# lbroseus/TALC

Hardware: AMD Instinct MI355X
Metric: corrected long-read bases/sec (whole node); k-mer-probe HBM GB/s (higher is better)
Workload: dtype u8

## Files before the change

talc_amd/csrc/pure_capi.cpp:

```cpp
#include <algorithm>
#include <cstdint>
#include <vector>

#include "talc_pure.h"
#include "talc_wfa.h"

using namespace talc;

extern "C" {

int pure_is_expected_by_model(double alpha, uint32_t nextc, uint32_t cc, int classe_unexpected) {
  return is_expected_by_model(alpha, nextc, cc, classe_unexpected != 0) ? 1 : 0;
}
int pure_is_expected_by_last_node(double alpha, uint32_t nextc, uint32_t cc) {
  return is_expected_by_last_node(alpha, nextc, cc) ? 1 : 0;
}
int pure_tag_next_nodes(double alpha, double err, uint32_t minc, const uint32_t* cnt4, const uint32_t* jc4, uint32_t count,
                        int complex, int32_t* tags4, double* dist4) {
  int t[4];
  double d[4];
  int n = tag_next_nodes(alpha, err, minc, cnt4, jc4, count, complex != 0, t, d);
  for (int i = 0; i < 4; ++i) { tags4[i] = t[i]; dist4[i] = d[i]; }
  return n;
}

struct KP { int32_t key; int32_t payload; };
struct KPLess { bool operator()(const KP& a, const KP& b) const { return a.key < b.key; } };
void pure_gnu_sort_pairs(int32_t* keys, int32_t* payloads, int n) {
  std::vector<KP> v(n);
  for (int i = 0; i < n; ++i) v[i] = KP{keys[i], payloads[i]};
  gnu_sort(v.data(), n, KPLess());
  for (int i = 0; i < n; ++i) { keys[i] = v[i].key; payloads[i] = v[i].payload; }
}
void pure_std_sort_pairs(int32_t* keys, int32_t* payloads, int n) {
  std::vector<KP> v(n);
  for (int i = 0; i < n; ++i) v[i] = KP{keys[i], payloads[i]};
  std::sort(v.begin(), v.end(), KPLess());
  for (int i = 0; i < n; ++i) { keys[i] = v[i].key; payloads[i] = v[i].payload; }
}

void pure_gnu_heapsort_pairs(int32_t* keys, int32_t* payloads, int n) {
  std::vector<KP> v(n);
  for (int i = 0; i < n; ++i) v[i] = KP{keys[i], payloads[i]};
  gs_heapsort(v.data(), 0, n, KPLess());
  for (int i = 0; i < n; ++i) { keys[i] = v[i].key; payloads[i] = v[i].payload; }
}
void pure_std_heapsort_pairs(int32_t* keys, int32_t* payloads, int n) {
  std::vector<KP> v(n);
  for (int i = 0; i < n; ++i) v[i] = KP{keys[i], payloads[i]};
  std::partial_sort(v.begin(), v.end(), v.end(), KPLess());
  for (int i = 0; i < n; ++i) { keys[i] = v[i].key; payloads[i] = v[i].payload; }
}

int pure_gardening(uint32_t maxb, int n, const double* scores, const double* dists, uint32_t* kept, int32_t* isComplex) {
  std::vector<ValIdx> wv(n + 1);
  std::vector<Rank4> r1(n + 1), r2(n + 1);
  bool cx = false;
  int nk = gardening(maxb, n, scores, dists, wv.data(), r1.data(), r2.data(), kept, &cx);
  *isComplex = cx ? 1 : 0;
  return nk;
}

void pure_sort_anchors(double cc, uint32_t* pos, uint32_t* count, int n) {
  std::vector<AnchorRec> a(n);
  for (int i = 0; i < n; ++i) a[i] = AnchorRec{0, 0, pos[i], count[i]};
  gnu_sort(a.data(), n, LessAnchor{cc});
  for (int i = 0; i < n; ++i) { pos[i] = a[i].pos; count[i] = a[i].count; }
}

void pure_wfa_xdrop(const uint8_t* q, int qlen, const uint8_t* d, int dlen, int x, int32_t* out4) {
  const WfaResult r = wfa_xdrop_scalar(q, qlen, d, dlen, x);
  out4[0] = r.moved; out4[1] = r.extCols; out4[2] = r.extRows; out4[3] = r.score;
}
}
```

talc_amd/csrc/talc_capi_correct.inc:

```

static uint32_t next_launch_stamp() {
  static std::atomic<uint32_t> launches{0};
  return 0x01000000u + (launches.fetch_add(1) & 0xFFFFFFu);
}
static void ensure_edge_boxes(talc_ctx* c, Stage& st) {
  const uint64_t gap = (uint64_t)c->p.max_border_length + 256;
  const uint32_t seqCap = (uint32_t)align_up((uint64_t)(2.2 * (double)gap) + 4ull * c->p.k + 64, 16);
  const uint64_t need = (uint64_t)st.n_slots * edge_box_bytes(seqCap) + (uint64_t)st.n_slots * 4;
  if (c->sw.edgeTasks == 0 || c->p.max_start_anchors < 2 || c->p.max_start_anchors > EDGE_BOX_ANCHORS ||
      seqCap > (1u << 16) || need > (1ull << 30)) {
    st.boxes.reset(); st.boxes_bytes = 0;
    return;
  }
  if (need > st.boxes_bytes || seqCap != st.box_seq_cap) {
    st.boxes.reset(); st.boxes_bytes = 0;
    if (st.boxes.alloc(need) != hipSuccess) { (void)hipGetLastError(); return; }
    st.boxes_bytes = need; st.box_seq_cap = seqCap;
  }
}

static int ensure_stage(talc_ctx* c, Stage& st, uint32_t maxLen, uint32_t scale, uint32_t n_work) {
  const SearchCaps caps = make_caps(maxLen, c->p.k, scale, scale == 1 ? c->sw.seqArena : 0, scale == 1 && c->sw.tinyCaps);
  hipDeviceProp_t prop;
  HIPCHK(hipGetDeviceProperties(&prop, c->device));
  uint32_t want = (uint32_t)prop.multiProcessorCount * (scale == 1 ? 4u * TALC_SEARCH_WAVES_PER_SIMD : scale <= 8 ? 4u : 1u);
  if (c->sw.searchSlots) want = c->sw.searchSlots;
  const uint32_t wantSlots = std::max<uint32_t>(1, std::min<uint32_t>(want, n_work));
  if (scale > 1 && c->sw.failRetryAlloc)
    return fail(TALC_ERR_NOMEM, "TALC_TEST_FAIL_RETRY_ALLOC: the retry stage is refused");
  for (int attempt = 0; attempt < 2; ++attempt) {
    uint32_t slots = wantSlots;
    size_t freeB = 0, totalB = 0;
    HIPCHK(hipMemGetInfo(&freeB, &totalB));
    const uint64_t avail = (uint64_t)(0.6 * (double)freeB) + st.scratch_bytes;
    while (slots > 1 && (uint64_t)slots * caps.slotBytes > avail) slots /= 2;
    const uint64_t need = (uint64_t)slots * caps.slotBytes;
    const bool cramped = slots < wantSlots || (uint64_t)caps.slotBytes > avail;
    if (cramped && attempt == 0 && c->cache.pool_bytes) { c->cache.trim(0); continue; }
    if ((uint64_t)caps.slotBytes > avail && need > st.scratch_bytes)
      return fail(TALC_ERR_NOMEM, "per-wave scratch of %llu bytes does not fit the device", (unsigned long long)caps.slotBytes);
    if (need > st.scratch_bytes) {
      st.scratch.reset(); st.scratch_bytes = 0;
      if (st.scratch.alloc(need) != hipSuccess) {
        (void)hipGetLastError();
        if (attempt == 0) { c->cache.trim(0); continue; }
        return fail(TALC_ERR_NOMEM, "cannot allocate %llu bytes of search scratch", (unsigned long long)need);
      }
      st.scratch_bytes = need;
    }
    st.n_slots = slots;
    st.caps = caps;
    return TALC_OK;
  }
  return fail(TALC_ERR_NOMEM, "search scratch does not fit the device");
}

struct TraceHost {
  DevBuf<TraceRec> d_recs; DevBuf<uint32_t> d_nrec; DevBuf<uint8_t> d_pool; DevBuf<uint32_t> d_npool;
  uint32_t cap = 0, poolCap = 0;
};

#ifdef TALC_PROF
static int prof_report(talc_ctx* c, talc_batch* b, const uint64_t* counters) {
  if (!c->sw.profReads.empty()) {
    if (FILE* f = fopen(c->sw.profReads.c_str(), "w")) {
      fprintf(f, "read\tlen\tstatus\tregions\tcost_est\thead\ttail\tgap_sum\tfork\tsolid\tticks_100MHz\tgap_sq\tgap_max\tsq640\tsteps\tedge_ticks\tanchors\tanchor_max\tstart\tbridges\tbridge_max\n");
      for (uint32_t r = 0; r < b->n_reads; ++r) {
        const ReadState& st = b->h_state[r];
        fprintf(f, "%u\t%llu\t%d\t%u\t%u\t%u\t%u\t%u\t%u\t%u\t%u\t%u\t%u\t%u\t%u\t%u\t%u\t%u\t%u\t%u\t%u\n", r, (unsigned long long)(b->h_offsets[r + 1] - b->h_offsets[r]), st.status,
                st.nRegions, st.costEst, st.pfHead, st.pfTail, st.pfGapSum, st.pfFork, st.pfSolid, st.pfTicks, st.pfGapSq, st.pfGapMax, st.pfShortReg, st.pfSteps, st.pfEdgeTicks, st.pfAnchors, st.pfAnchorMax, st.pfStart, st.pfBridges, st.pfBridgeMax);
      }
      fclose(f);
    }
  }
  if (!c->sw.profPrint) return TALC_OK;
  static const char* nm[] = TALC_PF_NAMES;
  const uint64_t tot = counters[2 + PF_TOTAL];
  for (int i = 0; i < PF_N; ++i) fprintf(stderr, "[prof] %-10s %14llu cycles  %5.1f%%\n", nm[i], (unsigned long long)counters[2 + i], tot ? 100.0 * counters[2 + i] / tot : 0.0);
  if (counters[127] > counters[126] && c->stage.n_slots)
    fprintf(stderr, "[prof] wave utilisation: %.1f%% of %u waves x %.3f ms (first start to last end, 100 MHz counter)\n",
            100.0 * (double)counters[125] / ((double)(counters[127] - counters[126]) * c->stage.n_slots), c->stage.n_slots,
            (double)(counters[127] - counters[126]) / 1e5);
  if (counters[124] != ~0ull && counters[124] > counters[126])
    fprintf(stderr, "[prof] the work queue ran dry %.3f ms after the first wave's start\n", (double)(counters[124] - counters[126]) / 1e5);
  if (c->sw.profSlow && c->stage.n_slots) {
    const uint32_t nw = std::min<uint32_t>(c->stage.n_slots, 8192);
    std::vector<uint64_t> lg(2 * (size_t)nw);
    HIPCHK(hipMemcpy(lg.data(), c->d_counters.get() + 128, lg.size() * 8, hipMemcpyDeviceToHost));
    std::vector<uint32_t> idx(nw);
    for (uint32_t i = 0; i < nw; ++i) idx[i] = i;
    const uint32_t t0 = (uint32_t)counters[126];
    auto endOf = [&](uint32_t w) { return (uint32_t)((uint32_t)lg[2 * w + 1] - t0); };
    std::sort(idx.begin(), idx.end(), [&](uint32_t a, uint32_t b2) { return endOf(a) > endOf(b2); });
    fprintf(stderr, "[slow] wave end times (ms), deciles from the last:");
    for (int d = 0; d <= 10; ++d) fprintf(stderr, " %.1f", endOf(idx[std::min<uint32_t>(nw - 1, (uint32_t)((uint64_t)d * nw / 10))]) / 1e5);
    fprintf(stderr, "\n");
    for (uint32_t i = 0; i < std::min<uint32_t>(nw, 24); ++i) {
      const uint32_t w = idx[i];
      const uint32_t qi = (uint32_t)(lg[2 * w] >> 32), r = (uint32_t)lg[2 * w], st = (uint32_t)(lg[2 * w + 1] >> 32) - t0;
      const uint64_t L = (b->h_offsets.empty() || r >= b->n_reads) ? 0 : b->h_offsets[r + 1] - b->h_offsets[r];
      fprintf(stderr, "[slow] wave %5u ends %8.3f ms: last read %7u (queue %7u, len %6llu) started %8.3f ms\n", w, endOf(w) / 1e5, r, qi,
              (unsigned long long)L, st / 1e5);
    }
  }
  return TALC_OK;
}
#endif

static int run_pipeline(talc_ctx* c, talc_batch* b, TraceHost* th, uint32_t traceRead) {
  HIPCHK(hipSetDevice(c->device));
  hipStream_t s = c->stream;
  int rc;
  TraceBuf tb = {};
  if (th) { tb.recs = th->d_recs.get(); tb.nrec = th->d_nrec.get(); tb.cap = th->cap; tb.pool = th->d_pool.get(); tb.npool = th->d_npool.get(); tb.poolCap = th->poolCap; tb.steps = c->sw.traceSteps ? 1 : 0; }
  memset(&c->timing, 0, sizeof c->timing);
  c->timing.n_kmers = b->n_kmers; c->timing.n_bases = b->n_bases;
  HIPCHK(hipEventRecord(c->ev[0], s));
  if (!b->encoded && (rc = launch_encode(c, b))) return rc;
  HIPCHK(hipEventRecord(c->ev[1], s));
  if ((rc = launch_coverage(c, b))) return rc;
  HIPCHK(hipEventRecord(c->ev[2], s));
  HIPCHK(hipMemsetAsync(c->d_hist.get() + 1024, 0, 256 * sizeof(uint32_t), s));
  if (b->n_reads)
    hipLaunchKernelGGL(k_structure, dim3(b->n_reads), dim3(64), 0, s, c->dp, c->view, b->d_codes.get(), b->d_offsets.get(), b->d_koff.get(),
                       b->d_cov.get(), b->d_covw.get(), b->d_nin.get(), b->d_state.get(), b->d_regions.get(), b->d_regoff.get(), b->d_headcov.get(), b->n_reads, tb, traceRead, c->d_hist.get() + 1024);
  HIPCHK(hipGetLastError());
  HIPCHK(hipEventRecord(c->ev[3], s));
  if (b->n_reads) {
    HIPCHK(hipMemsetAsync(c->d_hist.get(), 0, 1024 * sizeof(uint32_t), s));
    const unsigned nb = (b->n_reads + 255) / 256;
    hipLaunchKernelGGL(k_order_scale, dim3(1), dim3(64), 0, s, c->d_hist.get() + 1024);
    hipLaunchKernelGGL(k_order_hist, dim3(nb), dim3(256), 0, s, b->d_state.get(), b->n_reads, c->d_hist.get(), c->d_hist.get() + 1024);
    hipLaunchKernelGGL(k_order_scan, dim3(1), dim3(1024), 0, s, c->d_hist.get());
    hipLaunchKernelGGL(k_order_scatter, dim3(nb), dim3(256), 0, s, b->d_state.get(), b->n_reads, c->d_hist.get(), b->d_order.get(), c->d_hist.get() + 1024);
    HIPCHK(hipGetLastError());
  }
  HIPCHK(hipMemsetAsync(c->d_queue.get(), 0, kQueueWords * sizeof(uint32_t), s));
  HIPCHK(hipMemsetAsync(c->d_counters.get(), 0, (128 + 2 * 8192) * sizeof(uint64_t), s));
  HIPCHK(hipMemsetAsync(c->d_counters.get() + 126, 0xFF, sizeof(uint64_t), s));
  HIPCHK(hipMemsetAsync(c->d_counters.get() + 124, 0xFF, sizeof(uint64_t), s));
  if (b->n_reads) {
    if ((rc = ensure_stage(c, c->stage, b->max_len, 1, b->n_reads))) return rc;
    ensure_edge_boxes(c, c->stage);
    EdgeTaskArgs ea = {};
    if (c->stage.boxes) {
      ea.boxes = c->stage.boxes.get();
      ea.avail = (uint32_t*)(c->stage.boxes.get() + (uint64_t)c->stage.n_slots * edge_box_bytes(c->stage.box_seq_cap));
      ea.seqCap = c->stage.box_seq_cap;
      ea.minWeak = c->sw.edgeTaskMin; ea.heavy = c->sw.edgeTaskHeavy; ea.heavyRounds = c->sw.edgeTaskRounds;
      ea.lingerMod = c->sw.edgeLingerMod; ea.test = c->sw.edgeRedo ? 1u : 0u;
      ea.autoSwitch = c->sw.edgeTasks > 0 ? nullptr : c->d_hist.get() + 1024 + 129;
      HIPCHK(hipMemsetAsync(ea.avail, 0, (uint64_t)c->stage.n_slots * 4, s));
    }
    hipLaunchKernelGGL(k_search, dim3(c->stage.n_slots), dim3(64), 0, s, c->dp, c->view, c->stage.caps, b->d_codes.get(), b->d_offsets.get(),
                       b->d_koff.get(), b->d_cov.get(), b->d_covw.get(), b->d_state.get(), b->d_regions.get(), b->d_regoff.get(), b->d_headcov.get(), b->d_out.get(), b->d_outoff.get(), b->d_order.get(),
                       b->n_reads, c->d_queue.get(), c->stage.scratch.get(), c->d_counters.get(), tb, traceRead, next_launch_stamp(), ea);
    HIPCHK(hipGetLastError());
  }
  HIPCHK(hipEventRecord(c->ev[4], s));
  b->h_state.resize(b->n_reads);
  if (b->n_reads) HIPCHK(hipMemcpyAsync(b->h_state.data(), b->d_state.get(), b->n_reads * sizeof(ReadState), hipMemcpyDeviceToHost, s));
  HIPCHK(hipStreamSynchronize(s));
  std::vector<uint32_t> retry;
  for (uint32_t r = 0; r < b->n_reads; ++r) if (b->h_state[r].overflow) retry.push_back(r);
  c->timing.n_retried = (uint32_t)retry.size();
  HIPCHK(hipEventRecord(c->ev[5], s));
  for (uint32_t scale = 8; scale <= 64 && !retry.empty(); scale *= 8) {
    Stage big;
    if ((rc = ensure_stage(c, big, b->max_len, scale, (uint32_t)retry.size()))) {
      if (rc == TALC_ERR_NOMEM) break;
      return rc;
    }
    DevBuf<uint32_t> d_retry;
    if (d_retry.alloc(retry.size()) != hipSuccess) { (void)hipGetLastError(); break; }
    HIPCHK(hipMemcpyAsync(d_retry.get(), retry.data(), retry.size() * 4, hipMemcpyHostToDevice, s));
    for (uint32_t r : retry) {
      b->h_state[r].overflow = 0;
      HIPCHK(hipMemcpyAsync(b->d_state.get() + r, &b->h_state[r], sizeof(ReadState), hipMemcpyHostToDevice, s));
    }
    HIPCHK(hipMemsetAsync(c->d_queue.get(), 0, kQueueWords * sizeof(uint32_t), s));
    hipLaunchKernelGGL(k_search, dim3(big.n_slots), dim3(64), 0, s, c->dp, c->view, big.caps, b->d_codes.get(), b->d_offsets.get(), b->d_koff.get(),
                       b->d_cov.get(), b->d_covw.get(), b->d_state.get(), b->d_regions.get(), b->d_regoff.get(), b->d_headcov.get(), b->d_out.get(), b->d_outoff.get(), d_retry.get(), (uint32_t)retry.size(),
                       c->d_queue.get(), big.scratch.get(), c->d_counters.get(), tb, traceRead, next_launch_stamp(), EdgeTaskArgs());
    HIPCHK(hipGetLastError());
    HIPCHK(hipMemcpyAsync(b->h_state.data(), b->d_state.get(), b->n_reads * sizeof(ReadState), hipMemcpyDeviceToHost, s));
    HIPCHK(hipStreamSynchronize(s));
    d_retry.reset(); big = Stage();
    std::vector<uint32_t> again;
    for (uint32_t r : retry) if (b->h_state[r].overflow) again.push_back(r);
    retry.swap(again);
  }
  HIPCHK(hipEventRecord(c->ev[6], s));
  uint32_t nfail = 0;
  std::vector<uint64_t> dense_off(b->n_reads + 1);
  uint64_t pos = 0;
  for (uint32_t r = 0; r < b->n_reads; ++r) {
    dense_off[r] = pos;
    pos += b->h_state[r].outLen;
    if (b->h_state[r].overflow) nfail++;
  }
  dense_off[b->n_reads] = pos;
  b->h_dense_off = dense_off;
  if (b->d_dense && b->dense_cap < pos) b->d_dense.reset();
  if (!b->d_dense) { b->dense_cap = std::max<uint64_t>(pos, 1); HIPCHK(b->d_dense.alloc(c->cache, b->dense_cap)); }
  if (!b->d_dense_off) HIPCHK(b->d_dense_off.alloc(c->cache, b->n_reads + 1));
  HIPCHK(hipMemcpyAsync(b->d_dense_off.get(), dense_off.data(), (b->n_reads + 1) * 8, hipMemcpyHostToDevice, s));
  if (b->n_reads)
    hipLaunchKernelGGL(k_pack, dim3(b->n_reads), dim3(256), 0, s, b->d_out.get(), b->d_outoff.get(), b->d_state.get(), b->d_dense_off.get(), b->d_dense.get(),
                       b->n_reads, c->p.reverse ? 1 : 0);
  HIPCHK(hipGetLastError());
  HIPCHK(hipEventRecord(c->ev[7], s));
  uint64_t counters[128] = {0};
  HIPCHK(hipMemcpyAsync(counters, c->d_counters.get(), 128 * 8, hipMemcpyDeviceToHost, s));
  HIPCHK(hipStreamSynchronize(s));
  HIPCHK(hipEventElapsedTime(&c->timing.encode_ms, c->ev[0], c->ev[1]));
  HIPCHK(hipEventElapsedTime(&c->timing.coverage_ms, c->ev[1], c->ev[2]));
  HIPCHK(hipEventElapsedTime(&c->timing.structure_ms, c->ev[2], c->ev[3]));
  HIPCHK(hipEventElapsedTime(&c->timing.search_ms, c->ev[3], c->ev[4]));
  HIPCHK(hipEventElapsedTime(&c->timing.retry_ms, c->ev[5], c->ev[6]));
  HIPCHK(hipEventElapsedTime(&c->timing.emit_ms, c->ev[6], c->ev[7]));
  c->timing.n_trail_steps = counters[0];
  c->timing.n_dp_cells = counters[1];
  c->timing.n_failed = nfail;
#ifdef TALC_PROF
  if ((rc = prof_report(c, b, counters))) return rc;
#endif
  b->corrected = true;
  if (nfail) {
    fail(TALC_WARN_READ_ERRORS, "%u read(s) exhausted the device scratch even in the retry pass (status TALC_READ_ERROR)", nfail);
    return TALC_WARN_READ_ERRORS;
  }
  return TALC_OK;
}

int talc_batch_correct(talc_ctx* c, talc_batch* b) {
  if (!c || !b || b->ctx != c) return fail(TALC_ERR_INVALID, "bad context/batch");
  return run_pipeline(c, b, nullptr, 0xFFFFFFFFu);
}

uint64_t talc_batch_corrected_bytes(const talc_batch* b) { return (b && b->corrected) ? b->h_dense_off[b->n_reads] : 0; }

int talc_batch_fetch_corrected(talc_ctx* c, talc_batch* b, char* out, uint64_t out_capacity, uint64_t* out_offsets,
                               int32_t* status) {
  if (!c || !b || b->ctx != c) return fail(TALC_ERR_INVALID, "bad context/batch");
  if (!b->corrected) return fail(TALC_ERR_STATE, "talc_batch_correct has not run on this batch");
  HIPCHK(hipSetDevice(c->device));
  const uint64_t total = b->h_dense_off[b->n_reads];
  if (out_offsets) memcpy(out_offsets, b->h_dense_off.data(), (b->n_reads + 1) * 8);
  if (status)
    for (uint32_t r = 0; r < b->n_reads; ++r) status[r] = b->h_state[r].overflow ? TALC_READ_ERROR : b->h_state[r].status;
  if (out) {
    if (out_capacity < total) return fail(TALC_ERR_CAPACITY, "output buffer too small: need %llu bytes", (unsigned long long)total);
    if (total) {
      HIPCHK(hipMemcpyAsync(out, b->d_dense.get(), total, hipMemcpyDeviceToHost, c->stream));
      HIPCHK(hipStreamSynchronize(c->stream));
    }
  }
  return TALC_OK;
}

int talc_batch_fetch_read_stats(talc_ctx* c, talc_batch* b, int64_t* stats5) {
  if (!c || !b || b->ctx != c || !stats5) return fail(TALC_ERR_INVALID, "bad context/batch/buffer");
  if (!b->corrected) return fail(TALC_ERR_STATE, "talc_batch_correct has not run on this batch");
  const uint32_t K = c->p.k;
  for (uint32_t r = 0; r < b->n_reads; ++r) {
    const ReadState& st = b->h_state[r];
    const uint64_t L = b->h_offsets[r + 1] - b->h_offsets[r];
    int64_t* o = stats5 + 5ull * r;
    const bool row = L > K;
    const bool corrected = st.status == TALC_READ_CORRECTED && !st.overflow;
    o[0] = row ? 1 : 0;
    o[1] = row ? (int64_t)L : 0;
    o[2] = (row && st.status != TALC_READ_NO_SOLID_KMER && st.status != TALC_READ_SKIPPED_SHORT) ? (int64_t)st.inSpan : 0;
    o[3] = (row && st.status != TALC_READ_NO_SOLID_KMER && st.status != TALC_READ_SKIPPED_SHORT) ? (int64_t)st.nRegions : 0;
    o[4] = (row && corrected) ? (int64_t)st.outLen : 0;
  }
  return TALC_OK;
}

int talc_batch_copy_corrected_device(talc_ctx* c, talc_batch* b, void* device_out, uint64_t out_capacity,
                                     uint64_t* out_offsets, int32_t* status) {
  if (!c || !b || b->ctx != c || !device_out) return fail(TALC_ERR_INVALID, "bad context/batch/buffer");
  if (!b->corrected) return fail(TALC_ERR_STATE, "talc_batch_correct has not run on this batch");
  HIPCHK(hipSetDevice(c->device));
  const uint64_t total = b->h_dense_off[b->n_reads];
  if (out_offsets) memcpy(out_offsets, b->h_dense_off.data(), (b->n_reads + 1) * 8);
  if (status)
    for (uint32_t r = 0; r < b->n_reads; ++r) status[r] = b->h_state[r].overflow ? TALC_READ_ERROR : b->h_state[r].status;
  if (out_capacity < total) return fail(TALC_ERR_CAPACITY, "device buffer too small: need %llu bytes", (unsigned long long)total);
  if (total) {
    HIPCHK(hipMemcpyAsync(device_out, b->d_dense.get(), total, hipMemcpyDeviceToDevice, c->stream));
    HIPCHK(hipStreamSynchronize(c->stream));
  }
  return TALC_OK;
}

int talc_correct_batch(talc_ctx* c, const char* bases, const uint64_t* offsets, uint32_t n_reads, char* out,
                       uint64_t out_capacity, uint64_t* out_offsets, int32_t* status) {
  talc_batch* b = nullptr;
  int rc = talc_batch_create(c, bases, offsets, n_reads, &b);
  if (rc) return rc;
  rc = talc_batch_correct(c, b);
  int rc2 = (rc >= 0) ? talc_batch_fetch_corrected(c, b, out, out_capacity, out_offsets, status) : rc;
  talc_batch_destroy(b);
  return rc2 ? rc2 : rc;
}

int64_t talc_batch_trace_read(talc_ctx* c, talc_batch* b, uint32_t read_index, char* buf, uint64_t cap) {
  if (!c || !b || b->ctx != c || read_index >= b->n_reads) return fail(TALC_ERR_INVALID, "bad context/batch/read index");
  HIPCHK(hipSetDevice(c->device));
  const uint64_t off = b->h_offsets[read_index], len = b->h_offsets[read_index + 1] - off;
  std::vector<char> raw(std::max<uint64_t>(len, 1));
  if (len) HIPCHK(hipMemcpy(raw.data(), b->d_raw.get() + off, len, hipMemcpyDeviceToHost));
  uint64_t offs[2] = {0, len};
  talc_batch* one = nullptr;
  int rc = talc_batch_create(c, raw.data(), offs, 1, &one);
  if (rc) return rc;
  const std::unique_ptr<talc_batch> tbch(one);
  TraceHost th;
  th.cap = 1u << 18; th.poolCap = 1u << 24;
  HIPCHK(th.d_recs.alloc(th.cap));
  HIPCHK(th.d_nrec.alloc(1)); HIPCHK(th.d_npool.alloc(1));
  HIPCHK(th.d_pool.alloc(th.poolCap));
  HIPCHK(hipMemsetAsync(th.d_nrec.get(), 0, 4, c->stream)); HIPCHK(hipMemsetAsync(th.d_npool.get(), 0, 4, c->stream));
  rc = run_pipeline(c, tbch.get(), &th, 0);
  std::ostringstream os;
  uint32_t nrec = 0, npool = 0;
  HIPCHK(hipMemcpy(&nrec, th.d_nrec.get(), 4, hipMemcpyDeviceToHost));
  HIPCHK(hipMemcpy(&npool, th.d_npool.get(), 4, hipMemcpyDeviceToHost));
  nrec = std::min(nrec, th.cap); npool = std::min(npool, th.poolCap);
  std::vector<TraceRec> recs(nrec);
  std::vector<uint8_t> pool(std::max<uint32_t>(npool, 1));
  if (nrec) HIPCHK(hipMemcpy(recs.data(), th.d_recs.get(), (size_t)nrec * sizeof(TraceRec), hipMemcpyDeviceToHost));
  if (npool) HIPCHK(hipMemcpy(pool.data(), th.d_pool.get(), npool, hipMemcpyDeviceToHost));
  const int stv = tbch->h_state.empty() ? -1 : (tbch->h_state[0].overflow ? TALC_READ_ERROR : tbch->h_state[0].status);
  os << "STATUS " << stv << "\n";
// ... 40 lines not shown
```

talc_amd/csrc/talc_kernels_search.h:

```cpp
#pragma once
#include "talc_common.h"
#include "talc_kernels_probe.h"
#include "talc_pure.h"
#include "talc_wave.h"

namespace talc {

#define TCAP 288
#define NBUF (2 * TCAP)
#ifndef LDS_DP_CAP
#define LDS_DP_CAP 320
#endif
#ifndef HOT
#define HOT 8
#endif
#ifndef AIMS_LDS
#define AIMS_LDS 16
#endif

enum : uint32_t {
  OVF_ANCHORS = 1, OVF_FULLPATHS = 2, OVF_FULLPOOL = 4, OVF_TRAILS = 8, OVF_SEQ = 16, OVF_OUT = 32, OVF_WEAKPOOL = 64,
  OVF_REGIONS = 128, OVF_DP = 256
};

// ... 384 lines not shown
          ++new_start_pos;
          if (degree_of(new_start_pos, 0) > 1) OK = true;
        }
      }
      uint32_t new_end_pos = regEnd;
      if (OK & !lastAndNone) {
        int degEnd;
        if (reg < Rdeg) degEnd = (int)s_degE[reg];
        else degEnd = degree_of(new_end_pos, 1);
        if ((degEnd == 0) & (new_end_pos != n - 1)) {
          OK = false;
          while ((new_end_pos > regS[reg]) & !OK) {
            --new_end_pos;
            if (degree_of(new_end_pos, 1) > 1) OK = true;
          }
        }
      }
      if (OK) {
        if (reg + 1 < R) span = ((int)regS[reg + 1] - (int)(new_end_pos + K));
        if (span < 0) {
          if ((int)regE[reg + 1] + span >= (int)regS[reg + 1]) { if (l == 0) regS[reg + 1] = regS[reg + 1] - (uint32_t)span; }
          else { if (l == 0) regS[reg + 1] = new_start_pos; OK = false; }
          startMoved = true;
          WSYNC();
        }
        if (OK) {
          uint32_t c = 0;
          for (uint32_t i = new_start_pos + l; i <= new_end_pos; i += 64) c = max(c, cov_at(cov, i).x);
          c = wave_max_u32(c);
          const bool expected = !is_expected_by_model(P.ALPHA, c, solidThr, true);
          if (expected) {
            WSYNC();
            if (l == 0) { regS[nNew] = new_start_pos; regE[nNew] = new_end_pos; }
            WSYNC();
            ++nNew;
          }
        }
      }
    }
  }
  uint32_t Rfinal = (nNew > 0) ? nNew : R;
  bool checok = (R > 0);

  if (Rfinal > 0) {
    unsigned long long len = 0;
    if (regS[0] > 0) len += regS[0];
    const uint32_t eLast = regE[Rfinal - 1];
    if (eLast + 1 < n) len += (unsigned long long)L - ((unsigned long long)eLast + K);
    unsigned long long part = 0;
    for (uint32_t i = l; i + 1 < Rfinal; i += 64) {
      part += (unsigned long long)regE[i] + K - regS[i];
      if (regS[i + 1] > regE[i] + K) part += (unsigned long long)regS[i + 1] - ((unsigned long long)regE[i] + K);
    }
    len += wave_sum_u64(part);
    len += (unsigned long long)eLast + K - regS[Rfinal - 1];
    checok &= (len == (unsigned long long)L);
  }
  st.nRegions = Rfinal;
  if (l < kHeadCov) headCov[(uint64_t)r * kHeadCov + (uint32_t)l] = ((uint32_t)l < n) ? cov_at(cov, (uint32_t)l).x : 0u;
  {
    WSYNC();
    uint32_t* regH = regS + 2 * regCap;
    for (uint32_t i = l; i < Rfinal; i += 64) {
      const uint32_t s0 = regS[i], e0 = regE[i];
      const uint32_t hs = cov_hit_index(cov, s0);
      const bool endHit = ((cov_word(cov, e0 >> 6).bits >> (e0 & 63u)) & 1ull) != 0ull;
      const bool clean = ((s0 ^ e0) < (uint32_t)TALC_COV_TILE) && (e0 >= s0) && endHit && (cov_hit_index(cov, e0) - hs == e0 - s0);
      regH[i] = (hs & ~kRegClean) | (clean ? kRegClean : 0u);
    }
  }
  {
    unsigned long long part = 0;
    for (uint32_t i = l; i < Rfinal; i += 64) part += (unsigned long long)regE[i] - regS[i] + 1;
    st.inSpan = (uint32_t)wave_sum_u64(part);
  }
  if (!checok) st.status = TALC_READ_NO_STRUCTURE;
  if (checok && Rfinal > 0) {
    unsigned long long part = 0, sq = 0;
    for (uint32_t i = l; i + 1 < Rfinal; i += 64) {
      const unsigned long long g = (regS[i + 1] > regE[i] + K) ? (unsigned long long)(regS[i + 1] - (regE[i] + K)) : 0ull;
      part += 870ull * g + 20000ull;
      sq += g * g;
    }
    const unsigned long long gq = (unsigned long long)P.costGapQuad + ((unsigned long long)P.costGapFork * nFork) / max(m, 1ull);
    unsigned long long cost = wave_sum_u64(part) + gq * min(wave_sum_u64(sq), (unsigned long long)P.costGapCap * P.costGapCap);
    st.costGap = (uint32_t)min(cost >> 6, 0xFFFFFFFFull);
    if (l == 0) { atomicAdd(&batchStats[2 * (r & 63u)], (uint32_t)min(nFork, 0xFFFFull)); atomicAdd(&batchStats[2 * (r & 63u) + 1], (uint32_t)min(m, 0xFFFFFull)); }
    const unsigned long long head = regS[0], eLast = regE[Rfinal - 1];
    const unsigned long long tail = (eLast + 1 < n) ? (unsigned long long)L - (eLast + K) : 0ull;
    if (head > 0 && head <= P.MAX_BORDER_LEN) cost += (unsigned long long)P.costEdgeLin * head + (unsigned long long)P.costEdgeQuad * head * head;
    if (tail > 0 && tail <= P.MAX_BORDER_LEN) cost += (unsigned long long)P.costEdgeLin * tail + (unsigned long long)P.costEdgeQuad * tail * tail;
    cost += 50ull * (unsigned long long)L;
#ifdef TALC_PROF
    {
      unsigned long long gs = 0;
      for (uint32_t i = l; i + 1 < Rfinal; i += 64) gs += (regS[i + 1] > regE[i] + K) ? (unsigned long long)(regS[i + 1] - (regE[i] + K)) : 0ull;
      st.pfGapSum = (uint32_t)wave_sum_u64(gs);
      unsigned long long g2 = 0, sr = 0; uint32_t gm = 0;
      for (uint32_t i = l; i < Rfinal; i += 64) {
        const unsigned long long g = (i + 1 < Rfinal && regS[i + 1] > regE[i] + K) ? (unsigned long long)(regS[i + 1] - (regE[i] + K)) : 0ull;
        g2 += g * g; gm = max(gm, (uint32_t)g); sr += min(g, 640ull) * min(g, 640ull);
      }
      st.pfGapSq = (uint32_t)min(wave_sum_u64(g2), 0xFFFFFFFFull); st.pfGapMax = wave_max_u32(gm); st.pfShortReg = (uint32_t)wave_sum_u64(sr); st.pfSteps = 0;
      st.pfHead = (uint32_t)head; st.pfTail = (uint32_t)tail; st.pfFork = (uint32_t)nFork; st.pfSolid = (uint32_t)m; st.pfTicks = 0;
    }
#endif
    cost >>= 6;
    st.costEst = (uint32_t)min(cost, 0xFFFFFFFFull);
  }
  if (l == 0) state[r] = st;
  if (trace.recs && r == traceRead && l == 0) {
    uint32_t k = atomicAdd(trace.nrec, 1u);
    if (k < trace.cap) trace.recs[k] = TraceRec{TR_THRESHOLD, 0, 0, 0, 0, thr, 0, 0};
    for (uint32_t i = 0; i < Rfinal; ++i) {
      k = atomicAdd(trace.nrec, 1u);
      if (k < trace.cap) trace.recs[k] = TraceRec{TR_REGION, (int)regS[i], (int)regE[i], 0, 0, 0.0, 0, 0};
    }
  }
}

struct TrailSet {
  uint64_t* kmer; uint64_t* nmask; double* dist; uint32_t* cnt; int32_t* score; uint32_t* fail; int32_t* lanc;
  int32_t* ranc; uint32_t* buf;
};
TALC_D TrailSet make_set(uint8_t* meta) {
  TrailSet s;
  s.kmer = (uint64_t*)(meta + TrailSetLayout::kmer); s.nmask = (uint64_t*)(meta + TrailSetLayout::nmask);
  s.dist = (double*)(meta + TrailSetLayout::dist); s.cnt = (uint32_t*)(meta + TrailSetLayout::cnt);
  s.score = (int32_t*)(meta + TrailSetLayout::score); s.fail = (uint32_t*)(meta + TrailSetLayout::fail);
  s.lanc = (int32_t*)(meta + TrailSetLayout::lanc); s.ranc = (int32_t*)(meta + TrailSetLayout::ranc);
  s.buf = (uint32_t*)(meta + TrailSetLayout::buf);
  return s;
}

struct TrailRec { uint64_t kmer, nmask; double dist; uint32_t cnt; int32_t score; uint32_t fail; int32_t lanc, ranc; uint32_t buf; };

#define LSYNC() do { __builtin_amdgcn_fence(__ATOMIC_ACQ_REL, "wavefront"); __builtin_amdgcn_wave_barrier(); } while (0)

__shared__ TrailRec g_hot[2 * HOT];
__shared__ uint64_t g_aimK[AIMS_LDS], g_aimN[AIMS_LDS];
__shared__ uint32_t g_aimPos[AIMS_LDS];
#define BLOOM_WORDS 128
__shared__ unsigned long long g_bloom[BLOOM_WORDS];
__shared__ __attribute__((aligned(16))) int g_dp[3 * LDS_DP_CAP];

struct EdgeCand {
  bool have; double score; double dist; double idscore; uint32_t len; uint32_t lanc, ranc;
};

enum { PF_PROBE = 0, PF_CHILD, PF_AIMS, PF_CYCLE, PF_FFWD, PF_SCOREBR, PF_GARDEN, PF_EVALFULL, PF_XDROP, PF_EXTNW,
       PF_EDGEMISC, PF_ANCHORS, PF_ASSEMBLE, PF_STEPB, PF_STEPE, PF_SRCHB, PF_SRCHE, PF_PROLOG, PF_INITTR, PF_TOTAL, PF_NCALLS, PF_NSTEPS,
       PF_FFLOAD, PF_FFREC, PF_FFFLUSH, PF_FFENTRY, PF_NRECS, PF_RD0, PF_RD1, PF_RD2, PF_RD3, PF_RD4, PF_RD5, PF_RDMAX,
       PF_XSTAGE, PF_XLEV, PF_XSEL, PF_REFB, PF_RESULT, PF_CYQ, PF_CYX, PF_CYHIT, PF_CYFILL,
       PF_SB11, PF_SB12, PF_SB21, PF_SB10, PF_SBOTHER, PF_SEGEN, PF_XCALLS, PF_XNLEV, PF_FSFORK, PF_FSDEAD, PF_FSFILT, PF_FSLIM, PF_FK1, PF_FK2, PF_FKBAIL, PF_FORK, PF_ANCCALLS, PF_ANCITER, PF_TPUB, PF_TOWN, PF_TSTOLEN, PF_TWAIT, PF_TRUN, PF_EA0, PF_EA1, PF_EA2, PF_EA3, PF_EA4, PF_EASUM3, PF_EASUM4, PF_RANCH, PF_RANCHMAX, PF_RBR, PF_RBRMAX, PF_N };
#define TALC_PF_NAMES {"probe", "child", "aims", "cycle", "ffwd", "scorebr", "garden", "evalfull", "xdrop", "extnw", "edgemisc", \
                       "anchors", "assemble", "stepb*", "stepe*", "srchb*", "srche*", "prolog", "inittr", "total", "#ffcalls", "#ffsteps", \
                       "ff.load", "ff.record", "ff.flush", "ff.entry", "#ffrecords", "#reads<0.25ms", "#reads<1ms", "#reads<4ms", \
                       "#reads<16ms", "#reads<64ms", "#reads>=64ms", "maxread(10ns)", "x.stage", "x.levels", "x.select", "b.ref", "b.result", \
                       "#cyc.query", "#cyc.exact", "#cyc.found", "cyc.fill%sum", \
                       "#stepb 1->1", "#stepb 1->2", "#stepb 2->1", "#stepb 1->0", "#stepb other", "#stepe generic", "#xdrop calls", "#xdrop levels", \
                       "#ffstop fork", "#ffstop deadend", "#ffstop filter", "#ffstop limit/other", "#forkstep 1 child", "#forkstep fork+deadend", "#forkstep bailed", "forkstep", "#anchor lists", "#anchor level tests", \
                       "#edges published", "#anchors by owner", "#anchors by others", "t.owner waits", "t.run by others", \
                       "#edge anchors<1ms", "#edge anchors<4ms", "#edge anchors<16ms", "#edge anchors<64ms", "#edge anchors>=64ms", "ticks anchors 16-64ms", "ticks anchors>=64ms", "(per read) anchors", "(per read) longest anchor", "(per read) bridge attempts", "(per read) longest bridge attempt"}

struct Wv {
  DevParams P; TableView T; SearchLimits C;
  const uint8_t* read; uint32_t L, n; const uint2* cov; double lambda;
  TrailSet G[2];
  int ia;
  uint8_t* seqPool;
  uint32_t nBuf;
  unsigned long long freeMask[NBUF / 64];
  uint8_t *ref, *fullPool, *edgeLong, *edgeShort, *edgeTmp, *weak;
  AnchorRec *ancL, *ancR; uint32_t* ancPos;
  FullMeta* fullMeta;
  int *dpG;
  double* gScores; double* gDists; ValIdx* gVal; Rank4* gRank; uint32_t* gKept;
  uint32_t *regS, *regE, *wOff, *wLen;
  int location, dirRight;
  uint32_t Ls, Le, Rs, Re;
  uint32_t weakLen;
  bool complexRegion;
  bool ffPopped;
  int nAncL, nAncR;
  uint32_t refLen;
  int nFull; uint32_t fullUsed;
  EdgeCand best2[2];
  int nEdges;
  unsigned long long cells, steps;
  uint32_t overflow;
  const TraceBuf* tracep;
  bool tracing, traceSteps;
  unsigned long long* wideBloom;
  int* rowPool;
  uint32_t searchNo;
  uint32_t rowStride, rowAvail;
  uint32_t wideMask;
  uint32_t launchStamp;
  const CovWord* covw;
  uint32_t* regH;
  uint32_t LH, RH;
  const uint32_t* headCov;
  uint8_t* refBuf;
  uint8_t* boxes; uint32_t* avail; uint32_t* qwords;
  uint32_t boxBytes, boxSeqCap, nSlots, mySlot, nWork, taskMinWeak;
  uint32_t taskHeavy;
  uint32_t qi, heavyUpTo;
  uint32_t holding;
  uint32_t stealSeq;
  unsigned long long moreCells, moreSteps;
  uint32_t nanSeen;
  uint32_t taskTest;
};

enum { LOC_HEAD = 0, LOC_INNER = 1, LOC_TAIL = 2 };

__shared__ Wv g_X;
#define X g_X
#ifdef TALC_PROF
__shared__ uint32_t g_prof[PF_N];
#endif

#ifdef TALC_PROF
#define PROF_DECL unsigned long long _pf_t
#define PF_EDGE_T0() (_pf_e0 = __builtin_amdgcn_s_memrealtime())
#define PF_EDGE_T1() (_pf_edge += (uint32_t)(__builtin_amdgcn_s_memrealtime() - _pf_e0))
#define PROF_BEGIN() (_pf_t = __builtin_amdgcn_s_memtime())
#define PROF_END(cat) (g_prof[cat] += (uint32_t)(__builtin_amdgcn_s_memtime() - _pf_t))
#define PROF_DECL2 unsigned long long _pf_t2
#define PROF_COUNT(cat, n) do { if (lane_id() == 0) g_prof[cat] += (uint32_t)(n); } while (0)
#define PROF_BEGIN2() (_pf_t2 = __builtin_amdgcn_s_memtime())
#define PROF_END2(cat) (g_prof[cat] += (uint32_t)(__builtin_amdgcn_s_memtime() - _pf_t2))
#else
#define PROF_DECL
#define PF_EDGE_T0() ((void)0)
#define PF_EDGE_T1() ((void)0)
#define PROF_BEGIN() ((void)0)
#define PROF_END(cat) ((void)0)
#define PROF_DECL2
#define PROF_COUNT(cat, n) ((void)0)
#define PROF_BEGIN2() ((void)0)
#define PROF_END2(cat) ((void)0)
#endif

TALC_D CovRead cur_cov() { CovRead c; c.hits = (const uint2 TALC_AS1*)X.cov; c.words = (const CovWord TALC_AS1*)X.covw; return c; }
TALC_DNC unsigned long long cov_lookup(uint32_t i) { const uint2 v = cov_at(cur_cov(), i); return ((unsigned long long)v.y << 32) | v.x; }
#define COVX(i) ((uint32_t)cov_lookup(i))
#define COVY(i) ((uint32_t)(cov_lookup(i) >> 32))

TALC_D int* dp_array(int which, int need) {
  if ((uint32_t)need > X.C.dpCap) { X.overflow |= OVF_DP; }
  return X.dpG + (uint64_t)which * X.C.dpCap;
}

#define NW_REG_NB 12
TALC_DNC int nw_score(const uint8_t* a, int la, const uint8_t* b, int lb, int match, int mismatch, int gap,
                    bool freeBegin) {
  la = uni(la); lb = uni(lb);
  if (la < lb) { const uint8_t* t = a; a = b; b = t; int tl = la; la = lb; lb = tl; }
  unsigned long long ncells = 0;
  if (la <= 64 * NW_REG_NB) {
    const int B = (la + 63) >> 6;
    int r;
    if (B <= 1) r = wave_nw_reg<1>(a, la, b, lb, match, mismatch, gap, freeBegin, ncells);
    else if (B <= 2) r = wave_nw_reg<2>(a, la, b, lb, match, mismatch, gap, freeBegin, ncells);
    else if (B <= 3) r = wave_nw_reg<3>(a, la, b, lb, match, mismatch, gap, freeBegin, ncells);
    else if (B <= 4) r = wave_nw_reg<4>(a, la, b, lb, match, mismatch, gap, freeBegin, ncells);
    else if (B <= 6) r = wave_nw_reg<6>(a, la, b, lb, match, mismatch, gap, freeBegin, ncells);
    else if (B <= 8) r = wave_nw_reg<8>(a, la, b, lb, match, mismatch, gap, freeBegin, ncells);
    else r = wave_nw_reg<NW_REG_NB>(a, la, b, lb, match, mismatch, gap, freeBegin, ncells);
    X.cells += ncells;
    return r;
  }
  if ((uint32_t)(la + 1) > X.C.dpCap) { X.overflow |= OVF_DP; return 0; }
  int* row = dp_array(0, la + 1);
  const int r = wave_nw(a, la, b, lb, match, mismatch, gap, freeBegin, row, ncells);
  X.cells += ncells;
  return r;
}

#define NW2_REG_NB 8
TALC_DNC unsigned long long edit_and_lcs_sweep(const uint8_t* a, int la_, const uint8_t* b, int lb_, bool haveEdit_, bool haveLcs_) {
  const int la = uni(la_), lb = uni(lb_);
  const bool haveEdit = uni((int)haveEdit_) != 0, haveLcs = uni((int)haveLcs_) != 0;
  int editScore = 0, lcsLen = 0;
  if (!haveEdit && !haveLcs && la <= 64 * NW2_REG_NB) {
    unsigned long long ncells = 0;
    wave_edit_lcs_reg<NW2_REG_NB>(a, la, b, lb, editScore, lcsLen, ncells);
    X.cells += ncells;
  } else {
    if (!haveEdit) editScore = nw_score(a, la, b, lb, 0, -1, -1, false);
    if (!haveLcs) lcsLen = nw_score(a, la, b, lb, 1, 0, 0, false);
  }
  return ((unsigned long long)(uint32_t)uni(lcsLen) << 32) | (uint32_t)uni(editScore);
}

TALC_DN void edit_and_lcs(const uint8_t* a_, int la, const uint8_t* b_, int lb, int& editScore, int& lcsLen, bool needEdit_,
                          int acceptLcs_) {
  la = uni(la); lb = uni(lb);
  const bool needEdit = uni((int)needEdit_) != 0;
  const int acceptLcs = uni(acceptLcs_);
  const int acceptA = (!needEdit && acceptLcs > 0) ? 2 * acceptLcs : INT_MAX;
  const uint8_t* a = uni_ptr(a_); const uint8_t* b = uni_ptr(b_);
  if (la < lb) { const uint8_t* t = a; a = b; b = t; int tl = la; la = lb; lb = tl; }
  bool haveEdit = !needEdit, haveLcs = false;
  if (!needEdit) editScore = 0;
  constexpr int STAGE = 3 * LDS_DP_CAP * 4;
  const int qpad = (la + 16) & ~7;
  if (lb > 0 && qpad + lb + 16 <= STAGE) {
    uint8_t TALC_AS3* stage = (uint8_t TALC_AS3*)g_dp;
    const int l = lane_id();
    gcu8 ga = (gcu8)a; gcu8 gb = (gcu8)b;
    stage_copy(stage, ga, la);
    stage_copy(stage + qpad, gb, lb);
    if (l == 0) { stage[la] = 0xF0; stage[qpad + lb] = 0xF1; }
    WSYNC();
// ... 457 lines not shown
#ifdef TALC_PROF
    if (lane_id() == 0) g_prof[PF_XCALLS] += 1;
#endif
    constexpr int STAGE = 3 * LDS_DP_CAP * 4;
    uint8_t TALC_AS3* stage = (uint8_t TALC_AS3*)g_dp;
    const int ndiagonals = min(max(xdrop, 0), qlen) + min(max(xdrop, 0), dlen) + 1;
    if (MODE == 2) {
      int* mem = X.dpG + 2ull * X.C.dpCap + 256;
      WfaPhase ph{-1, 31, mem, mem + 512};
      rc = wave_xdrop_wfa<1>(seq2 + S, qlen, seq1 + S, dlen, xdrop, stage, STAGE, extCols, extRows, extScore, ncells, &ph);
      if (rc == 2) {
        ph.fromLevel = 31; ph.toLevel = 63;
        rc = wave_xdrop_wfa<2>(seq2 + S, qlen, seq1 + S, dlen, xdrop, stage, STAGE, extCols, extRows, extScore, ncells, &ph);
        if (rc == 2) {
          ph.fromLevel = 63; ph.toLevel = 127;
          rc = wave_xdrop_wfa<4>(seq2 + S, qlen, seq1 + S, dlen, xdrop, stage, STAGE, extCols, extRows, extScore, ncells, &ph);
          if (rc == 2) {
            ph.fromLevel = 127; ph.toLevel = (ndiagonals <= 511) ? -1 : 255;
            rc = wave_xdrop_wfa<8>(seq2 + S, qlen, seq1 + S, dlen, xdrop, stage, STAGE, extCols, extRows, extScore, ncells, &ph);
            if (rc == 2) {
              ph.fromLevel = 255; ph.toLevel = -1;
              rc = wave_xdrop_wfa<16>(seq2 + S, qlen, seq1 + S, dlen, xdrop, stage, STAGE, extCols, extRows, extScore, ncells, &ph);
            }
          }
        }
      }
    }
    else if (MODE == 0 && ndiagonals <= 63) rc = wave_xdrop_wfa<1>(seq2 + S, qlen, seq1 + S, dlen, xdrop, stage, STAGE, extCols, extRows, extScore, ncells, nullptr, state ? keepKey : 0u);
    else if (MODE == 1 && ndiagonals <= 255) {
      int* mem = X.dpG + 2ull * X.C.dpCap + 256;
      WfaPhase ph{-1, 31, mem, mem + 512};
      rc = wave_xdrop_wfa<1>(seq2 + S, qlen, seq1 + S, dlen, xdrop, stage, STAGE, extCols, extRows, extScore, ncells, &ph, state ? keepKey : 0u);
      if (rc == 2) {
        ph.fromLevel = 31; ph.toLevel = (ndiagonals <= 127) ? -1 : 63;
        rc = wave_xdrop_wfa<2>(seq2 + S, qlen, seq1 + S, dlen, xdrop, stage, STAGE, extCols, extRows, extScore, ncells, &ph);
        if (rc == 2) {
          ph.fromLevel = 63; ph.toLevel = -1;
          rc = wave_xdrop_wfa<4>(seq2 + S, qlen, seq1 + S, dlen, xdrop, stage, STAGE, extCols, extRows, extScore, ncells, &ph);
        }
      }
    }
    else rc = -1;
    if (LEAF && rc < 0) { r.fallback = true; return r; }
    if (rc < 0) {
      rc = -1;
      const unsigned long long packed = xdrop_sweep(seq2 + S, qlen, seq1 + S, dlen, xdrop);
      extCols = (int)(uint32_t)packed; extRows = (int)(uint32_t)(packed >> 32);
    }
    PROF_END(PF_XDROP);
    X.cells += ncells;
  }
  const int ext1 = extRows, ext2 = extCols;
  r.extRef = state ? ext1 : ext2;
  r.extCand = state ? ext2 : ext1;
  r.lenRefExt = S + r.extRef;
  r.lenHistExt = S + r.extCand;
  r.posOnRef = X.dirRight ? (S + r.extRef) : (refLen - K - r.extRef);
  if (max(r.lenRefExt, r.lenHistExt) >= K) {
    if (withScore) {
      bool sameAnchor = LEAF && rc == 1;
      if (LEAF && !sameAnchor) { r.fallback = true; return r; }
      if (!LEAF && rc == 1) {
        const int l = lane_id();
        sameAnchor = ballot64(l < S && ((gcu8)ref)[l < S ? l : 0] != ((gcu8)cand)[l < S ? l : 0]) == 0ull;
      }
      if (sameAnchor) r.score = extScore;
      else { PROF_BEGIN(); r.score = nw_score(ref, r.lenRefExt, cand, r.lenHistExt, 0, -1, -1, false); PROF_END(PF_EXTNW); }
    }
  } else {
    r.score = (-1) * xdrop;
    r.stop = true;
  }
  return r;
}

TALC_DNC SeedExt seed_and_extension_wide(const uint8_t* ref, int refLen, const uint8_t* cand, int candLen, int xdrop, bool withScore) {
  return seed_and_extension_body<2>(ref, refLen, cand, candLen, xdrop, withScore);
}
TALC_DN SeedExt seed_and_extension_mid(const uint8_t* ref, int refLen, const uint8_t* cand, int candLen, int xdrop, bool withScore) {
  return seed_and_extension_body<1>(ref, refLen, cand, candLen, xdrop, withScore);
}
TALC_DN SeedExt seed_and_extension_mid_leaf(const uint8_t* ref, int refLen, const uint8_t* cand, int candLen, int xdrop, uint32_t keepKey) {
  return seed_and_extension_body<1, true>(ref, refLen, cand, candLen, xdrop, true, keepKey);
}
TALC_DN SeedExt seed_and_extension_leaf(const uint8_t* ref, int refLen, const uint8_t* cand, int candLen, int xdrop, uint32_t keepKey) {
  {
    const int rl = uni(refLen), cl = uni(candLen), x = max(uni(xdrop), 0);
    const int S = uni(X.dirRight) ? (int)X.P.K - 1 : (int)X.P.K;
    const int qlen = min(rl, cl) - S, dlen = max(rl, cl) - S;
    if (qlen > 0 && dlen > 0) {
      const int nd = min(x, qlen) + min(x, dlen) + 1;
      if (nd > 63 && nd <= 255) [[clang::musttail]] return seed_and_extension_mid_leaf(ref, refLen, cand, candLen, xdrop, keepKey);
    }
  }
  return seed_and_extension_body<0, true>(ref, refLen, cand, candLen, xdrop, true, keepKey);
}
TALC_DN SeedExt seed_and_extension(const uint8_t* ref, int refLen, const uint8_t* cand, int candLen, int xdrop, bool withScore) {
  {
    const int rl = uni(refLen), cl = uni(candLen), x = max(uni(xdrop), 0);
    const int S = uni(X.dirRight) ? (int)X.P.K - 1 : (int)X.P.K;
    const int qlen = min(rl, cl) - S, dlen = max(rl, cl) - S;
    if (qlen > 0 && dlen > 0) {
      const int nd = min(x, qlen) + min(x, dlen) + 1;
      if (nd > 255 && nd <= 1023) [[clang::musttail]] return seed_and_extension_wide(ref, refLen, cand, candLen, xdrop, withScore);
      if (nd > 63 && nd <= 255) [[clang::musttail]] return seed_and_extension_mid(ref, refLen, cand, candLen, xdrop, withScore);
    }
  }
  return seed_and_extension_body<0>(ref, refLen, cand, candLen, xdrop, withScore);
}

TALC_D SeedExt seedext_plain(int refLen, int candLen, int extCols, int extRows, int xdrop) {
  const int K = uni((int)X.P.K);
  const int S = uni(X.dirRight) ? K - 1 : K;
  const bool state = !(refLen < candLen);
  const int qlen = (state ? candLen : refLen) - S, dlen = (state ? refLen : candLen) - S;
  if (!(qlen > 0 && dlen > 0)) { extCols = 0; extRows = 0; }
  SeedExt r;
  r.stop = false; r.score = 0;
  r.extRef = state ? extRows : extCols;
  r.extCand = state ? extCols : extRows;
  r.lenRefExt = S + r.extRef;
  r.lenHistExt = S + r.extCand;
  r.posOnRef = X.dirRight ? (S + r.extRef) : (refLen - K - r.extRef);
  if (!(max(r.lenRefExt, r.lenHistExt) >= K)) { r.score = (-1) * xdrop; r.stop = true; }
  return r;
}

TALC_DN bool seed_and_extension_multi(const uint8_t* ref, int refLen, const uint8_t* cand, int candLen, int xHi, int* resCols,
                                      int* resRows, int* resScore) {
  PROF_DECL;
  refLen = uni(refLen); candLen = uni(candLen); xHi = uni(xHi); ref = uni_ptr(ref); cand = uni_ptr(cand);
  resCols = (int*)uni_ptr(resCols); resRows = (int*)uni_ptr(resRows); resScore = (int*)uni_ptr(resScore);
  const int K = (int)X.P.K;
  const int S = X.dirRight ? K - 1 : K;
  const bool state = !(refLen < candLen);
  const uint8_t* seq1 = state ? ref : cand; const int len1 = state ? refLen : candLen;
  const uint8_t* seq2 = state ? cand : ref; const int len2 = state ? candLen : refLen;
  const int qlen = len2 - S, dlen = len1 - S;
  if (!(qlen > 0 && dlen > 0) || xHi < 0) return false;
  PROF_BEGIN();
  constexpr int STAGE = 3 * LDS_DP_CAP * 4;
  uint8_t TALC_AS3* stage = (uint8_t TALC_AS3*)g_dp;
  unsigned long long ncells = 0;
  const int ndiagonals = min(xHi, qlen) + min(xHi, dlen) + 1;
  int rc = -1;
  if (ndiagonals <= 63) rc = wave_xdrop_wfa_multi<1>(seq2 + S, qlen, seq1 + S, dlen, xHi, stage, STAGE, resCols, resRows, resScore, ncells);
  else if (ndiagonals <= 127) rc = wave_xdrop_wfa_multi<2>(seq2 + S, qlen, seq1 + S, dlen, xHi, stage, STAGE, resCols, resRows, resScore, ncells);
  PROF_END(PF_XDROP);
  X.cells += ncells;
  WSYNC();
  return rc >= 0;
}

TALC_D bool trail_seed_and_extend(int set_, int t_, int len_, int xdrop_) {
  const int set = uni(set_), t = uni(t_), len = uni(len_), xdrop = uni(xdrop_);
  WSYNC();
  const uint32_t buf = (uint32_t)uni((int)tr_buf(set, t));
  SeedExt e = seed_and_extension_leaf(X.ref, (int)X.refLen, X.seqPool + (uint64_t)buf * X.C.seqCap, len, xdrop, buf + 1u);
  if (uni((int)e.fallback) != 0) e = seed_and_extension(X.ref, (int)X.refLen, X.seqPool + (uint64_t)buf * X.C.seqCap, len, xdrop, true);
  const int lenHistExt = uni(e.lenHistExt), score = uni(e.score), posOnRef = uni(e.posOnRef);
  const bool stop = uni((int)e.stop) != 0;
  TrailRec r = tr_get(set, t);
  const bool ok1 = (lenHistExt == len);
  r.fail = ok1 ? 0u : r.fail + 1u;
  r.score = score;
  if (X.dirRight) r.ranc = posOnRef; else r.lanc = posOnRef;
  const bool ok = (uni((int)r.fail) <= (uint32_t)X.P.MAX_BORDER_FAILURES) & !stop;
  if (lane_id() == 0) tr_put(set, t, r);
  tr_sync(t);
  return ok;
}

TALC_DN void record_edge(int set_, int t_, int len0_) {
  PROF_DECL;
  const int set = uni(set_), t = uni(t_), len0 = uni(len0_);
  const int K = (int)X.P.K;
  WSYNC();
  uint32_t trBuf, trFail, lanc, ranc; int lastScore; unsigned long long distBits;
  {
    const TrailRec tr = tr_get(set, t);
    trBuf = (uint32_t)uni((int)tr.buf); trFail = (uint32_t)uni((int)tr.fail); lastScore = uni(tr.score);
    lanc = (uint32_t)uni(tr.lanc); ranc = (uint32_t)uni(tr.ranc);
    distBits = uni64((unsigned long long)__double_as_longlong(tr.dist / ((double)len0 + 0.01)));
  }
  const uint8_t* path = X.seqPool + (uint64_t)trBuf * X.C.seqCap;
  int len = len0;
  const uint32_t nbBases = trFail * X.P.CHECK_INTERVAL;
  if ((uint32_t)len >= nbBases + (uint32_t)K) len = len - (int)nbBases;
  const int refLen = uni((int)X.refLen);
  const bool shorter = (len <= refLen);
  int xdrop1 = (int)lastScore * (-1);
  SeedExt cur, nxt;
  const uint8_t* A = uni_ptr(shorter ? X.ref : path); const int lenA = shorter ? refLen : len;
  const uint8_t* Bq = uni_ptr(shorter ? path : X.ref); const int lenB = shorter ? len : refLen;
  int* const resCols = uni_ptr(X.dpG);
  int* const resRows = resCols + X.C.dpCap;
  int* const resScore = resCols + 2ull * X.C.dpCap;
  bool multi = false;
  if (xdrop1 >= 1 && (uint32_t)(xdrop1 + 1) <= X.C.dpCap && xdrop1 < 128)
    multi = seed_and_extension_multi(A, lenA, Bq, lenB, xdrop1, resCols, resRows, resScore);
  auto scalar = [](SeedExt e) -> SeedExt {
    e.lenRefExt = uni(e.lenRefExt); e.lenHistExt = uni(e.lenHistExt); e.posOnRef = uni(e.posOnRef); e.score = uni(e.score);
    e.stop = uni((int)e.stop) != 0; e.extRef = uni(e.extRef); e.extCand = uni(e.extCand);
    return e;
  };
  auto ext_at = [&](int x) -> SeedExt {
    if (multi && x >= 0) return seedext_plain(lenA, lenB, uni(resCols[x]), uni(resRows[x]), x);
    return scalar(seed_and_extension(A, lenA, Bq, lenB, x, false));
  };
  nxt = ext_at(xdrop1);
  bool goFurther = true;
  do {
    --xdrop1;
    cur = nxt;
    nxt = ext_at(xdrop1);
    if (nxt.lenHistExt < cur.lenHistExt) goFurther = false;
  } while (goFurther & (xdrop1 > 0));
  bool haveScore = false;
  int multiScore = 0;
  if (multi && !cur.stop) {
    const int sc = uni(resScore[xdrop1 + 1]);
    const int S = X.dirRight ? K - 1 : K;
    const int l = lane_id();
    if (sc <= 0 && ballot64(l < S && ((gcu8)A)[l < S ? l : 0] != ((gcu8)Bq)[l < S ? l : 0]) == 0ull) { haveScore = true; multiScore = sc; }
  }
  PROF_BEGIN();
  int scoreI;
  int lcs;
  {
    int es;
    edit_and_lcs(A, cur.lenRefExt, Bq, cur.lenHistExt, es, lcs, !cur.stop && !haveScore, 0);
    es = uni(es); lcs = uni(lcs);
    scoreI = cur.stop ? cur.score : (haveScore ? multiScore : es);
  }
  const double score = (double)scoreI;
  const double idscore = (double)lcs / (double)max(cur.lenRefExt, cur.lenHistExt);
  const double dist = __longlong_as_double((long long)distBits);
  if (dist != dist) X.nanSeen = 1u;
  uint8_t* tmp = uni_ptr(X.edgeTmp);
  uint32_t newLen;
  if (!shorter) {
    newLen = (uint32_t)cur.lenRefExt;
    if (newLen > X.C.edgeCap) { X.overflow |= OVF_SEQ; return; }
    copy_bytes(tmp, path, newLen, false);
  } else {
    const uint32_t from = (uint32_t)cur.lenRefExt;
    const uint32_t rest = (uint32_t)refLen > from ? (uint32_t)refLen - from : 0;
    newLen = (uint32_t)len + rest;
    if (newLen > X.C.edgeCap) { X.overflow |= OVF_SEQ; return; }
    copy_bytes(tmp, path, (uint32_t)len, false);
    copy_bytes(tmp + len, X.ref + from, rest, false);
  }
  WSYNC();
  uint32_t cutLen = 0, cutFrom = 0;
  if (newLen > (uint32_t)K) { cutLen = newLen - (uint32_t)K; cutFrom = (uint32_t)K; }
  X.nEdges++;
  const int bi = shorter ? 1 : 0;
  EdgeCand best = X.best2[bi];
  uint8_t* bestSeq = shorter ? X.edgeShort : X.edgeLong;
  bool take = false;
  if (!best.have) take = true;
  else if (score > best.score) take = true;
  else if (score == best.score && dist > best.dist) take = true;
  if (uni((int)take)) {
    best.have = true; best.score = score; best.dist = dist; best.idscore = idscore; best.len = cutLen;
    best.lanc = lanc; best.ranc = ranc;
    X.best2[bi] = best;
    copy_bytes(bestSeq, tmp + cutFrom, cutLen, false);
    WSYNC();
  }
  PROF_END(PF_EDGEMISC);
}

struct StepTags { int tags; uint32_t nc[4]; };

TALC_D ModelThresholds model_thresholds(uint32_t count, bool& inTable) {
  ModelThresholds m;
  const uint32_t TALC_AS1* thr = (const uint32_t TALC_AS1*)X.P.thr;
  const uint32_t lnRaw = lambda_noise_of(count, X.P.ERR);
  inTable = (count < X.P.thrN) & (lnRaw < X.P.thrN);
  const uint32_t c = min(count, X.P.thrN - 1u), ln = min(lnRaw, X.P.thrN - 1u);
  m.minExpected = thr[2u * c];
  m.belowUnexpected = thr[2u * ln + 1u];
  return m;
}

TALC_D StepTags probe_and_tag(int t, bool valid, bool complex) {
  StepTags r;
  uint32_t cnt[4] = {0, 0, 0, 0}, jc[4] = {0, 0, 0, 0};
  int tg[4] = {TAG_NONE, TAG_NONE, TAG_NONE, TAG_NONE};
  double ds[4] = {0, 0, 0, 0};
  if (valid) {
    uint64_t km, nm; uint32_t lc;
    if (t < HOT) { const TrailRec& h = g_hot[X.ia * HOT + t]; km = h.kmer; nm = h.nmask; lc = h.cnt; }
    else { const TrailRec h = tr_get_slow(X.ia, t); km = h.kmer; nm = h.nmask; lc = h.cnt; }
    const uint32_t K = X.P.K;
    const uint64_t succN = X.dirRight ? (nm >> 1) : (nm & ((1ULL << (K - 1)) - 1));
    bool inTable;
    const ModelThresholds mt = model_thresholds(lc, inTable);
    if (!succN) dev_next_counts(X.T, km, X.dirRight, cnt, jc);
    if (inTable) tag_next_nodes_with(mt, X.P.ERR, X.P.MIN_COUNT, cnt, jc, lc, complex, tg, (double*)nullptr);
    else tag_next_nodes(X.P.ALPHA, X.P.ERR, X.P.MIN_COUNT, cnt, jc, lc, complex, tg, ds);
  }
  r.tags = (tg[0] & 0xff) | ((tg[1] & 0xff) << 8) | ((tg[2] & 0xff) << 16) | ((tg[3] & 0xff) << 24);
#pragma unroll
  for (int b = 0; b < 4; ++b) r.nc[b] = cnt[b];
  return r;
}
TALC_D double shfl_f64(double v, int src) {
  long long x = __double_as_longlong(v);
  int lo = lane_get((int)(x & 0xffffffffll), src), hi = lane_get((int)(x >> 32), src);
// ... 295 lines not shown
    }
  }
  const int slot = nNew + l;
  if (has) {
    ((gu8)X.seqPool)[(uint64_t)ch.buf * X.C.seqCap + (uint32_t)len] = (uint8_t)bI;
    tr_put(ib, slot, ch);
  }
  WSYNC();
  int hit = -1;
  {
    const AnchorRec* aims = X.dirRight ? X.ancR : X.ancL;
    const int nAims = X.dirRight ? X.nAncR : X.nAncL;
    const int nl = min(nAims, AIMS_LDS);
    for (int a = 0; a < nl; ++a) if (has && hit < 0 && g_aimK[a] == ch.kmer && g_aimN[a] == ch.nmask) hit = a;
    for (int a = AIMS_LDS; a < nAims; ++a) { const AnchorRec ar = aims[a]; if (has && hit < 0 && ar.kmer == ch.kmer && ar.nmask == ch.nmask) hit = a; }
  }
  uint32_t hv = 0;
  bool maybe = false;
  if (has && hit < 0) maybe = bloom_query(ch.kmer, ch.nmask, hv) && (len > (int)K);
#ifdef TALC_PROF
  { const int q = (int)__popcll(ballot64(has && hit < 0)), x = (int)__popcll(ballot64(maybe)); if (l == 0) { g_prof[PF_CYQ] += (uint32_t)q; g_prof[PF_CYX] += (uint32_t)x; } }
#endif
  unsigned long long sp = ballot64(has && (hit >= 0 || maybe)), popM = 0ull;
  while (sp != 0ull) {
    const int f = (int)__builtin_ctzll(sp); sp &= sp - 1ull;
    const int hitF = lane_get(hit, f);
    if (hitF >= 0) {
      const uint64_t kmF = ((uint64_t)(uint32_t)lane_get((int)(uint32_t)(ch.kmer >> 32), f) << 32) | (uint32_t)lane_get((int)(uint32_t)ch.kmer, f);
      const uint64_t nmF = ((uint64_t)(uint32_t)lane_get((int)(uint32_t)(ch.nmask >> 32), f) << 32) | (uint32_t)lane_get((int)(uint32_t)ch.nmask, f);
      if (!uni((int)record_bridge_at_aim(nNew + f, hitF, len, kmF, nmF))) popM |= 1ull << f;
    } else {
      const bool cyc = uni((int)is_cycle_exact(lane_get(t, f), nNew + f, len)) != 0;
#ifdef TALC_PROF
      if (l == 0 && cyc) g_prof[PF_CYHIT] += 1;
#endif
      if (cyc) { pool_free((uint32_t)lane_get((int)ch.buf, f)); popM |= 1ull << f; }
    }
  }
  const bool surv = has && (((popM >> l) & 1ull) == 0ull);
  if (surv && hit < 0) {
    atomicOr(&g_bloom[hv >> 25], (1ull << ((hv >> 19) & 63u)) | (1ull << ((hv >> 13) & 63u)));
    const uint32_t wm = X.wideMask;
    if (wm != 0u) wide_or(X.wideBloom + wide_word(hv, wm), wide_bits(hv));
  }
  const unsigned long long survM = ballot64(surv);
  if (popM != 0ull) {
    TrailRec r = TrailRec();
    if (surv) r = tr_get(ib, slot);
    WSYNC();
    const unsigned long long below = (l == 0) ? 0ull : (~0ull >> (64 - l));
    if (surv) tr_put(ib, nNew + (int)__popcll(survM & below), r);
  }
  nNew += (int)__popcll(survM);
  WSYNC();
  return nNew;
}

TALC_D int step_bridge(int nCur, int len, uint32_t& stepCounter) {
  PROF_DECL;
  const DevParams& P = X.P;
  const int l = lane_id();
  const AnchorRec* aims = X.dirRight ? X.ancR : X.ancL;
  const int nAims = X.dirRight ? X.nAncR : X.nAncL;
  const int ib = X.ia ^ 1;
  int nNew = 0;
  uint32_t pend = 0; int nPend = 0;
  const bool complexIn = ((uint32_t)nCur > P.MAXB);
  for (int base = 0; base < nCur; base += 64) {
    const int tl = base + l;
    PROF_BEGIN();
    const StepTags mine = probe_and_tag(tl, tl < nCur, complexIn);
    PROF_END(PF_PROBE);
    const int cnt = min(64, nCur - base);
    X.steps += (unsigned long long)cnt;
    if (nCur > 1) {
      PROF_BEGIN();
      const int nn = uni(bridge_children_by_lane(mine.tags, mine.nc[0], mine.nc[1], mine.nc[2], mine.nc[3], base, cnt, len, nNew));
      PROF_END(PF_CHILD);
      if (nn >= 0) { nNew = nn; continue; }
    }
    for (int tt = 0; tt < cnt; ++tt) {
      const int t = base + tt;
      const int tags = lane_get(mine.tags, tt);
      const uint32_t pnc0 = (uint32_t)lane_get((int)mine.nc[0], tt), pnc1 = (uint32_t)lane_get((int)mine.nc[1], tt),
                     pnc2 = (uint32_t)lane_get((int)mine.nc[2], tt), pnc3 = (uint32_t)lane_get((int)mine.nc[3], tt);
      const int lastI = last_successor(tags);
      if (lastI < 0) pool_free(tr_buf(X.ia, t));
#pragma nounroll
      for (int i = 0; i < 4; ++i) {
        const int tag = (int)(int8_t)((tags >> (8 * i)) & 0xff);
        if (tag == TAG_NONE || tag == TAG_UNEXPECTED) continue;
        const uint32_t nc = (i == 0) ? pnc0 : (i == 1) ? pnc1 : (i == 2) ? pnc2 : pnc3;
        if (nNew >= TCAP) { X.overflow |= OVF_TRAILS; continue; }
        if ((uint32_t)(len + 1) > X.C.seqCap) { X.overflow |= OVF_SEQ; continue; }
        PROF_BEGIN();
        uint64_t km2, nm2;
        make_child<true>(t, nNew, i, len, nc, i == lastI, km2, nm2);
        PROF_END(PF_CHILD);
        int hit = -1;
        PROF_BEGIN();
        {
          const int nl = min(nAims, AIMS_LDS);
          const bool eq0 = (l < nl) && (g_aimK[l] == km2) && (g_aimN[l] == nm2);
          const unsigned long long m0 = ballot64(eq0);
          if (m0) hit = (int)__ffsll((long long)m0) - 1;
          for (int ab = AIMS_LDS; ab < nAims && hit < 0; ab += 64) {
            const int a = ab + l;
            const bool eq = (a < nAims) && (aims[a].kmer == km2) && (aims[a].nmask == nm2);
            const unsigned long long m = ballot64(eq);
            if (m) hit = ab + (int)__ffsll((long long)m) - 1;
          }
        }
        PROF_END(PF_AIMS);
        if (hit >= 0) {
          if (!uni((int)record_bridge_at_aim(nNew, hit, len, km2, nm2))) continue;
          ++nNew;
        } else {
          PROF_BEGIN();
          uint32_t hv;
          const bool cyc = uni((int)is_cycle(t, nNew, len, km2, nm2, hv)) != 0;
          PROF_END(PF_CYCLE);
          if (cyc) { pool_free(tr_buf(ib, nNew)); continue; }
          if (l == nPend) pend = hv;
          if (++nPend == 64) { bloom_flush(pend, 64); nPend = 0; }
          ++nNew;
        }
      }
    }
  }
  bloom_flush(pend, nPend);
  const bool complex = ((uint32_t)nNew > P.MAXB);
  ++stepCounter;
#ifdef TALC_PROF
  if (l == 0) g_prof[(nCur == 1 && nNew == 1) ? PF_SB11 : (nCur == 1 && nNew == 2) ? PF_SB12 : (nCur == 2 && nNew == 1) ? PF_SB21 : (nCur == 1 && nNew == 0) ? PF_SB10 : PF_SBOTHER] += 1;
#endif
  int nOut;
  if (complex & (stepCounter % P.CHECK_INTERVAL == 0)) {
    PROF_BEGIN();
    score_bridges(ib, nNew, len, stepCounter);
    PROF_END(PF_SCOREBR);
    bool cx = false;
    PROF_BEGIN();
    nOut = uni(garden(nNew, len + 1, cx));
    PROF_END(PF_GARDEN);
    X.complexRegion |= cx;
  } else {
    swap_sets();
    nOut = nNew;
  }
  return nOut;
}

TALC_DNC int score_edges_multi(int ib_, int n_, int len_, int& xdrop_);
TALC_D int score_edges(int ib_, int n_, int len_, int& xdrop_) {
  const int n = uni(n_), len = uni(len_);
  if (n == 0) return 0;
  const int ib = uni(ib_);
  const int xdrop = uni(xdrop_) + 2;
  if (n == 1) {
    const bool ok = uni((int)trail_seed_and_extend(ib, 0, len, xdrop)) != 0;
    xdrop_ = ok ? (int)((double)uni(tr_get(ib, 0).score) * (-1)) : 0;
    if (!ok) { record_edge(ib, 0, len); pool_free((uint32_t)uni((int)tr_buf(ib, 0))); return 0; }
    return 1;
  }
  int xd = xdrop - 2;
  const int kept = uni(score_edges_multi(ib, n, len, xd));
  xdrop_ = uni(xd);
  return kept;
}
TALC_DNC int score_edges_multi(int ib_, int n_, int len_, int& xdrop_) {
  const int n = uni(n_), len = uni(len_), ib = uni(ib_);
  const int l = lane_id();
  const int xdrop = uni(xdrop_) + 2;
  int new_xdrop = 0;
  int nSel = 0;
  for (int t = 0; t < n; ++t) {
    const bool ok = uni((int)trail_seed_and_extend(ib, t, len, xdrop)) != 0;
    if (l == 0) X.gKept[t] = ok ? 1u : 0u;
    if (ok) {
      const int current_xdrop = (int)((double)uni(tr_get(ib, t).score) * (-1));
      if ((new_xdrop > current_xdrop) || (new_xdrop == 0)) new_xdrop = current_xdrop;
      ++nSel;
    }
  }
  WSYNC();
  xdrop_ = new_xdrop;
  if (nSel == 0) {
    for (int t = 0; t < n; ++t) { record_edge(ib, t, len); pool_free((uint32_t)uni((int)tr_buf(ib, t))); }
    return 0;
  }
  int w = 0;
  for (int t = 0; t < n; ++t) {
    if (uni((int)X.gKept[t])) {
      if (w != t) {
        const TrailRec r = tr_get(ib, t);
        WSYNC();
        if (l == 0) tr_put(ib, w, r);
        WSYNC();
      }
      ++w;
    } else {
      pool_free((uint32_t)uni((int)tr_buf(ib, t)));
    }
  }
  WSYNC();
  return w;
}

TALC_DN int step_edge(int nCur, int len, uint32_t& stepCounter, uint32_t PATH_MAXLENGTH, int& xdrop) {
  PROF_DECL;
  const DevParams& P = X.P;
  const int l = lane_id();
  const int ib = X.ia ^ 1;
  int nNew = 0;
  uint32_t pend = 0; int nPend = 0;
  const bool complexIn = (nCur > 7);
  for (int base = 0; base < nCur; base += 64) {
    const int tl = base + l;
    PROF_BEGIN();
    const StepTags mine = probe_and_tag(tl, tl < nCur, complexIn);
    PROF_END(PF_PROBE);
    const int cnt = min(64, nCur - base);
    X.steps += (unsigned long long)cnt;
    for (int tt = 0; tt < cnt; ++tt) {
      const int t = base + tt;
      const int tags = lane_get(mine.tags, tt);
      const uint32_t pnc0 = (uint32_t)lane_get((int)mine.nc[0], tt), pnc1 = (uint32_t)lane_get((int)mine.nc[1], tt),
                     pnc2 = (uint32_t)lane_get((int)mine.nc[2], tt), pnc3 = (uint32_t)lane_get((int)mine.nc[3], tt);
      int counter = 0;
      const int lastI = last_successor(tags);
#pragma nounroll
      for (int i = 0; i < 4; ++i) {
        const int tag = (int)(int8_t)((tags >> (8 * i)) & 0xff);
        if (tag == TAG_NONE || tag == TAG_UNEXPECTED) continue;
        ++counter;
        const uint32_t nc = (i == 0) ? pnc0 : (i == 1) ? pnc1 : (i == 2) ? pnc2 : pnc3;
        if (nNew >= TCAP) { X.overflow |= OVF_TRAILS; continue; }
        if ((uint32_t)(len + 1) > X.C.seqCap) { X.overflow |= OVF_SEQ; continue; }
        PROF_BEGIN();
        uint64_t km2, nm2;
        make_child<false>(t, nNew, i, len, nc, i == lastI, km2, nm2);
        PROF_END(PF_CHILD);
        PROF_BEGIN();
        uint32_t hv;
        const bool cycle = uni((int)is_cycle(t, nNew, len, km2, nm2, hv)) != 0;
        PROF_END(PF_CYCLE);
        if (cycle || (stepCounter + 1 > PATH_MAXLENGTH)) {
          trail_seed_and_extend(ib, nNew, len + 1, xdrop);
          record_edge(ib, nNew, len + 1);
          pool_free(tr_buf(ib, nNew));
          continue;
        }
        if (l == nPend) pend = hv;
        if (++nPend == 64) { bloom_flush(pend, 64); nPend = 0; }
        ++nNew;
      }
      if (counter == 0) {
        trail_seed_and_extend(X.ia, t, len, xdrop);
        record_edge(X.ia, t, len);
        pool_free(tr_buf(X.ia, t));
      }
    }
  }
  bloom_flush(pend, nPend);
  ++stepCounter;
#ifdef TALC_PROF
  if (l == 0) g_prof[PF_SEGEN] += 1;
#endif
  int nOut;
  if ((stepCounter % P.CHECK_INTERVAL == 0) || ((uint32_t)nNew >= P.MAX_BORDER_PATHS)) {
    nNew = uni(score_edges(X.ia ^ 1, nNew, len + 1, xdrop));
    if (nNew > 5) {
      bool cx = false;
      PROF_BEGIN();
      nOut = uni(garden(nNew, len + 1, cx));
      PROF_END(PF_GARDEN);
      X.complexRegion |= cx;
    } else { swap_sets(); nOut = nNew; }
  } else { swap_sets(); nOut = nNew; }
  return nOut;
}

template <bool dirRight>
TALC_D int fast_forward_dir(int len_, uint32_t& stepCounter_, uint32_t PATH_MAXLENGTH_, bool edge_) {
  const DevParams& P = X.P;
  const int l = lane_id();
  const bool edge = uni((int)edge_) != 0;
  if (uni((int)(X.traceSteps)) != 0) return 0;
  const TrailRec r0 = tr_get(X.ia, 0);
  if (uni64(r0.nmask) != 0ull) return 0;
  const uint32_t K = (uint32_t)uni((int)P.K), MINC = (uint32_t)uni((int)P.MIN_COUNT), CHECK = (uint32_t)uni((int)P.CHECK_INTERVAL);
  const uint32_t seqCap = (uint32_t)uni((int)X.C.seqCap), PMAX = (uint32_t)uni((int)PATH_MAXLENGTH_);
  const uint64_t cap = uni64(X.T.capacity);
  const Bucket TALC_AS4* tab = (const Bucket TALC_AS4*)uni_ptr(dirRight ? X.T.right : X.T.left);
  const uint64_t kmask = (1ULL << (2 * K)) - 1, m1 = (1ULL << (2 * (K - 1))) - 1;
  uint64_t kmer = uni64(r0.kmer);
  uint32_t cnt = (uint32_t)uni((int)r0.cnt);
  const int len0 = uni(len_);
  const uint32_t sc0 = (uint32_t)uni((int)stepCounter_);
  int maxSteps = 0;
  if (sc0 < PMAX && (uint32_t)len0 < seqCap) {
    maxSteps = (int)min(PMAX - sc0, seqCap - (uint32_t)len0);
    if (edge) maxSteps = min(maxSteps, (int)(CHECK - (sc0 % CHECK)));
  }
  gu8 seq = (gu8)uni_ptr(X.seqPool + (uint64_t)r0.buf * X.C.seqCap);
  const unsigned long long bw0 = g_bloom[l], bw1 = g_bloom[l + 64];
  int bwLo = (int)(uint32_t)bw0, bwHi = (int)(uint32_t)(bw0 >> 32), bxLo = (int)(uint32_t)bw1, bxHi = (int)(uint32_t)(bw1 >> 32);
  int recN = 0, recB = 0;
  uint32_t cFlush = cnt;
  double dist = r0.dist;
  int done = 0, flushed = 0;
  uint64_t key = dirRight ? (kmer & m1) : (kmer >> 2);

  auto flush = [&]() {
    const int n = done - flushed;
    if (n <= 0) return;
    if (l < n) seq[len0 + flushed + l] = (uint8_t)recB;
    int cprev = lane_shr1(recN);
    if (l == 0) cprev = (int)cFlush;
    const double term = fabs((double)(uint32_t)cprev - (double)(uint32_t)recN) / sqrt((double)(uint32_t)cprev);
    const unsigned long long tb = (unsigned long long)__double_as_longlong(term);
    const int tLo = (int)(uint32_t)tb, tHi = (int)(uint32_t)(tb >> 32);
    for (int j = 0; j < n; ++j) {
      const unsigned long long v = ((unsigned long long)(uint32_t)lane_get(tHi, j) << 32) | (uint32_t)lane_get(tLo, j);
      dist = dist + __longlong_as_double((long long)v);
    }
    cFlush = (uint32_t)lane_get(recN, n - 1);
    flushed = done;
  };

  uint64_t slot = table_slot(table_hash(key), cap);
  v8u32 b = *(const v8u32 TALC_AS4*)(tab + slot);
  while (done < maxSteps) {
    bool found = false;
    while (true) {
      const uint64_t bk = ((uint64_t)b[1] << 32) | b[0];
      if ((bk & kKeyMask) == key) { found = true; break; }
      if (bk == kEmptyKey) break;
      if (++slot == cap) slot = 0;
      b = *(const v8u32 TALC_AS4*)(tab + slot);
    }
    if (!found) break;
    asm volatile("" :: "s"(b[6]), "s"(b[7]));
    const uint32_t c0 = b[2], c1 = b[3], c2 = b[4], c3 = b[5];
    int m;
    asm("s_cmp_ge_u32 %4, %5\n\ts_cselect_b32 %0, 1, 0\n\ts_cmp_ge_u32 %3, %5\n\ts_addc_u32 %0, %0, %0\n\t"
        "s_cmp_ge_u32 %2, %5\n\ts_addc_u32 %0, %0, %0\n\ts_cmp_ge_u32 %1, %5\n\ts_addc_u32 %0, %0, %0"
        : "=&s"(m) : "s"(c0), "s"(c1), "s"(c2), "s"(c3), "s"(MINC) : "scc");
    if (m == 0 || (m & (m - 1)) != 0) break;
    const int which = __builtin_ctz((unsigned)m);
    uint32_t nc;
    asm("s_max_u32 %0, %1, %2\n\ts_max_u32 %0, %0, %3\n\ts_max_u32 %0, %0, %4" : "=&s"(nc) : "s"(c0), "s"(c1), "s"(c2), "s"(c3) : "scc");
    uint64_t km2;
    if (dirRight) km2 = ((kmer << 2) | (uint64_t)which) & kmask;
    else km2 = ((uint64_t)which << (2 * (K - 1))) | (kmer >> 2);
    key = dirRight ? (km2 & m1) : (km2 >> 2);
    const uint64_t h2 = table_hash(key);
    slot = table_slot(h2, cap);
    b = *(const v8u32 TALC_AS4*)(tab + slot);
    const int bwi = bloom_word(h2);
    const int bwl = bwi & 63;
    const bool upper = (bwi & 64) != 0;
    const unsigned long long bm = bloom_mask(h2);
    const unsigned long long bv = upper ? (((unsigned long long)(uint32_t)lane_get(bxHi, bwl) << 32) | (uint32_t)lane_get(bxLo, bwl))
                                        : (((unsigned long long)(uint32_t)lane_get(bwHi, bwl) << 32) | (uint32_t)lane_get(bwLo, bwl));
    if ((bv & bm) == bm) break;
    if (upper) { bxLo = lane_set(bxLo, (int)(uint32_t)(bv | bm), bwl); bxHi = lane_set(bxHi, (int)(uint32_t)((bv | bm) >> 32), bwl); }
    else { bwLo = lane_set(bwLo, (int)(uint32_t)(bv | bm), bwl); bwHi = lane_set(bwHi, (int)(uint32_t)((bv | bm) >> 32), bwl); }
    const int rs = done - flushed;
    recN = lane_set(recN, (int)nc, rs);
    recB = lane_set(recB, which, rs);
    kmer = km2;
    cnt = nc;
    ++done;
    if (done - flushed == 64) flush();
  }

  flush();
  g_bloom[l] = ((unsigned long long)(uint32_t)bwHi << 32) | (uint32_t)bwLo;
  g_bloom[l + 64] = ((unsigned long long)(uint32_t)bxHi << 32) | (uint32_t)bxLo;
  stepCounter_ = sc0 + (uint32_t)done;
#ifdef TALC_PROF
  if (l == 0) { g_prof[PF_NCALLS] += 1; g_prof[PF_NSTEPS] += (uint32_t)done; }
#endif
  if (done) {
    X.steps += (unsigned long long)done;
    if (l == 0) {
      TrailRec r = r0;
      r.kmer = kmer; r.cnt = cnt; r.dist = dist;
      tr_put(X.ia, 0, r);
    }
  }
  LSYNC();
  return done;
}

template <int P>
TALC_D uint32_t dpp_row_shr(uint32_t v, uint32_t old) {
  return (uint32_t)__builtin_amdgcn_update_dpp((int)old, (int)v, 0x110 + P, 0xF, 0xF, false);
}

template <bool dirRight, bool WIDEF>
TALC_D int fast_forward_walk(int len_, uint32_t& stepCounter_, uint32_t PATH_MAXLENGTH_, bool edge_) {
  PROF_DECL; PROF_DECL2;
  PROF_BEGIN2();
  const DevParams& P = X.P;
  const int l = lane_id();
  const bool edge = uni((int)edge_) != 0;
  if (uni((int)(X.traceSteps)) != 0) return 0;
  const TrailRec r0 = tr_get(X.ia, 0);
  if (uni64(r0.nmask) != 0ull) return 0;
  const uint32_t K = (uint32_t)uni((int)P.K), CHECK = (uint32_t)uni((int)P.CHECK_INTERVAL);
  const uint32_t seqCap = (uint32_t)uni((int)X.C.seqCap), PMAX = (uint32_t)uni((int)PATH_MAXLENGTH_);
  const uint64_t cap = uni64(X.T.capacity);
  const uint32_t TALC_AS1* wtab = (const uint32_t TALC_AS1*)uni_ptr(dirRight ? X.T.walkRight : X.T.walkLeft);
  const uint32_t wideMask = WIDEF ? (uint32_t)uni((int)X.wideMask) : 0u;
  unsigned long long* const wideBloom = WIDEF ? (unsigned long long*)uni_ptr(X.wideBloom) : nullptr;
  const uint64_t kmask = (1ULL << (2 * K)) - 1, m1 = (1ULL << (2 * (K - 1))) - 1;
  uint64_t kmer = uni64(r0.kmer);
  uint32_t cnt = (uint32_t)uni((int)r0.cnt);
  const int len0 = uni(len_);
  const uint32_t sc0 = (uint32_t)uni((int)stepCounter_);
  int maxSteps = 0;
  if (sc0 < PMAX && (uint32_t)len0 < seqCap) {
    maxSteps = (int)min(PMAX - sc0, seqCap - (uint32_t)len0);
    if (edge) maxSteps = min(maxSteps, (int)(CHECK - (sc0 % CHECK)));
  }
  gu8 seq = (gu8)uni_ptr(X.seqPool + (uint64_t)r0.buf * X.C.seqCap);
  const int nAims = edge ? 0 : uni(dirRight ? X.nAncR : X.nAncL);
  int lanc = uni((int)r0.lanc), ranc = uni((int)r0.ranc);
  bool popped = false;
  uint32_t* recN = (uint32_t*)g_dp;
  uint32_t cFlush = cnt;
  double dist = r0.dist;
  int done = 0, flushed = 0;

  auto flush = [&]() {
    const int n = done - flushed;
    if (n <= 0) return;
    PROF_DECL; PROF_BEGIN();
    const uint32_t cn = (l < n) ? recN[l] : 1u;
    const uint32_t cprev = (l == 0) ? cFlush : ((l < n) ? recN[l - 1] : 1u);
    const double term = fabs((double)cprev - (double)cn) / sqrt((double)cprev);
    double* recT = (double*)(g_dp + 64);
    recT[l] = term;
    LSYNC();
#pragma unroll 8
    for (int j = 0; j < n; ++j) dist = dist + recT[j];
    cFlush = (uint32_t)lane_get((int)cn, n - 1);
    flushed = done;
    LSYNC();
    PROF_END(PF_FFFLUSH);
  };

  const uint32_t laneOff = (l < TALC_WALK_LEVELS) ? (uint32_t)(2 + (l >> 1)) : (l == TALC_WALK_LEVELS + 1 ? 1u : 0u);
  const uint32_t laneShift = (l < TALC_WALK_LEVELS && (l & 1)) ? 16u : 0u;
  const int lj = min(l, TALC_WALK_LEVELS - 1);
  const uint32_t laneSingle = (l < TALC_WALK_LEVELS) ? kWalkSingle : 0u;
  uint64_t key = dirRight ? (kmer & m1) : (kmer >> 2);
  uint32_t hh = (uint32_t)(table_hash(key) >> 32);
  PROF_END2(PF_FFENTRY);
  uint32_t ePre = 0;
  bool havePre = false;
  while (done < maxSteps) {
    if (done - flushed > 64 - TALC_WALK_LEVELS) flush();
    PROF_BEGIN();
    uint64_t slot = ((uint64_t)hh * (uint64_t)(uint32_t)cap) >> 32;
    uint32_t e = havePre ? ePre : wtab[slot * 8 + laneOff];
    havePre = false;
    bool found = true;
    while (true) {
      const uint64_t bk = ((uint64_t)(uint32_t)lane_get((int)e, TALC_WALK_LEVELS + 1) << 32) | (uint32_t)lane_get((int)e, TALC_WALK_LEVELS);
      if (bk == key) break;
      if (bk == kEmptyKey) { found = false; break; }
      if (++slot == cap) slot = 0;
      e = wtab[slot * 8 + laneOff];
    }
    PROF_END(PF_FFLOAD);
#ifdef TALC_PROF
    if (l == 0) g_prof[PF_NRECS] += 1;
#endif
    if (!found) break;
    PROF_BEGIN();
    const uint32_t lev = (e >> laneShift) & 0xFFFFu, top = lev & kWalkTopNone;
#ifdef TALC_PROF
    {
      const unsigned long long pm = ballot64((l < TALC_WALK_LEVELS) && (lev & kWalkSingle) != 0u);
      const int j0 = __builtin_ctzll(~pm);
      if (j0 < TALC_WALK_LEVELS && j0 < maxSteps - done) {
        const uint32_t t0 = (uint32_t)lane_get((int)top, j0);
        if (l == 0) g_prof[(t0 >= X.P.MIN_COUNT) ? PF_FSFORK : PF_FSDEAD] += 1;
      }
    }
#endif
    const unsigned long long passMask = ballot64((lev & laneSingle) != 0u);
    int nOK = min(__builtin_ctzll(~passMask), maxSteps - done);
    if (nOK == 0) break;
    const uint32_t which = (l < TALC_WALK_LEVELS) ? (lev >> kWalkBaseShift) : 0u;
    uint32_t pre = which << (dirRight ? 2 * (TALC_WALK_LEVELS - 1 - lj) : 2 * lj);
    pre |= dpp_row_shr<1>(pre, 0u);
    pre |= dpp_row_shr<2>(pre, 0u);
    pre |= dpp_row_shr<4>(pre, 0u);
    pre |= dpp_row_shr<8>(pre, 0u);
    uint64_t km;
    if (dirRight) km = ((kmer << (2 * (lj + 1))) | (uint64_t)(pre >> (2 * (TALC_WALK_LEVELS - 1 - lj)))) & kmask;
    else km = ((uint64_t)pre << (2 * (K - 1 - (uint32_t)lj))) | (kmer >> (2 * (lj + 1)));
    const uint64_t key2 = dirRight ? (km & m1) : (km >> 2);
    const uint32_t hv = (uint32_t)(table_hash(key2) >> 32);
    {
      const uint64_t slotN = ((uint64_t)(uint32_t)lane_get((int)hv, TALC_WALK_LEVELS - 1) * (uint64_t)(uint32_t)cap) >> 32;
      ePre = wtab[slotN * 8 + laneOff];
    }
    bool dup = dpp_row_shr<1>(hv, ~hv) == hv;
    dup |= dpp_row_shr<2>(hv, ~hv) == hv;
    dup |= dpp_row_shr<3>(hv, ~hv) == hv;
    dup |= dpp_row_shr<4>(hv, ~hv) == hv;
    dup |= dpp_row_shr<5>(hv, ~hv) == hv;
    dup |= dpp_row_shr<6>(hv, ~hv) == hv;
    dup |= dpp_row_shr<7>(hv, ~hv) == hv;
    dup |= dpp_row_shr<8>(hv, ~hv) == hv;
    dup |= dpp_row_shr<9>(hv, ~hv) == hv;
    dup |= dpp_row_shr<10>(hv, ~hv) == hv;
    dup |= dpp_row_shr<11>(hv, ~hv) == hv;
    static_assert(TALC_WALK_LEVELS == 12, "the lane roles above are written for 12 levels (+ 2 key lanes) in a 16-lane row");
    const int bwi = (int)(hv >> 25);
    const unsigned long long bm = (1ull << ((hv >> 19) & 63u)) | (1ull << ((hv >> 13) & 63u));
    bool seen = (g_bloom[bwi] & bm) == bm;
    unsigned long long* const wideW = WIDEF ? wideBloom + wide_word(hv, wideMask) : nullptr;
    const unsigned long long bmW = WIDEF ? wide_bits(hv) : 0ull;
    if (WIDEF) {
      const bool ask = seen && (l < TALC_WALK_LEVELS);
      if (ballot64(ask) != 0ull) { const unsigned long long bvW = ask ? wide_load(wideW) : 0ull; seen = ask && ((bvW & bmW) == bmW); }
    }
    const unsigned long long hitMask = ballot64(seen || dup) | (1ull << TALC_WALK_LEVELS);
    const int hitLevel = __builtin_ctzll(hitMask);
    int aimIdx = -1;
    if (nAims > 0 && nAims <= AIMS_LDS && hitLevel < nOK) {
      const uint64_t kmH = ((uint64_t)(uint32_t)lane_get((int)(uint32_t)(km >> 32), hitLevel) << 32) | (uint32_t)lane_get((int)(uint32_t)km, hitLevel);
      const unsigned long long am = ballot64((l < nAims) && (g_aimK[l < AIMS_LDS ? l : 0] == kmH) && (g_aimN[l < AIMS_LDS ? l : 0] == 0ull));
      if (am != 0ull) aimIdx = (int)__builtin_ctzll(am);
    }
#ifdef TALC_PROF
    if (hitLevel < nOK && aimIdx < 0 && l == 0) g_prof[PF_FSFILT] += 1;
#endif
    nOK = min(nOK, hitLevel);
    const int nTake = nOK + (aimIdx >= 0 ? 1 : 0);
    if (nTake == 0) break;
    if (l < nTake) {
      atomicOr(&g_bloom[bwi], bm);
      if (WIDEF) wide_or(wideW, bmW);
      recN[done - flushed + l] = top;
      seq[len0 + done + l] = (uint8_t)which;
    }
    const int last = nTake - 1;
    kmer = ((uint64_t)(uint32_t)lane_get((int)(uint32_t)(km >> 32), last) << 32) | (uint32_t)lane_get((int)(uint32_t)km, last);
    key = dirRight ? (kmer & m1) : (kmer >> 2);
    hh = (uint32_t)lane_get((int)hv, last);
    havePre = (last == TALC_WALK_LEVELS - 1);
    cnt = (uint32_t)lane_get((int)top, last);
    done += nTake;
    LSYNC();
    PROF_END(PF_FFREC);
    if (aimIdx >= 0) {
      flush();
      WSYNC();
      const int apos = (int)g_aimPos[aimIdx];
      if (dirRight) ranc = apos; else lanc = apos;
      const uint32_t clen = (uint32_t)(len0 + done);
      if (X.nFull >= (int)X.C.fullCap) X.overflow |= OVF_FULLPATHS;
      else if (X.fullUsed + clen > X.C.fullPool) X.overflow |= OVF_FULLPOOL;
      else {
        wave_copy_bytes(X.fullPool + X.fullUsed, (const uint8_t*)seq, clen, false);
        if (l == 0) X.fullMeta[X.nFull] = FullMeta{X.fullUsed, clen, lanc, ranc, dist / ((double)clen + 0.01)};
        X.fullUsed += (clen + 15u) & ~15u;
        X.nFull++;
        WSYNC();
      }
      if (X.overflow) break;
      if (clen > X.refLen) { popped = true; break; }
      continue;
    }
    if (nOK < TALC_WALK_LEVELS) break;
  }
  flush();
  stepCounter_ = sc0 + (uint32_t)done;
#ifdef TALC_PROF
  if (l == 0) { g_prof[PF_NCALLS] += 1; g_prof[PF_NSTEPS] += (uint32_t)done; }
#endif
  if (done) {
    X.steps += (unsigned long long)done;
    if (l == 0) {
      TrailRec r = r0;
      r.kmer = kmer; r.cnt = cnt; r.dist = dist; r.lanc = lanc; r.ranc = ranc;
      tr_put(X.ia, 0, r);
    }
  }
  if (popped) { pool_free((int)r0.buf); X.ffPopped = true; }
  LSYNC();
  return done;
}

TALC_DN int fast_forward_steps(int len, uint32_t& stepCounter, uint32_t PATH_MAXLENGTH, bool edge) {
  return uni((int)X.dirRight) ? fast_forward_dir<true>(len, stepCounter, PATH_MAXLENGTH, edge)
                              : fast_forward_dir<false>(len, stepCounter, PATH_MAXLENGTH, edge);
}
TALC_DNC int fast_forward_wide(int len, uint32_t& stepCounter, uint32_t PATH_MAXLENGTH, bool edge) {
  return uni((int)X.dirRight) ? fast_forward_walk<true, true>(len, stepCounter, PATH_MAXLENGTH, edge)
                              : fast_forward_walk<false, true>(len, stepCounter, PATH_MAXLENGTH, edge);
}
TALC_DN int fast_forward(int len, uint32_t& stepCounter, uint32_t PATH_MAXLENGTH, bool edge) {
  if (uni((int)(X.T.walkRight != nullptr && X.P.MIN_COUNT < kWalkTopNone)) != 0)
  {
    if (uni((int)X.wideMask) != 0) [[clang::musttail]] return fast_forward_wide(len, stepCounter, PATH_MAXLENGTH, edge);
    return uni((int)X.dirRight) ? fast_forward_walk<true, false>(len, stepCounter, PATH_MAXLENGTH, edge)
                                : fast_forward_walk<false, false>(len, stepCounter, PATH_MAXLENGTH, edge);
  }
  [[clang::musttail]] return fast_forward_steps(len, stepCounter, PATH_MAXLENGTH, edge);
}

TALC_DN int fork_step(int len_, uint32_t sc_, uint32_t PMAX_) {
  PROF_DECL;
  PROF_BEGIN();
  const DevParams& P = X.P;
  const int l = lane_id();
  const int len = uni(len_);
  const uint32_t sc = (uint32_t)uni((int)sc_), PMAX = (uint32_t)uni((int)PMAX_);
  if (uni((int)X.traceSteps) != 0) return 0;
  if ((uint32_t)uni((int)P.MAXB) < 2u || (uint32_t)uni((int)P.MAX_INNER_PATHS) < 2u) return 0;
  const TrailRec r0 = tr_get(X.ia, 0);
  if (uni64(r0.nmask) != 0ull) return 0;
  const uint32_t K = (uint32_t)uni((int)P.K), MINC = (uint32_t)uni((int)P.MIN_COUNT), seqCap = (uint32_t)uni((int)X.C.seqCap);
  if (!(sc < PMAX) || (uint32_t)len + 1u > seqCap) return 0;
  const bool dirRight = uni(X.dirRight) != 0;
  const uint64_t kmask = (1ULL << (2 * K)) - 1, m1 = (1ULL << (2 * (K - 1))) - 1;
  const uint64_t kmer = uni64(r0.kmer);
  const uint32_t cnt = (uint32_t)uni((int)r0.cnt);
  auto child_of = [&](uint64_t km, uint32_t b) -> uint64_t {
    return dirRight ? (((km << 2) | (uint64_t)b) & kmask) : (((uint64_t)b << (2 * (K - 1))) | (km >> 2));
  };
  auto get64 = [&](uint64_t v, int src) -> uint64_t {
    return ((uint64_t)(uint32_t)lane_get((int)(uint32_t)(v >> 32), src) << 32) | (uint32_t)lane_get((int)(uint32_t)v, src);
  };
  bool tipInTable;
  const ModelThresholds mtTip = model_thresholds(cnt, tipInTable);
  if (uni((int)tipInTable) == 0) return 0;
  const uint64_t kmMine = (l == 4) ? kmer : child_of(kmer, (uint32_t)(l & 3));
  const uint64_t keyMine = dirRight ? (kmMine & m1) : (kmMine >> 2);
  const Bucket* tab = dirRight ? X.T.right : X.T.left;
  const uint64_t cap = X.T.capacity;
  const uint64_t hMine = table_hash(keyMine);
  uint64_t slotMine = table_slot(hMine, cap);
  BucketRegs br;
  br.key = kEmptyKey; br.cnt[0] = br.cnt[1] = br.cnt[2] = br.cnt[3] = 0u; br.jc01 = br.jc23 = 0u;
  if (l <= 4) br = load_bucket(tab + slotMine);
  bool okTip = false;
  if (l == 4) okTip = probe_bucket_from(tab, cap, keyMine, slotMine, br);
  uint32_t tc[4], tj[4];
  {
    const uint32_t found4 = (uint32_t)lane_get((int)okTip, 4);
#pragma unroll
    for (int i = 0; i < 4; ++i) {
      tc[i] = found4 ? (uint32_t)lane_get((int)br.cnt[i], 4) : 0u;
      tj[i] = found4 ? (uint32_t)lane_get((int)br.jc(i), 4) : 0u;
    }
  }
  int tg[4];
  tag_next_nodes_with(mtTip, P.ERR, MINC, tc, tj, cnt, false, tg, (double*)nullptr);
  int fm = 0;
#pragma unroll
  for (int i = 0; i < 4; ++i) if (tg[i] != TAG_NONE && tg[i] != TAG_UNEXPECTED) fm |= 1 << i;
  fm = uni(fm);
  const int nF = __builtin_popcount((unsigned)fm);
  int taken = 0;
  if (nF == 1 || nF == 2) {
    const bool mine = (l < 4) && (((fm >> l) & 1) != 0);
    const uint32_t hvMine = (uint32_t)(hMine >> 32);
    bool maybe = false;
    if (mine) { uint32_t hq; maybe = bloom_query(kmMine, 0ull, hq); }
    const int iA = __builtin_ctz((unsigned)fm);
    int iS = iA, bC = 0;
    uint32_t cS = 0, cC = 0, hvS = 0, hvC = 0;
    uint64_t kmS = 0, kmC = 0;
    bool ok = ballot64(mine && maybe) == 0ull;
    if (ok && nF == 2) {
      ok = (sc + 1u < PMAX) && ((uint32_t)len + 2u <= seqCap);
      if (ok) {
        bool found = false;
        if (mine) found = probe_bucket_from(tab, cap, keyMine, slotMine, br);
        uint32_t nSucc = 0, which = 0, cSucc = 0;
#pragma unroll
        for (int i = 0; i < 4; ++i) if (found && br.cnt[i] >= MINC) { ++nSucc; which = (uint32_t)i; cSucc = br.cnt[i]; }
        const int iB = __builtin_ctz((unsigned)(fm & (fm - 1)));
        const int nA = lane_get((int)nSucc, iA), nB = lane_get((int)nSucc, iB);
        ok = ((nA == 1) & (nB == 0)) | ((nA == 0) & (nB == 1));
        if (ok) {
          iS = nA ? iA : iB;
          bC = lane_get((int)which, iS);
          cC = (uint32_t)lane_get((int)cSucc, iS);
        }
      }
    }
    if (ok) {
      cS = (iS == 0) ? tc[0] : (iS == 1) ? tc[1] : (iS == 2) ? tc[2] : tc[3];
      kmS = get64(kmMine, iS);
      hvS = (uint32_t)lane_get((int)hvMine, iS);
      if (nF == 2) {
        kmC = child_of(kmS, (uint32_t)bC);
        ok = !bloom_query(kmC, 0ull, hvC);
        hvC = (uint32_t)uni((int)hvC);
      }
    }
    if (ok) {
      const uint32_t wm = (uint32_t)uni((int)X.wideMask);
      gu8 seq = (gu8)uni_ptr(X.seqPool + (uint64_t)r0.buf * X.C.seqCap);
      if (l == 0) {
        TrailRec r = r0;
        seq[len] = (uint8_t)iS;
        r.dist = r0.dist + fabs((double)cnt - (double)cS) / sqrt((double)cnt);
        r.kmer = kmS; r.cnt = cS;
        atomicOr(&g_bloom[hvS >> 25], (1ull << ((hvS >> 19) & 63u)) | (1ull << ((hvS >> 13) & 63u)));
        if (wm != 0u) wide_or(X.wideBloom + wide_word(hvS, wm), wide_bits(hvS));
        if (nF == 2) {
          seq[len + 1] = (uint8_t)bC;
          r.dist = r.dist + fabs((double)cS - (double)cC) / sqrt((double)cS);
          r.kmer = kmC; r.cnt = cC;
          atomicOr(&g_bloom[hvC >> 25], (1ull << ((hvC >> 19) & 63u)) | (1ull << ((hvC >> 13) & 63u)));
          if (wm != 0u) wide_or(X.wideBloom + wide_word(hvC, wm), wide_bits(hvC));
        }
        tr_put(X.ia, 0, r);
      }
      taken = nF;
      X.steps += (nF == 2) ? 3ull : 1ull;
      LSYNC();
    }
  }
#ifdef TALC_PROF
  if (l == 0) g_prof[taken == 1 ? PF_FK1 : taken == 2 ? PF_FK2 : PF_FKBAIL] += 1;
#endif
  PROF_END(PF_FORK);
  return taken;
}

TALC_D void init_first_trail(const AnchorRec& a, const AnchorRec* inList, bool withAims, uint32_t pathMax) {
  const int K = (int)X.P.K;
  uint32_t firstCount;
  {
    const uint32_t h = (uint32_t)uni((int)(X.dirRight ? X.LH : X.RH)), rs0 = (uint32_t)uni((int)(X.dirRight ? X.Ls : X.Rs));
    if ((h & kRegClean) != 0u && a.pos >= rs0) firstCount = (*(const v2u32 TALC_AS1*)((const uint2 TALC_AS1*)X.cov + (h & ~kRegClean) + (a.pos - rs0))).x;
    else firstCount = COVX(a.pos);
  }
  (void)inList;
  pool_reset();
  const uint32_t b0 = (uint32_t)pool_alloc();
  {
    const int l0 = lane_id();
    if (l0 < K) ((gu8)(X.seqPool + (uint64_t)b0 * X.C.seqCap))[l0] = ((gcu8)X.read)[a.pos + (uint32_t)(X.dirRight ? l0 : K - 1 - l0)];
  }
  if (withAims && (uint32_t)uni((int)X.rowAvail) != 0u) row_set_covered(b0, 0u);
  uint32_t wm = 0;
  if (pathMax > (uint32_t)WIDE_BLOOM_MIN_PATH && X.wideBloom != nullptr && X.T.walkRight != nullptr && X.P.MIN_COUNT < kWalkTopNone) {
    uint32_t words = 1024;
    while (words < (uint32_t)WIDE_BLOOM_WORDS && words < pathMax / 2) words <<= 1;
    wm = words - 1;
    for (uint32_t i = (uint32_t)lane_id(); i < words; i += 64) X.wideBloom[i] = 0ull;
    WSYNC();
  }
  X.wideMask = (uint32_t)uni((int)wm);
  if (lane_id() == 0) g_keep.owner = 0u;
  g_bloom[lane_id()] = 0ull; g_bloom[lane_id() + 64] = 0ull;
  LSYNC();
// ... 95 lines not shown
    if (!pool_shape(PATH_MAXLENGTH)) return false;
    rows_shape();
    PROF_BEGIN2(); init_first_trail(a, anchors + s, true, PATH_MAXLENGTH); PROF_END2(PF_INITTR);
    int nCur = 1;
    int len = (int)K;
    const uint32_t maxInner = (uint32_t)uni((int)P.MAX_INNER_PATHS);
    while ((int)(nCur > 0) & (int)((uint32_t)nCur <= maxInner) & (int)((uint32_t)uni((int)stepCounter) < PATH_MAXLENGTH) & (int)(uni((int)X.overflow) == 0)) {
      if (nCur == 1) {
        PROF_BEGIN2(); len += uni(fast_forward(len, stepCounter, PATH_MAXLENGTH, false)); PROF_END2(PF_FFWD);
        if (X.ffPopped) { X.ffPopped = false; nCur = 0; break; }
        if (!(stepCounter < PATH_MAXLENGTH)) break;
        const int fs = uni(fork_step(len, stepCounter, PATH_MAXLENGTH));
        if (fs > 0) { len += fs; stepCounter += (uint32_t)fs; continue; }
      }
      PROF_BEGIN2();
      nCur = uni(step_bridge(nCur, len, stepCounter));
      PROF_END2(PF_STEPB);
      ++len;
      if (uni((int)(X.traceSteps))) trace_rec(TR_STEP, (int)stepCounter, nCur, X.nFull, 0, 0.0, nullptr, 0, false);
    }
#ifdef TALC_PROF
    if (l == 0) {
      const uint32_t dt = (uint32_t)(__builtin_amdgcn_s_memrealtime() - _pf_b0);
      g_prof[PF_RBR] += 1; if (dt > g_prof[PF_RBRMAX]) g_prof[PF_RBRMAX] = dt;
    }
#endif
    if (X.overflow) return false;
    if (X.nFull > 0) {
      int nOK = 0;
      const uint32_t limit2 = X.Re;
      PROF_BEGIN();
      FullMeta lone = FullMeta();
      uint32_t loneFlags = 0;
      unsigned long long loneIdBits = 0;
      for (int t = 0; t < X.nFull; ++t) {
        const FullMeta fm = X.fullMeta[t];
        const uint8_t* ps = X.fullPool + fm.off;
        double score, idv;
        int es, lcs;
        int accept = 0;
        bool needed = true;
        if (X.nFull == 1 && P.MIN_INNER > 0.0) {
          const double mxl = (double)max(X.refLen, fm.len);
          int T = (int)ceil(P.MIN_INNER * mxl);
          while (T > 1 && (double)(T - 1) / mxl >= P.MIN_INNER) --T;
          while ((double)T / mxl < P.MIN_INNER) ++T;
          accept = T;
          uint32_t cutLen1 = 0; bool ok1 = true;
          if (fm.len >= 2 * K) cutLen1 = fm.len - 2 * K;
          else if (fm.len > K) ok1 = ((uint32_t)fm.ranc + 2 * K - fm.len <= limit2);
          else ok1 = false;
          const uint32_t bestLen1 = ok1 ? cutLen1 : 0u;
          const double diff1 = (double)X.weakLen - (double)bestLen1;
          needed = ok1 && ((diff1 < X.weakLen * 0.05) || ((X.weakLen < 6) & (bestLen1 < 6)));
        }
        es = 0; lcs = 0;
        if (uni((int)needed)) {
          int quick = -1;
          if (X.nFull == 1 && accept > 0) quick = uni(lcs_reaches(X.ref, (int)X.refLen, ps, (int)fm.len, accept));
          if (quick >= 0) lcs = quick;
          else edit_and_lcs(X.ref, (int)X.refLen, ps, (int)fm.len, es, lcs, X.nFull > 1, accept);
        }
        score = (double)es;
        idv = (double)lcs / (double)max(X.refLen, fm.len);
        bool ok = true;
        uint32_t cutLen = 0;
        uint32_t ranc = (uint32_t)fm.ranc;
        if (fm.len >= 2 * K) cutLen = fm.len - 2 * K;
        else if ((fm.len < 2 * K) & (fm.len > K)) {
          if (ranc + 2 * K - fm.len <= limit2) ranc = ranc + 2 * K - fm.len;
          else ok = false;
        } else ok = false;
        if (X.nFull == 1) {
          lone = fm; lone.ranc = (int32_t)ranc;
          loneFlags = (ok ? 1u : 0u) | (cutLen << 1);
          loneIdBits = uni64((unsigned long long)__double_as_longlong(idv));
        } else if (l == 0) {
          X.gScores[t] = score; X.gDists[t] = idv; X.gKept[t] = (ok ? 1u : 0u) | (cutLen << 1);
          X.fullMeta[t].ranc = (int32_t)ranc;
        }
        nOK += ok ? 1 : 0;
      }
      if (X.nFull > 1) WSYNC();
      PROF_END(PF_EVALFULL);
      const int nCand = (nOK == X.nFull) ? X.nFull : nOK;
      PROF_BEGIN();
      if (nCand > 0) {
        FullMeta bm;
        uint32_t flags;
        double bestId;
        if (X.nFull == 1) {
          bm.off = (uint32_t)uni((int)lone.off); bm.len = (uint32_t)uni((int)lone.len); bm.lanc = uni(lone.lanc); bm.ranc = uni(lone.ranc); bm.dist = 0.0;
          flags = (uint32_t)uni((int)loneFlags);
          bestId = __longlong_as_double((long long)loneIdBits);
        } else {
          const int index = uni(find_best_bridge(nCand));
          bm = X.fullMeta[index];
          flags = X.gKept[index];
          bestId = X.gDists[index];
        }
        const uint32_t bestLen = (flags & 1u) ? (flags >> 1) : 0u;
        const double diff = (double)X.weakLen - (double)bestLen;
        if (((diff < X.weakLen * 0.05) || ((X.weakLen < 6) & (bestLen < 6))) & (bestId >= P.MIN_INNER)) {
          X.Le = (uint32_t)bm.lanc;
          X.Rs = (uint32_t)bm.ranc;
          if (weakUsed + bestLen > X.C.weakPool) { X.overflow |= OVF_WEAKPOOL; return false; }
          if (bestLen) copy_bytes(X.weak + weakUsed, X.fullPool + bm.off + K, bestLen, !X.dirRight);
          weakOutOff = weakUsed; weakOutLen = bestLen;
          weakUsed += bestLen;
          WSYNC();
          found = true;
        }
      }
      PROF_END(PF_RESULT);
    }
  }
  return found;
}

TALC_D void edge_anchor_search(const AnchorRec* anchors_, int s_) {
  PROF_DECL2;
#ifdef TALC_PROF
  const unsigned long long _pf_a0 = __builtin_amdgcn_s_memrealtime();
#endif
  const DevParams& P = X.P;
  const AnchorRec* anchors = uni_ptr(anchors_);
  const int s = uni(s_);
  const uint32_t K = (uint32_t)uni((int)P.K);
  const uint32_t readLen = (uint32_t)uni((int)X.L), maxInner = (uint32_t)uni((int)P.MAX_INNER_PATHS), CHECK = (uint32_t)uni((int)P.CHECK_INTERVAL);
  const AnchorRec a = uni_anchor(anchors + s);
  const uint32_t whichStart = a.pos;
  uint32_t stepCounter = 0;
  int xdrop = (int)((double)(int)P.CHECK_INTERVAL * P.FAILURE_RATE + 1.0);
  uint32_t gapLen;
  X.refLen = 0;
  X.ref = X.refBuf;
  if (X.dirRight) {
    gapLen = readLen - (whichStart + K);
    X.ref = const_cast<uint8_t*>(X.read) + whichStart;
    X.refLen = readLen - whichStart;
  } else {
    gapLen = whichStart;
    ref_append(whichStart, whichStart + K);
    ref_append(0, whichStart);
  }
  WSYNC();
  const uint32_t PATH_MAXLENGTH = (uint32_t)(int)(1.2 * (double)gapLen + (double)(2 * K));
  if (!pool_shape(PATH_MAXLENGTH)) return;
  PROF_BEGIN2(); init_first_trail(a, anchors + s, false, PATH_MAXLENGTH); PROF_END2(PF_INITTR);
  int nCur = 1;
  int len = (int)K;
  while ((int)(nCur > 0) & (int)((uint32_t)nCur <= maxInner) & (int)((uint32_t)uni((int)stepCounter) < PATH_MAXLENGTH) & (int)(uni((int)X.overflow) == 0)) {
    if (nCur == 1) {
      PROF_BEGIN2();
      const int ff = uni(fast_forward(len, stepCounter, PATH_MAXLENGTH, true));
      len += ff;
      PROF_END2(PF_FFWD);
      if (ff > 0 && ((uint32_t)uni((int)stepCounter) % CHECK == 0)) {
        PROF_BEGIN2();
        nCur = uni(score_edges(X.ia, 1, len, xdrop));
        PROF_END2(PF_STEPE);
        continue;
      }
      if (!((uint32_t)uni((int)stepCounter) < PATH_MAXLENGTH)) break;
    }
    PROF_BEGIN2();
    nCur = uni(step_edge(nCur, len, stepCounter, PATH_MAXLENGTH, xdrop));
    PROF_END2(PF_STEPE);
    ++len;
    if (uni((int)(X.traceSteps)))
      trace_rec(TR_STEP, (int)stepCounter, nCur, X.nEdges, xdrop, 0.0, nullptr, 0, false);
  }
#ifdef TALC_PROF
  if (lane_id() == 0) {
    const unsigned long long dt = __builtin_amdgcn_s_memrealtime() - _pf_a0;
    const int bk = dt < 100000ull ? 0 : dt < 400000ull ? 1 : dt < 1600000ull ? 2 : dt < 6400000ull ? 3 : 4;
    g_prof[PF_EA0 + bk] += 1;
    if (bk == 3) g_prof[PF_EASUM3] += (uint32_t)dt;
    if (bk == 4) g_prof[PF_EASUM4] += (uint32_t)dt;
    g_prof[PF_RANCH] += 1; if ((uint32_t)dt > g_prof[PF_RANCHMAX]) g_prof[PF_RANCHMAX] = (uint32_t)dt;
  }
#endif
}

TALC_DN void edge_anchor_search_task(const AnchorRec* anchors, int s) { edge_anchor_search(anchors, s); }

#define EDGE_BOX_ANCHORS 8
struct EdgeBoxHdr {
  const uint8_t* read; const uint2* cov; const CovWord* covw; double lambda;
  uint32_t L, n, location, dirRight, Ls, Le, Rs, Re, LH, RH, weakLen, limit;
  uint32_t done, first, pad[2];
  AnchorRec anc[EDGE_BOX_ANCHORS];
};
struct EdgeBoxRes { EdgeCand best[2]; uint32_t complex, overflow, redo, pad; };
static_assert(sizeof(EdgeCand) == 48 && sizeof(EdgeBoxRes) == 112 && sizeof(AnchorRec) == 24, "edge box records are moved as dwords");
static_assert(offsetof(EdgeBoxHdr, anc) == 96 && sizeof(EdgeBoxHdr) == 96 + 24 * EDGE_BOX_ANCHORS, "edge box header layout");
static const uint32_t kBoxResOff = 320, kBoxResStride = 128, kBoxSeqOff = kBoxResOff + EDGE_BOX_ANCHORS * kBoxResStride;
__host__ __device__ inline uint64_t edge_box_bytes(uint32_t seqCap) { return (kBoxSeqOff + 2ull * EDGE_BOX_ANCHORS * seqCap + 255ull) / 256ull * 256ull; }

struct EdgeTaskArgs {
  uint8_t* boxes; uint32_t* avail;
  uint32_t seqCap;
  uint32_t minWeak;
  uint32_t heavy, heavyRounds;
  uint32_t lingerMod;
  uint32_t test;
  const uint32_t* autoSwitch;
};
TALC_D uint32_t aload32(const uint32_t* p) { return __hip_atomic_load(p, __ATOMIC_RELAXED, __HIP_MEMORY_SCOPE_AGENT); }
TALC_D void astore32(uint32_t* p, uint32_t v) { __hip_atomic_store(p, v, __ATOMIC_RELAXED, __HIP_MEMORY_SCOPE_AGENT); }
TALC_D uint32_t aadd32(uint32_t* p, uint32_t v) { return __hip_atomic_fetch_add(p, v, __ATOMIC_RELAXED, __HIP_MEMORY_SCOPE_AGENT); }
TALC_D uint32_t axchg32(uint32_t* p, uint32_t v) { return __hip_atomic_exchange(p, v, __ATOMIC_RELAXED, __HIP_MEMORY_SCOPE_AGENT); }
TALC_D void agent_fence() { __builtin_amdgcn_fence(__ATOMIC_SEQ_CST, "agent"); }
TALC_D uint8_t* edge_box(uint32_t slot) { return X.boxes + (uint64_t)slot * X.boxBytes; }
TALC_D uint32_t* edge_box_seq(uint8_t* box, int s, int bi) { return (uint32_t*)(box + kBoxSeqOff + (uint64_t)(2 * s + bi) * X.boxSeqCap); }

TALC_DNC void edge_box_store(uint8_t* box_, int s_, uint32_t complexFlag_) {
  uint8_t* box = uni_ptr(box_); const int s = uni(s_);
  const int l = lane_id();
  LSYNC();
  EdgeBoxRes* st = (EdgeBoxRes*)g_dp;
  const uint32_t cap = (uint32_t)uni((int)X.boxSeqCap);
  const bool tooLong = (X.best2[0].have && X.best2[0].len > cap) || (X.best2[1].have && X.best2[1].len > cap);
  if (l == 0) {
    st->best[0] = X.best2[0]; st->best[1] = X.best2[1];
    st->complex = uni((int)complexFlag_); st->overflow = X.overflow; st->redo = (X.nanSeen != 0u || tooLong) ? 1u : 0u; st->pad = 0;
  }
  LSYNC();
  uint32_t* dst = (uint32_t*)(box + kBoxResOff + (uint32_t)s * kBoxResStride);
  if (l < (int)(sizeof(EdgeBoxRes) / 4)) astore32(dst + l, (uint32_t)g_dp[l]);
  if (!tooLong) {
    for (int bi = 0; bi < 2; ++bi) {
      if (!X.best2[bi].have) continue;
      const uint32_t nw = (X.best2[bi].len + 3u) >> 2;
      const uint32_t* src = (const uint32_t*)uni_ptr(bi == 0 ? X.edgeLong : X.edgeShort);
      uint32_t* q = uni_ptr(edge_box_seq(box, s, bi));
      for (uint32_t i = (uint32_t)l; i < nw; i += 64) astore32(q + i, src[i]);
    }
  }
  LSYNC();
}
TALC_D void edge_box_load(uint8_t* box, int s) {
  const int l = lane_id();
  LSYNC();
  const uint32_t* src = (const uint32_t*)(box + kBoxResOff + (uint32_t)s * kBoxResStride);
  if (l < (int)(sizeof(EdgeBoxRes) / 4)) g_dp[l] = (int)aload32(src + l);
  LSYNC();
}
TALC_D void edge_box_take(uint8_t* box, int s, int bi, uint32_t len) {
  uint32_t* dst = (uint32_t*)uni_ptr(bi == 0 ? X.edgeLong : X.edgeShort);
  const uint32_t* q = uni_ptr(edge_box_seq(box, s, bi));
  const uint32_t nw = (len + 3u) >> 2;
  for (uint32_t i = (uint32_t)lane_id(); i < nw; i += 64) dst[i] = aload32(q + i);
}
TALC_D void edge_box_fold(uint8_t* box, int first, int limit) {
  EdgeCand best0, best1; best0.have = false; best1.have = false;
  int win0 = -1, win1 = -1;
  for (int s = first; s < limit; ++s) {
    edge_box_load(box, s);
    const EdgeBoxRes* r = (const EdgeBoxRes*)g_dp;
    const EdgeCand c0 = r->best[0], c1 = r->best[1];
    if (c0.have && (!best0.have || c0.score > best0.score || (c0.score == best0.score && c0.dist > best0.dist))) { best0 = c0; win0 = s; }
    if (c1.have && (!best1.have || c1.score > best1.score || (c1.score == best1.score && c1.dist > best1.dist))) { best1 = c1; win1 = s; }
  }
  LSYNC();
  X.best2[0] = best0; X.best2[1] = best1;
  if (uni(win0) >= 0) edge_box_take(box, uni(win0), 0, best0.len);
  if (uni(win1) >= 0) edge_box_take(box, uni(win1), 1, best1.len);
  WSYNC();
}

TALC_D bool queue_is_dry() {
  uint32_t v = 0;
  if (lane_id() == 0) v = aload32(X.qwords);
  return (uint32_t)uni((int)v) >= X.nWork;
}

TALC_D int edge_ctx_load(uint8_t* box) {
  const int l = lane_id();
  const uint32_t* box32 = (const uint32_t*)box;
  LSYNC();
  if (l < 24) g_dp[l] = (int)aload32(box32 + l);
  LSYNC();
  const EdgeBoxHdr* h = (const EdgeBoxHdr*)g_dp;
  const int limit = uni((int)h->limit);
  X.read = h->read; X.cov = h->cov; X.covw = h->covw; X.lambda = h->lambda; X.L = h->L; X.n = h->n;
  X.location = (int)h->location; X.dirRight = (int)h->dirRight;
  X.Ls = h->Ls; X.Le = h->Le; X.Rs = h->Rs; X.Re = h->Re; X.LH = h->LH; X.RH = h->RH; X.weakLen = h->weakLen;
  X.ffPopped = false; X.tracing = false; X.traceSteps = false;
  X.nAncL = X.dirRight ? limit : 0; X.nAncR = X.dirRight ? 0 : limit;
  LSYNC();
  return limit;
}

TALC_DNC bool edge_task_steal(int tries);

TALC_DNC int edge_anchors_as_tasks(const AnchorRec* anchors_, int s0_, int limit_) {
  const AnchorRec* anchors = uni_ptr(anchors_);
  const int s0 = uni(s0_), limit = uni(limit_);
  const int l = lane_id();
  const uint32_t me = (uint32_t)uni((int)X.mySlot);
  uint8_t* box = uni_ptr(edge_box(me));
  uint32_t* box32 = (uint32_t*)box;
  uint32_t* done = box32 + offsetof(EdgeBoxHdr, done) / 4;
  const int first = s0 > 0 ? s0 - 1 : s0;
  if (s0 > 0) {
    const uint32_t cap = (uint32_t)uni((int)X.boxSeqCap);
    if ((X.best2[0].have && X.best2[0].len > cap) || (X.best2[1].have && X.best2[1].len > cap)) return 0;
    edge_box_store(box, s0 - 1, 0u);
  }
  LSYNC();
  {
    EdgeBoxHdr* h = (EdgeBoxHdr*)g_dp;
    if (l == 0) {
      h->read = X.read; h->cov = X.cov; h->covw = X.covw; h->lambda = X.lambda;
      h->L = X.L; h->n = X.n; h->location = (uint32_t)X.location; h->dirRight = (uint32_t)X.dirRight;
      h->Ls = X.Ls; h->Le = X.Le; h->Rs = X.Rs; h->Re = X.Re; h->LH = X.LH; h->RH = X.RH; h->weakLen = X.weakLen; h->limit = (uint32_t)limit;
      h->done = 0; h->first = (uint32_t)s0; h->pad[0] = 0; h->pad[1] = 0;
    }
    LSYNC();
    if (l < 24) astore32(box32 + l, (uint32_t)g_dp[l]);
    for (int i = l; i < 6 * limit; i += 64) astore32(box32 + 24 + i, ((const uint32_t*)anchors)[i]);
    LSYNC();
  }
  agent_fence();
  const uint32_t nTasks = (uint32_t)(limit - s0);
  if (l == 0) { aadd32(X.qwords + kQueueOpen, nTasks); (void)axchg32(X.avail + me, nTasks); }
  PROF_COUNT(PF_TPUB, 1);
  uint32_t nMine = 0;
  while (true) {
    int old = 0;
    if (l == 0) old = (int)aadd32(X.avail + me, 0xFFFFFFFFu);
    old = uni(old);
    if (old <= 0) break;
    if (l == 0) (void)aadd32(X.qwords + kQueueOpen, 0xFFFFFFFFu);
    ++nMine;
    PROF_COUNT(PF_TOWN, 1);
    const int s = limit - old;
    X.best2[0].have = false; X.best2[1].have = false; X.nanSeen = 0u;
    edge_anchor_search_task(anchors, s);
    edge_box_store(box, s, 0u);
    if (uni((int)X.overflow)) break;
  }
  int rest = 0;
  if (l == 0) { rest = (int)axchg32(X.avail + me, 0u); if (rest < 0) rest = 0; if (rest > 0) (void)aadd32(X.qwords + kQueueOpen, (uint32_t)(-rest)); }
  rest = uni(rest);
  const uint32_t expected = nTasks - (uint32_t)rest - nMine;
  PROF_COUNT(PF_TSTOLEN, expected);
  {
    PROF_DECL; PROF_BEGIN();
    if (l == 0) { while (aload32(done) < expected) __builtin_amdgcn_s_sleep(32); }
    WSYNC();
    PROF_END(PF_TWAIT);
  }
  agent_fence();
  if (uni((int)X.overflow)) return 0;
  uint32_t ovf = 0, redo = 0, cx = 0;
  for (int s = s0; s < limit; ++s) {
    edge_box_load(box, s);
    const EdgeBoxRes* r = (const EdgeBoxRes*)g_dp;
    ovf |= r->overflow; redo |= r->redo; cx |= r->complex;
  }
  LSYNC();
  if (uni((int)ovf)) { X.overflow |= (uint32_t)uni((int)ovf); return 0; }
  if (uni((int)redo)) {
    edge_box_fold(box, first, s0);
    return 0;
  }
  if (uni((int)cx)) X.complexRegion = true;
  edge_box_fold(box, first, limit);
  return 1;
}

TALC_DNC void edge_task_run(uint32_t victim_, int old_) {
  PROF_DECL2;
  PROF_BEGIN2();
  const int l = lane_id();
  const int old = uni(old_);
  agent_fence();
  uint8_t* box = uni_ptr(edge_box((uint32_t)uni((int)victim_)));
  uint32_t* box32 = (uint32_t*)box;
  const int limit = edge_ctx_load(box), s = limit - old;
  X.headCov = nullptr;
  X.cells = 0; X.steps = 0; X.overflow = 0; X.complexRegion = false;
  X.nanSeen = 0u; X.nEdges = 0;
  AnchorRec* mine = uni_ptr(X.dirRight ? X.ancL : X.ancR);
  if (s >= 0 && s < limit && limit <= EDGE_BOX_ANCHORS) {
    if (l < 6) ((uint32_t*)(mine + s))[l] = aload32(box32 + 24 + 6 * s + l);
    WSYNC();
    X.best2[0].have = false; X.best2[1].have = false;
    edge_anchor_search_task(mine, s);
    if (X.taskTest) X.nanSeen = 1u;
    edge_box_store(box, s, X.complexRegion ? 1u : 0u);
  }
  agent_fence();
  if (l == 0) (void)aadd32(box32 + offsetof(EdgeBoxHdr, done) / 4, 1u);
  PROF_END2(PF_TRUN);
}

TALC_DNC bool edge_task_steal(int tries_) {
  const int l = lane_id();
  const int tries = uni(tries_);
  const uint32_t nS = (uint32_t)uni((int)X.nSlots), me = (uint32_t)uni((int)X.mySlot);
  {
    int open = 0;
    if (l == 0) open = (int)aload32(X.qwords + kQueueOpen);
    if (uni(open) <= 0) return false;
  }
  const uint32_t nWin = (nS + 63u) >> 6;
  for (int k = 0; k < tries; ++k) {
    X.stealSeq += 1u;
    const uint32_t win = (me * 2654435761u + X.stealSeq * 40503u) % nWin;
    const uint32_t i = win * 64u + (uint32_t)l;
    const int v = (i < nS && i != me) ? (int)aload32(X.avail + i) : 0;
    unsigned long long m = ballot64(v > 0);
    while (m != 0ull) {
      const int src = (int)__builtin_ctzll(m);
      m &= m - 1ull;
      const uint32_t victim = (uint32_t)__shfl((int)i, src);
      int old = 0;
      if (l == 0) old = (int)aadd32(X.avail + victim, 0xFFFFFFFFu);
      old = uni(old);
      if (old > 0) {
        if (l == 0) (void)aadd32(X.qwords + kQueueOpen, 0xFFFFFFFFu);
        edge_task_run(victim, old);
        return true;
      }
    }
  }
  return false;
}

TALC_DNC void edge_between_reads() {
  if (!X.holding) { X.holding = 1u; return; }
  if (lane_id() == 0) (void)aadd32(X.qwords + kQueueFinished, 1u);
  while (edge_task_steal(1)) { X.moreCells += X.cells; X.moreSteps += X.steps; }
}
TALC_DNC unsigned long long edge_linger(uint32_t n_work_) {
  const uint32_t n_work = (uint32_t)uni((int)n_work_);
  const int l = lane_id();
  unsigned long long idle = 0;
  while (true) {
    WSYNC();
    if (edge_task_steal(8)) { X.moreCells += X.cells; X.moreSteps += X.steps; continue; }
    uint32_t fin = 0;
    if (l == 0) fin = aload32(X.qwords + kQueueFinished);
    if ((uint32_t)uni((int)fin) >= n_work) break;
    const unsigned long long t0 = __builtin_amdgcn_s_memrealtime();
    for (int i = 0; i < 4; ++i) __builtin_amdgcn_s_sleep(127);
    idle += __builtin_amdgcn_s_memrealtime() - t0;
  }
  return idle;
}

TALC_DN bool search_edge(uint32_t& weakOutOff, uint32_t& weakOutLen, uint32_t& weakUsed) {
  const DevParams& P = X.P;
  const AnchorRec* anchors = uni_ptr(X.dirRight ? X.ancL : X.ancR);
  const int nAnch = uni(X.dirRight ? X.nAncL : X.nAncR);
  const int limit = min(nAnch, uni((int)P.MAX_START_ANCHORS));
  X.best2[0].have = false; X.best2[1].have = false; X.nEdges = 0; X.nanSeen = 0u;
  bool mayPublish = (X.boxes != nullptr) && limit <= EDGE_BOX_ANCHORS && !X.tracing && X.weakLen >= X.taskMinWeak;
  for (int s = 0; s < limit; ++s) {
    if (uni((int)mayPublish) && limit - s >= 2 && ((X.weakLen >= X.taskHeavy && X.qi < X.heavyUpTo) || queue_is_dry())) {
      const int folded = uni(edge_anchors_as_tasks(anchors, s, limit));
      if (X.overflow) return false;
      if (folded) break;
      mayPublish = false;
    }
    edge_anchor_search(anchors, s);
    if (X.overflow) return false;
  }
  bool found = false;
  if (X.best2[1].have || X.best2[0].have) {
    const int wi = X.best2[0].have ? 0 : 1;
    const EdgeCand w = X.best2[wi];
    const uint8_t* wseq = (wi == 0) ? X.edgeLong : X.edgeShort;
    const double diff = (double)X.weakLen - (double)w.len;
    double minScore;
    if ((X.weakLen >= 300) || X.complexRegion) minScore = fmax(0.75, P.MIN_BORDER);
    else minScore = P.MIN_BORDER;
    if (((diff < X.weakLen * 0.05) || ((X.weakLen < 6) & (w.len < 6))) & (w.idscore >= minScore)) {
      found = true;
      if (weakUsed + w.len > X.C.weakPool) { X.overflow |= OVF_WEAKPOOL; return false; }
      if (w.len) copy_bytes(X.weak + weakUsed, wseq, w.len, !X.dirRight);
      weakOutOff = weakUsed; weakOutLen = w.len;
      weakUsed += w.len;
      if (X.location == LOC_TAIL) X.Le = w.lanc; else X.Rs = w.ranc;
      WSYNC();
    }
  }
  return found;
}

TALC_DNC void trace_search_cold() {
  if (!X.tracing) return;
  const int locRef = X.location == LOC_HEAD ? 0 : X.location == LOC_INNER ? 1 : 2;
  const int nL = (X.location == LOC_HEAD) ? 0 : X.nAncL, nR = (X.location == LOC_TAIL) ? 0 : X.nAncR;
  trace_rec(TR_SEARCH, locRef, X.dirRight, nL, nR, 0.0, nullptr, 0, false);
  const int K = (int)X.P.K;
  for (int i = 0; i < nL; ++i) trace_rec(TR_ANCHOR, 0, (int)X.ancL[i].pos, (int)X.ancL[i].count, 0, 0.0, X.read + X.ancL[i].pos, K, false);
  for (int i = 0; i < nR; ++i) trace_rec(TR_ANCHOR, 1, (int)X.ancR[i].pos, (int)X.ancR[i].count, 0, 0.0, X.read + X.ancR[i].pos, K, false);
}

#ifndef TALC_SEARCH_WAVES_PER_SIMD
#define TALC_SEARCH_WAVES_PER_SIMD 5
#endif
__global__ void __launch_bounds__(64, TALC_SEARCH_WAVES_PER_SIMD)
k_search(DevParams P, TableView T, SearchCaps C, const uint8_t* __restrict__ codes, const uint64_t* __restrict__ offsets,
         const uint64_t* __restrict__ koff, const uint2* __restrict__ covAll, const CovWord* __restrict__ covWords,
         ReadState* __restrict__ state,
         const uint32_t* __restrict__ regions, const uint64_t* __restrict__ regoff, const uint32_t* __restrict__ headCovAll,
         uint8_t* __restrict__ outAll,
         const uint64_t* __restrict__ outoff, const uint32_t* __restrict__ order, uint32_t n_work,
         uint32_t* __restrict__ queue, uint8_t* __restrict__ scratchAll, uint64_t* __restrict__ counters, TraceBuf trace,
         uint32_t traceRead, uint32_t launchStamp, EdgeTaskArgs E) {
  __shared__ uint32_t s_next;
  const int l = lane_id();
  uint8_t* slot = scratchAll + (uint64_t)blockIdx.x * C.slotBytes;
  X.P = P; X.T = T; X.C = (const SearchLimits&)C;
  X.G[0] = make_set(slot + C.o_setA);
  X.G[1] = make_set(slot + C.o_setB);
  X.ia = 0;
  X.seqPool = slot + C.o_seqPool;
  X.refBuf = slot + C.o_ref; X.ref = X.refBuf; X.ancL = (AnchorRec*)(slot + C.o_ancL); X.ancR = (AnchorRec*)(slot + C.o_ancR);
  X.ancPos = (uint32_t*)(slot + C.o_ancPos);
  X.fullMeta = (FullMeta*)(slot + C.o_fullMeta); X.fullPool = slot + C.o_fullPoolB;
  X.edgeLong = slot + C.o_edgeLong; X.edgeShort = slot + C.o_edgeShort; X.edgeTmp = slot + C.o_edgeTmp;
  X.dpG = (int*)(slot + C.o_dp);
  X.wideBloom = (unsigned long long*)(slot + C.o_wideBloom); X.wideMask = 0;
  X.rowPool = (int*)(slot + C.o_rowPool); X.rowStride = 0; X.rowAvail = 0;
  X.launchStamp = launchStamp;
  if (E.boxes != nullptr && E.autoSwitch != nullptr && *E.autoSwitch == 0u) E.boxes = nullptr;
  X.boxes = E.boxes; X.avail = E.avail; X.qwords = queue; X.boxSeqCap = E.seqCap; X.boxBytes = (uint32_t)edge_box_bytes(E.seqCap);
  X.nSlots = gridDim.x; X.mySlot = blockIdx.x; X.nWork = n_work; X.taskMinWeak = E.minWeak; X.nanSeen = 0u; X.taskTest = E.test;
  X.taskHeavy = E.heavy; X.heavyUpTo = (E.heavyRounds >= 0xFFFFu) ? 0xFFFFFFFFu : E.heavyRounds * gridDim.x;
  X.qi = 0; X.holding = 0u; X.stealSeq = 0u; X.moreCells = 0; X.moreSteps = 0;
  const uint32_t lingerMod = max(E.lingerMod, 1u);
  X.searchNo = 16u;
  {
    uint8_t* g = slot + C.o_gard;
    X.gScores = (double*)g; g += 8ull * (TCAP + 64);
    X.gDists = (double*)g; g += 8ull * (TCAP + 64);
    X.gVal = (ValIdx*)g; g += 16ull * (TCAP + 64);
    X.gRank = (Rank4*)g; g += 32ull * (TCAP + 64);
    X.gKept = (uint32_t*)g;
// ... 403 lines not shown
```

talc_amd/csrc/talc_switches.h:

```cpp
#pragma once
#include <algorithm>
#include <cstdint>
#include <cstdlib>
#include <string>

namespace talc {

struct Switches {
  int timing = 0;
  bool hostParse = false;
  int walk = -1;
  uint32_t filterBits = 20;
  uint32_t tableSlotsX10 = 0;
  uint32_t searchSlots = 0;
  uint32_t seqArena = 0;
  bool tinyCaps = false;
  bool failRetryAlloc = false;
  int edgeTasks = -1;
  uint32_t edgeTaskMin = 150, edgeTaskHeavy = 200, edgeTaskRounds = 0xFFFF, edgeLingerMod = 16;
  bool edgeRedo = false;
  bool traceSteps = false;
  uint32_t fakeGpus = 0;
  std::string profReads;
  bool profPrint = false, profSlow = false;
};

inline Switches read_switches() {
  auto given = [](const char* name) { return std::getenv(name) != nullptr; };
  auto num = [](const char* name, long unset) { const char* e = std::getenv(name); return e ? std::atol(e) : unset; };
  auto clamped = [&](const char* name, long unset, long lo, long hi) { return (uint32_t)std::min(std::max(num(name, unset), lo), hi); };
  Switches s;
  if (const char* e = std::getenv("TALC_TIMING")) s.timing = e[0] == '2' ? 2 : 1;
  s.hostParse = given("TALC_HOST_PARSE");
  if (given("TALC_WALK")) s.walk = num("TALC_WALK", 0) != 0 ? 1 : 0;
  if (const char* e = std::getenv("TALC_FILTER_BITS")) s.filterBits = (uint32_t)std::min<uint64_t>(64, std::max<uint64_t>(4, std::strtoull(e, nullptr, 10)));
  if (const char* e = std::getenv("TALC_TABLE_SLOTS_X10")) { const uint64_t v = std::strtoull(e, nullptr, 10); if (v >= 20 && v <= 80) s.tableSlotsX10 = (uint32_t)v; }
  s.searchSlots = clamped("TALC_SEARCH_SLOTS", 0, 0, 1L << 30);
  s.seqArena = clamped("TALC_SEQ_ARENA", 0, 0, 1L << 30);
  s.tinyCaps = num("TALC_TEST_TINY_CAPS", 0) > 0;
  s.failRetryAlloc = given("TALC_TEST_FAIL_RETRY_ALLOC");
  if (given("TALC_EDGE_TASKS")) { const long v = num("TALC_EDGE_TASKS", 0); s.edgeTasks = v == 0 ? 0 : v > 0 ? 1 : -1; }
  s.edgeTaskMin = clamped("TALC_EDGE_TASK_MIN", 150, 0, 1L << 30);
  s.edgeTaskHeavy = clamped("TALC_EDGE_TASK_HEAVY", 200, 0, 1L << 30);
  s.edgeTaskRounds = clamped("TALC_EDGE_TASK_ROUNDS", 0xFFFF, 0, 0xFFFF);
  s.edgeLingerMod = clamped("TALC_EDGE_LINGER_MOD", 16, 1, 1L << 20);
  s.edgeRedo = given("TALC_TEST_EDGE_REDO");
  s.traceSteps = num("TALC_TRACE_STEPS", 0) != 0;
  s.fakeGpus = clamped("TALC_FAKE_GPUS", 0, 0, 1L << 20);
  if (const char* e = std::getenv("TALC_PROF_READS")) s.profReads = e;
  s.profPrint = given("TALC_PROF_PRINT");
  s.profSlow = given("TALC_PROF_SLOW");
  return s;
}

}
```

talc_amd/csrc/talc_wave.h:

```cpp
#pragma once
#include <limits.h>

#include "talc_common.h"

namespace talc {

#define WSYNC() __syncthreads()

TALC_D int lane_id() { return (int)__builtin_amdgcn_mbcnt_hi(~0u, __builtin_amdgcn_mbcnt_lo(~0u, 0u)); }
TALC_D int lane_id_here() { int l = lane_id(); asm volatile("" : "+v"(l)); return l; }
#define TALC_WAVE_REDUCE(v, OP, IDENT)                                                                   \
  do {                                                                                                   \
    v = OP(v, __builtin_amdgcn_update_dpp(IDENT, v, 0x111, 0xF, 0xF, false));                            \
    v = OP(v, __builtin_amdgcn_update_dpp(IDENT, v, 0x112, 0xF, 0xF, false));                            \
    v = OP(v, __builtin_amdgcn_update_dpp(IDENT, v, 0x114, 0xF, 0xF, false));                            \
    v = OP(v, __builtin_amdgcn_update_dpp(IDENT, v, 0x118, 0xF, 0xF, false));                            \
    v = OP(v, __builtin_amdgcn_update_dpp(IDENT, v, 0x142, 0xA, 0xF, false));                            \
    v = OP(v, __builtin_amdgcn_update_dpp(IDENT, v, 0x143, 0xC, 0xF, false));                            \
  } while (0)
TALC_D int wave_max_i32(int v) {
  TALC_WAVE_REDUCE(v, max, INT_MIN);
  return __builtin_amdgcn_readlane(v, 63);
}
TALC_D int talc_or_i32(int a, int b) { return a | b; }
// ... 410 lines not shown
  return min(wfa_first_diff_raw(x, y) >> 3, 8u);
}
template <int NR>
TALC_D void wfa_extend(const uint8_t TALC_AS3* stage, int qpad, int kmin, int (&a)[NR], bool (&act)[NR]) {
  const int l = lane_id();
  if constexpr (NR == 1) {
    const int k = kmin + l;
    unsigned qa = (unsigned)((a[0] + k) >> 1), da = qa + (unsigned)(qpad - k), t = 0u;
    if (act[0]) {
      t = wfa_first_diff_raw(lds_load_u64(stage + qa), lds_load_u64(stage + da));
      a[0] += 2 * (int)min(t >> 3, 8u); qa += 8; da += 8;
    }
    while (ballot64(t > 63u) != 0ull) {
      const bool go = t > 63u;
      t = 0u;
      if (go) {
        const unsigned long long q0 = lds_load_u64(stage + qa), d0 = lds_load_u64(stage + da);
        const unsigned long long q1 = lds_load_u64(stage + qa + 8), d1 = lds_load_u64(stage + da + 8);
        const unsigned t0 = wfa_first_diff_raw(q0, d0), t1 = wfa_first_diff_raw(q1, d1);
        const unsigned n = (t0 > 63u) ? 8u + min(t1 >> 3, 8u) : (t0 >> 3);
        a[0] += 2 * (int)n; qa += 16; da += 16;
        t = min(t0, t1);
      }
    }
    act[0] = false;
  } else {
    unsigned qa[NR], da[NR];
    bool any = false;
#pragma unroll
    for (int s = 0; s < NR; ++s) {
      const int k = kmin + 64 * s + l;
      qa[s] = (unsigned)((a[s] + k) >> 1); da[s] = (unsigned)(qpad + ((a[s] - k) >> 1));
      if (act[s]) {
        const unsigned n = wfa_equal_prefix8(lds_load_u64(stage + qa[s]), lds_load_u64(stage + da[s]));
        a[s] += 2 * (int)n; qa[s] += 8; da[s] += 8;
        act[s] = (n == 8u);
      }
      any |= act[s];
    }
    while (ballot64(any) != 0ull) {
      any = false;
#pragma unroll
      for (int s = 0; s < NR; ++s) {
        if (act[s]) {
          const unsigned long long q0 = lds_load_u64(stage + qa[s]), d0 = lds_load_u64(stage + da[s]);
          const unsigned long long q1 = lds_load_u64(stage + qa[s] + 8), d1 = lds_load_u64(stage + da[s] + 8);
          const unsigned n0 = wfa_equal_prefix8(q0, d0), n1 = wfa_equal_prefix8(q1, d1);
          const unsigned n = (n0 == 8u) ? 8u + n1 : n0;
          a[s] += 2 * (int)n; qa[s] += 16; da[s] += 16;
          act[s] = (n == 16u);
          any |= act[s];
        }
      }
    }
  }
}

template <int NR>
TALC_D int wfa_select(const int (&F)[NR], const int (&E)[NR], int kmin, int kmax, int qlen, int dlen,
                      int& extCols, int& extRows, int& extScore) {
  const int l = lane_id();
  const int NEG = -(1 << 29);
  int mF = NEG;
#pragma unroll
  for (int s = 0; s < NR; ++s) mF = max(mF, F[s]);
  const int A = wave_max_i32(mF);
  const int cols = qlen + 1, rows = dlen + 1;
  auto minmaxS = [&](int a, bool dropTopBorder, int& mn, int& mx) {
    int lmn = INT_MAX, lmx = INT_MIN;
#pragma unroll
    for (int s = 0; s < NR; ++s) {
      const int k = kmin + 64 * s + l;
      const int c = (a + k) >> 1;
      const bool on = (((k - a) & 1) == 0) & (F[s] >= a) & !(dropTopBorder & (c == a));
      if (on) { lmn = min(lmn, c); lmx = max(lmx, c); }
    }
    mn = wave_min_i32(lmn); mx = wave_max_i32(lmx);
  };
  auto at = [&](const int (&r)[NR], int k) -> int {
    const int j = k - kmin, slot = j >> 6;
    int v = r[0];
#pragma unroll
    for (int s = 0; s < NR; ++s) if (s == slot) v = r[s];
    return lane_get(v, j & 63);
  };
  auto kept = [&](int a, int c) -> bool {
    const int k = 2 * c - a;
    if (c < 0 || a - c < 0 || k < kmin || k > kmax) return false;
    return at(F, k) >= a;
  };
  auto take = [&](int a, int c) { extCols = c; extRows = a - c; extScore = -at(E, 2 * c - a); };
  auto firstMax = [&](int a) -> int {
    int key = INT_MAX;
#pragma unroll
    for (int s = 0; s < NR; ++s) {
      const int j = 64 * s + l, k = kmin + j;
      if ((((k - a) & 1) == 0) & (F[s] == a)) key = min(key, (E[s] << 10) | j);
    }
    const int kk = wave_min_i32(key);
    if (kk == INT_MAX) return 0;
    const int k = kmin + (kk & 1023);
    extCols = (a + k) >> 1; extRows = (a - k) >> 1; extScore = -(kk >> 10);
    return 1;
  };
  bool early = false;
  if (A + 1 >= 2) {
    int mn, mx;
    minmaxS(A, false, mn, mx);
    const int lo = max(1 + mn, A + 3 - rows), hi = min(2 + mx, cols);
    early = lo >= hi;
  }
  if (!early) return firstMax(A);
  int maxColA = 1;
  if (A >= 2) {
    int mn1, mx1, mn2, mx2;
    minmaxS(A - 1, true, mn1, mx1);
    minmaxS(A - 2, false, mn2, mx2);
    const int cm = max(mx1, mx2);
    maxColA = (cm == INT_MIN) ? cols : min(2 + cm, cols);
  }
  const int c2 = maxColA - 1;
  if (kept(A, c2)) { take(A, c2); return 1; }
  if (A >= 2 && kept(A, c2 - 1)) { take(A, c2 - 1); return 1; }
  return firstMax(A - 1);
}

TALC_D void stage_copy(uint8_t TALC_AS3* dst, gcu8 src, int n) {
  const int l = lane_id_here();
  typedef uint64_t __attribute__((aligned(1))) u64u;
  const int nw = n >> 3;
  for (int w = l; w < nw; w += 64) ((uint64_t TALC_AS3*)dst)[w] = *(const u64u TALC_AS1*)(src + 8 * w);
  const int t = (nw << 3) + l;
  if (t < n) dst[t] = src[t];
}

struct WfaPhase {
  int fromLevel;
  int toLevel;
  int* memF; int* memE;
};

#ifdef TALC_PROF
__shared__ uint32_t g_wprof[4];
#define WPROF_T() __builtin_amdgcn_s_memtime()
#define WPROF_ADD(i, t0) (g_wprof[i] += (uint32_t)(__builtin_amdgcn_s_memtime() - (t0)))
#else
#define WPROF_T() 0ull
#define WPROF_ADD(i, t0) ((void)(t0))
#endif

struct WfaKeep { uint32_t owner; int level; int qlenAt; int pad_; uint16_t F[64]; uint8_t E[64]; };
__shared__ WfaKeep g_keep;

template <int NR>
TALC_D int wave_xdrop_wfa(const uint8_t* __restrict__ querySeg_, int qlen, const uint8_t* __restrict__ dbSeg_, int dlen, int x,
                          uint8_t TALC_AS3* stage, int stageCap, int& extCols, int& extRows, int& extScore,
                          unsigned long long& cells, const WfaPhase* ph = nullptr, uint32_t keepKey_ = 0) {
  gcu8 querySeg = (gcu8)uni_ptr(querySeg_); gcu8 dbSeg = (gcu8)uni_ptr(dbSeg_);
  const int l = lane_id();
  qlen = uni(qlen); dlen = uni(dlen); x = uni(x);
  extCols = extRows = extScore = 0;
  if (qlen <= 0 || dlen <= 0) return 0;
  const int NEG = -(1 << 29);
  const int X = min(max(x, 0), 1 << 20);
  const int fromLevel = ph ? ph->fromLevel : -1, toLevel = ph ? ph->toLevel : -1;
  const int Xm = (toLevel >= 0) ? min(X, toLevel) : X;
  const int kmin = -min(Xm, dlen), kmax = min(Xm, qlen);
  const int nd = kmax - kmin + 1;
  if (nd > 64 * NR - 1) return -1;
  const int qS = min(qlen, dlen + X), dS = min(dlen, qlen + X);
  const int qpad = (qS + 16) & ~7;
  if (qpad + dS + 16 > stageCap) return -1;
  const unsigned long long _t0 = WPROF_T();
  if (fromLevel < 0) {
    stage_copy(stage, querySeg, qS);
    stage_copy(stage + qpad, dbSeg, dS);
    if (l == 0) { stage[qS] = 0xF0; stage[qpad + dS] = 0xF1; }
  }
  WSYNC();
  WPROF_ADD(0, _t0);
  const unsigned long long _t1 = WPROF_T();
  const int bmax = x >= 2 ? x - 1 : (x == 1 ? 1 : 0);
  const int corner = qlen + dlen;
  int F[NR], E[NR], amax[NR], forb[NR];
#pragma unroll
  for (int s = 0; s < NR; ++s) {
    const int j = 64 * s + l, k = kmin + j, ak = k < 0 ? -k : k;
    amax[s] = (j < nd) ? min(2 * qlen - k, 2 * dlen + k) : NEG;
    forb[s] = (ak == bmax + 1) ? ak : -1;
    F[s] = NEG; E[s] = 0;
  }
  auto extend = [&](int (&a)[NR], bool (&act)[NR]) { wfa_extend<NR>(stage, qpad, kmin, a, act); };
  bool cornerHit = false;
  int cornerE = 0;
  int eStart = 1;
  const uint32_t keepKey = (NR == 1 && fromLevel < 0) ? (uint32_t)uni((int)keepKey_) : 0u;
  bool tracking = keepKey != 0u;
  const int kOfLane = kmin + l;
  const int aq = 2 * qlen - kOfLane;
  bool resumed = false;
  if (NR == 1 && keepKey != 0u) {
    const int lv = uni(g_keep.level), qat = uni(g_keep.qlenAt);
    if ((uint32_t)uni((int)g_keep.owner) == keepKey && lv >= 1 && lv < x && lv <= 31 && lv < qat && qat <= qlen && lv < dlen) {
      const int ak = kOfLane < 0 ? -kOfLane : kOfLane;
      const bool in = (l < nd) & (ak <= lv);
      const uint32_t f16 = g_keep.F[(kOfLane + 32) & 63];
      F[0] = (in && f16 != 0xFFFFu) ? (int)f16 : NEG;
      E[0] = in ? (int)g_keep.E[(kOfLane + 32) & 63] : 0;
      eStart = lv + 1;
      resumed = true;
    }
  }
  auto keep_level = [&](int level) {
    if (level >= 1 && level <= 31) {
      if (l < nd) { g_keep.F[(kOfLane + 32) & 63] = (uint16_t)(F[0] >= 0 ? F[0] : 0xFFFF); g_keep.E[(kOfLane + 32) & 63] = (uint8_t)E[0]; }
      if (l == 0) { g_keep.owner = keepKey; g_keep.level = level; g_keep.qlenAt = qlen; }
    }
  };
  if (resumed) {
  } else
  if (fromLevel >= 0) {
#pragma unroll
    for (int s = 0; s < NR; ++s) {
      const int j = 64 * s + l, k = kmin + j, ak = k < 0 ? -k : k;
      const bool in = (j < nd) & (ak <= fromLevel);
      F[s] = in ? ph->memF[in ? k + 256 : 256] : NEG;
      E[s] = in ? ph->memE[in ? k + 256 : 256] : 0;
    }
    eStart = fromLevel + 1;
  } else {
    int a0[NR]; bool act0[NR];
    const int j0 = -kmin;
#pragma unroll
    for (int s = 0; s < NR; ++s) { a0[s] = 0; act0[s] = (64 * s + l == j0) && x >= 0; }
    extend(a0, act0);
#pragma unroll
    for (int s = 0; s < NR; ++s) if (64 * s + l == j0) F[s] = a0[s];
    unsigned long long hit = 0;
#pragma unroll
    for (int s = 0; s < NR; ++s) hit |= ballot64(F[s] == corner);
    cornerHit = hit != 0ull;
    if (tracking && ballot64(F[0] == aq) != 0ull) tracking = false;
  }
  const int eEnd = (toLevel >= 0) ? min(x, toLevel) : x;
  unsigned long long work = 0;
  const int kc = qlen - dlen;
  const bool cornerInBand = (kc >= kmin) & (kc <= kmax);
  int eLast = eStart - 1;
  for (int e = eStart; e <= eEnd && !cornerHit; ++e) {
    if (NR == 1 && tracking && e == x) { keep_level(e - 1); tracking = false; }
    const bool forbLevel = (e == bmax + 1);
    int rotR[NR], rotL[NR];
#pragma unroll
    for (int s = 0; s < NR; ++s) { rotR[s] = lane_ror1(F[s]); rotL[s] = lane_rol1(F[s]); }
    const int sLo = max(0, -e - kmin) >> 6, sHi = min(nd - 1, e - kmin) >> 6;
    int b[NR]; bool act[NR];
#pragma unroll
    for (int s = 0; s < NR; ++s) {
      b[s] = NEG; act[s] = false;
      if (NR == 1 || (s >= sLo && s <= sHi)) {
        const int fl = (NR > 1 && l == 0) ? rotR[(s + NR - 1) % NR] : rotR[s];
        const int fr = (NR > 1 && l == 63) ? rotL[(s + 1) % NR] : rotL[s];
        int v2 = fl + 1; v2 = (v2 <= amax[s]) ? v2 : NEG;
        int v3 = fr + 1; v3 = (v3 <= amax[s]) ? v3 : NEG;
        int v = max(max(v2, v3), min(F[s] + 2, amax[s]));
        if (forbLevel) v = (v == forb[s]) ? NEG : v;
        b[s] = v;
        act[s] = (v > F[s]) & (v >= 0);
      }
    }
    bool moved[NR];
#pragma unroll
    for (int s = 0; s < NR; ++s) moved[s] = act[s];
    extend(b, act);
    if (NR == 1 && tracking && ballot64(b[0] == aq) != 0ull) {
      keep_level(e - 1);
      tracking = false;
    }
    unsigned long long hit = 0;
#pragma unroll
    for (int s = 0; s < NR; ++s) {
      if (moved[s]) { F[s] = b[s]; E[s] = e; }
      if (cornerInBand) hit |= ballot64(F[s] == corner);
    }
    if (hit != 0ull) { cornerHit = true; cornerE = e; }
    eLast = e;
  }
  if (NR == 1 && tracking && !cornerHit && eLast < x) keep_level(eLast);
  if (eLast >= eStart) {
    const int eh = min(eLast, (nd - 1) / 2);
    const int lo = max(eh, eStart - 1);
    if (eh >= eStart) work += (unsigned long long)((eh - eStart + 1) * (eh + eStart + 1));
    if (eLast > lo) work += (unsigned long long)((eLast - lo) * nd);
  }
  cells += work;
  WPROF_ADD(1, _t1);
#ifdef TALC_PROF
  if (eLast >= eStart) g_wprof[3] += (uint32_t)(eLast - eStart + 1);
#endif
  const unsigned long long _t2 = WPROF_T();
  if (cornerHit) { extCols = qlen; extRows = dlen; extScore = -cornerE; return 1; }
  if (toLevel >= 0 && toLevel < x) {
#pragma unroll
    for (int s = 0; s < NR; ++s) {
      const int j = 64 * s + l, k = kmin + j, ak = k < 0 ? -k : k;
      if ((j < nd) & (ak <= toLevel)) { ph->memF[k + 256] = F[s]; ph->memE[k + 256] = E[s]; }
    }
    WSYNC();
    return 2;
  }
  const int rsel = wfa_select<NR>(F, E, kmin, kmax, qlen, dlen, extCols, extRows, extScore);
  WPROF_ADD(2, _t2);
  return rsel;
}

template <int NR>
TALC_D int wave_xdrop_wfa_multi(const uint8_t* __restrict__ querySeg_, int qlen, const uint8_t* __restrict__ dbSeg_, int dlen, int xHi,
                                uint8_t TALC_AS3* stage, int stageCap, int* resCols, int* resRows, int* resScore,
                                unsigned long long& cells) {
  gcu8 querySeg = (gcu8)uni_ptr(querySeg_); gcu8 dbSeg = (gcu8)uni_ptr(dbSeg_);
  const int l = lane_id();
  qlen = uni(qlen); dlen = uni(dlen); xHi = uni(xHi);
  if (qlen <= 0 || dlen <= 0 || xHi < 0) return -1;
  const int NEG = -(1 << 29);
  const int X = min(xHi, 1 << 20);
  const int kmin = -min(X, dlen), kmax = min(X, qlen);
  const int nd = kmax - kmin + 1;
  if (nd > 64 * NR - 1) return -1;
  const int qS = min(qlen, dlen + X), dS = min(dlen, qlen + X);
  const int qpad = (qS + 16) & ~7;
  if (qpad + dS + 16 > stageCap) return -1;
  stage_copy(stage, querySeg, qS);
// ... 327 lines not shown
```

talc_amd/csrc/talc_wfa.h:

```cpp
#pragma once
#include <climits>
#include <cstdint>
#include <vector>

namespace talc {

struct WfaResult { int moved; int extCols; int extRows; int score; };

inline WfaResult wfa_xdrop_scalar(const uint8_t* q, int qlen, const uint8_t* d, int dlen, int x) {
  WfaResult res = {0, 0, 0, 0};
  if (qlen == 0 || dlen == 0) return res;
  const int NEG = -(1 << 29);
  const int bmax = x >= 2 ? x - 1 : (x == 1 ? 1 : 0);
  const int X = x < 0 ? 0 : x;
  const int kmin = -(X < dlen ? X : dlen), kmax = (X < qlen ? X : qlen);
  const int nd = kmax - kmin + 1;
  std::vector<int> F(nd + 2, NEG), G(nd + 2, NEG), E(nd + 2, 0), amin(nd + 2), amax(nd + 2);
  auto idx = [&](int k) { return k - kmin + 1; };
  for (int k = kmin; k <= kmax; ++k) {
    const int ak = k < 0 ? -k : k;
    amin[idx(k)] = ak + (ak > bmax ? 2 : 0);
    const int a1 = 2 * qlen - k, a2 = 2 * dlen + k;
    amax[idx(k)] = a1 < a2 ? a1 : a2;
  }
  auto extend = [&](int a, int k) {
    int c = (a + k) / 2, r = (a - k) / 2;
    while (c < qlen && r < dlen && q[c] == d[r]) { ++c; ++r; }
    return c + r;
  };
  const int corner = qlen + dlen, kc = qlen - dlen;
  F[idx(0)] = x >= 0 ? extend(0, 0) : 0;
  bool cornerHit = (kc >= kmin && kc <= kmax && F[idx(kc)] == corner);
  int cornerE = 0;
  for (int e = 1; e <= x && !cornerHit; ++e) {
    for (int k = kmin; k <= kmax; ++k) {
      const int i = idx(k);
      const int fm = F[i], fl = F[i - 1], fr = F[i + 1];
      int best = NEG;
      const int v[3] = {fm + 2, fl + 1, fr + 1};
      for (int t = 0; t < 3; ++t)
        if (v[t] >= amin[i] && v[t] <= amax[i] && v[t] > best) best = v[t];
      int nv = fm;
      if (best > fm) { nv = extend(best, k); E[i] = e; }
      G[i] = nv;
    }
    F.swap(G);
    if (kc >= kmin && kc <= kmax && F[idx(kc)] == corner) { cornerHit = true; cornerE = e; }
  }
  if (cornerHit) { res.moved = 1; res.extCols = qlen; res.extRows = dlen; res.score = -cornerE; return res; }
  int A = 0;
  for (int k = kmin; k <= kmax; ++k) if (F[idx(k)] > A) A = F[idx(k)];
  const int cols = qlen + 1, rows = dlen + 1;
  auto minmaxS = [&](int a, bool dropTopBorder, int& mn, int& mx) {
    mn = INT_MAX; mx = INT_MIN;
    if (a < 0) return;
    for (int k = kmin; k <= kmax; ++k) {
      if (((k - a) & 1) || F[idx(k)] < a) continue;
      const int c = (a + k) / 2;
      if (dropTopBorder && c == a) continue;
      if (c < mn) mn = c;
      if (c > mx) mx = c;
    }
  };
  auto kept = [&](int a, int c) {
    const int k = 2 * c - a;
    return c >= 0 && a - c >= 0 && k >= kmin && k <= kmax && F[idx(k)] >= a;
  };
  auto firstMax = [&](int a) {
    int bestE = INT_MAX, bestK = 0;
    for (int k = kmin; k <= kmax; ++k) {
      if (((k - a) & 1) || F[idx(k)] != a) continue;
      if (E[idx(k)] < bestE) { bestE = E[idx(k)]; bestK = k; }
    }
    if (bestE == INT_MAX) return;
    res.moved = 1; res.extCols = (a + bestK) / 2; res.extRows = (a - bestK) / 2; res.score = -bestE;
  };
  bool early = false;
  if (A + 1 >= 2) {
    int mn, mx; minmaxS(A, false, mn, mx);
    const int a = A + 1;
    const int lo = (1 + mn > a + 2 - rows) ? 1 + mn : a + 2 - rows;
    const int hi = (2 + mx < cols) ? 2 + mx : cols;
    early = lo >= hi;
  }
  if (!early) { firstMax(A); return res; }
  int maxColA;
  if (A >= 2) {
    int mn1, mx1, mn2, mx2;
    minmaxS(A - 1, true, mn1, mx1); minmaxS(A - 2, false, mn2, mx2);
    const int cm = mx1 > mx2 ? mx1 : mx2;
    maxColA = (2 + cm < cols) ? 2 + cm : cols;
  } else {
    maxColA = 1;
  }
  const int c2 = maxColA - 1;
  auto take = [&](int a, int c) {
    const int k = 2 * c - a;
    res.moved = 1; res.extCols = c; res.extRows = a - c; res.score = -E[idx(k)];
  };
  if (kept(A, c2)) { take(A, c2); return res; }
  if (A >= 2 && kept(A, c2 - 1)) { take(A, c2 - 1); return res; }
  firstMax(A - 1);
  return res;
}

}
```

Baseline: 4.648 billion.

## Add fused edge lane that walks and scores single-path edges with resumable WFA

Introduces an edge_lane path for single-trail edge extension that combines the fast-forward k-mer walk with x-drop seed extension. The walk body is refactored into reusable walk_record/walk_flush helpers, and the WFA gains a prestaged mode plus resumable kept-level state so repeated x-drop checks can continue instead of restarting. The aim is to cut repeated re-staging and re-alignment work at each check interval. It brings a sizeable new control path, enabled by default, with correctness risk in resume conditions and extra state to maintain.

```diff
diff --git a/talc_amd/csrc/pure_capi.cpp b/talc_amd/csrc/pure_capi.cpp
--- a/talc_amd/csrc/pure_capi.cpp
+++ b/talc_amd/csrc/pure_capi.cpp
@@ -72,4 +72,12 @@
   const WfaResult r = wfa_xdrop_scalar(q, qlen, d, dlen, x);
   out4[0] = r.moved; out4[1] = r.extCols; out4[2] = r.extRows; out4[3] = r.score;
 }
+
+int pure_wfa_xdrop_resume(const uint8_t* q, int qlen, const uint8_t* d, int dlen, int x, int32_t* keep130, int32_t* out4) {
+  static_assert(sizeof(WfaKept) == 130 * sizeof(int32_t), "WfaKept is 130 ints");
+  bool resumed = false;
+  const WfaResult r = wfa_xdrop_scalar_run(q, qlen, d, dlen, x, reinterpret_cast<WfaKept*>(keep130), &resumed);
+  out4[0] = r.moved; out4[1] = r.extCols; out4[2] = r.extRows; out4[3] = r.score;
+  return resumed ? 1 : 0;
 }
+}
diff --git a/talc_amd/csrc/talc_capi_correct.inc b/talc_amd/csrc/talc_capi_correct.inc
--- a/talc_amd/csrc/talc_capi_correct.inc
+++ b/talc_amd/csrc/talc_capi_correct.inc
@@ -143,12 +143,13 @@
     if ((rc = ensure_stage(c, c->stage, b->max_len, 1, b->n_reads))) return rc;
     ensure_edge_boxes(c, c->stage);
     EdgeTaskArgs ea = {};
+    ea.test = c->sw.edgeLane ? 0u : kTestNoEdgeLane;
     if (c->stage.boxes) {
       ea.boxes = c->stage.boxes.get();
       ea.avail = (uint32_t*)(c->stage.boxes.get() + (uint64_t)c->stage.n_slots * edge_box_bytes(c->stage.box_seq_cap));
       ea.seqCap = c->stage.box_seq_cap;
       ea.minWeak = c->sw.edgeTaskMin; ea.heavy = c->sw.edgeTaskHeavy; ea.heavyRounds = c->sw.edgeTaskRounds;
-      ea.lingerMod = c->sw.edgeLingerMod; ea.test = c->sw.edgeRedo ? 1u : 0u;
+      ea.lingerMod = c->sw.edgeLingerMod; ea.test |= c->sw.edgeRedo ? kTestEdgeRedo : 0u;
       ea.autoSwitch = c->sw.edgeTasks > 0 ? nullptr : c->d_hist.get() + 1024 + 129;
       HIPCHK(hipMemsetAsync(ea.avail, 0, (uint64_t)c->stage.n_slots * 4, s));
     }
@@ -179,9 +180,11 @@
       HIPCHK(hipMemcpyAsync(b->d_state.get() + r, &b->h_state[r], sizeof(ReadState), hipMemcpyHostToDevice, s));
     }
     HIPCHK(hipMemsetAsync(c->d_queue.get(), 0, kQueueWords * sizeof(uint32_t), s));
+    EdgeTaskArgs rea = {};
+    rea.test = c->sw.edgeLane ? 0u : kTestNoEdgeLane;
     hipLaunchKernelGGL(k_search, dim3(big.n_slots), dim3(64), 0, s, c->dp, c->view, big.caps, b->d_codes.get(), b->d_offsets.get(), b->d_koff.get(),
                        b->d_cov.get(), b->d_covw.get(), b->d_state.get(), b->d_regions.get(), b->d_regoff.get(), b->d_headcov.get(), b->d_out.get(), b->d_outoff.get(), d_retry.get(), (uint32_t)retry.size(),
-                       c->d_queue.get(), big.scratch.get(), c->d_counters.get(), tb, traceRead, next_launch_stamp(), EdgeTaskArgs());
+                       c->d_queue.get(), big.scratch.get(), c->d_counters.get(), tb, traceRead, next_launch_stamp(), rea);
     HIPCHK(hipGetLastError());
     HIPCHK(hipMemcpyAsync(b->h_state.data(), b->d_state.get(), b->n_reads * sizeof(ReadState), hipMemcpyDeviceToHost, s));
     HIPCHK(hipStreamSynchronize(s));
diff --git a/talc_amd/csrc/talc_kernels_search.h b/talc_amd/csrc/talc_kernels_search.h
--- a/talc_amd/csrc/talc_kernels_search.h
+++ b/talc_amd/csrc/talc_kernels_search.h
@@ -560,7 +560,7 @@
        PF_EDGEMISC, PF_ANCHORS, PF_ASSEMBLE, PF_STEPB, PF_STEPE, PF_SRCHB, PF_SRCHE, PF_PROLOG, PF_INITTR, PF_TOTAL, PF_NCALLS, PF_NSTEPS,
        PF_FFLOAD, PF_FFREC, PF_FFFLUSH, PF_FFENTRY, PF_NRECS, PF_RD0, PF_RD1, PF_RD2, PF_RD3, PF_RD4, PF_RD5, PF_RDMAX,
        PF_XSTAGE, PF_XLEV, PF_XSEL, PF_REFB, PF_RESULT, PF_CYQ, PF_CYX, PF_CYHIT, PF_CYFILL,
-       PF_SB11, PF_SB12, PF_SB21, PF_SB10, PF_SBOTHER, PF_SEGEN, PF_XCALLS, PF_XNLEV, PF_FSFORK, PF_FSDEAD, PF_FSFILT, PF_FSLIM, PF_FK1, PF_FK2, PF_FKBAIL, PF_FORK, PF_ANCCALLS, PF_ANCITER, PF_TPUB, PF_TOWN, PF_TSTOLEN, PF_TWAIT, PF_TRUN, PF_EA0, PF_EA1, PF_EA2, PF_EA3, PF_EA4, PF_EASUM3, PF_EASUM4, PF_RANCH, PF_RANCHMAX, PF_RBR, PF_RBRMAX, PF_N };
+       PF_SB11, PF_SB12, PF_SB21, PF_SB10, PF_SBOTHER, PF_SEGEN, PF_XCALLS, PF_XNLEV, PF_FSFORK, PF_FSDEAD, PF_FSFILT, PF_FSLIM, PF_FK1, PF_FK2, PF_FKBAIL, PF_FORK, PF_ANCCALLS, PF_ANCITER, PF_TPUB, PF_TOWN, PF_TSTOLEN, PF_TWAIT, PF_TRUN, PF_EA0, PF_EA1, PF_EA2, PF_EA3, PF_EA4, PF_EASUM3, PF_EASUM4, PF_RANCH, PF_RANCHMAX, PF_RBR, PF_RBRMAX, PF_EDGELANE, PF_N };
 #define TALC_PF_NAMES {"probe", "child", "aims", "cycle", "ffwd", "scorebr", "garden", "evalfull", "xdrop", "extnw", "edgemisc", \
                        "anchors", "assemble", "stepb*", "stepe*", "srchb*", "srche*", "prolog", "inittr", "total", "#ffcalls", "#ffsteps", \
                        "ff.load", "ff.record", "ff.flush", "ff.entry", "#ffrecords", "#reads<0.25ms", "#reads<1ms", "#reads<4ms", \
@@ -569,7 +569,9 @@
                        "#stepb 1->1", "#stepb 1->2", "#stepb 2->1", "#stepb 1->0", "#stepb other", "#stepe generic", "#xdrop calls", "#xdrop levels", \
                        "#ffstop fork", "#ffstop deadend", "#ffstop filter", "#ffstop limit/other", "#forkstep 1 child", "#forkstep fork+deadend", "#forkstep bailed", "forkstep", "#anchor lists", "#anchor level tests", \
                        "#edges published", "#anchors by owner", "#anchors by others", "t.owner waits", "t.run by others", \
-                       "#edge anchors<1ms", "#edge anchors<4ms", "#edge anchors<16ms", "#edge anchors<64ms", "#edge anchors>=64ms", "ticks anchors 16-64ms", "ticks anchors>=64ms", "(per read) anchors", "(per read) longest anchor", "(per read) bridge attempts", "(per read) longest bridge attempt"}
+                       "#edge anchors<1ms", "#edge anchors<4ms", "#edge anchors<16ms", "#edge anchors<64ms", "#edge anchors>=64ms", "ticks anchors 16-64ms", "ticks anchors>=64ms", "(per read) anchors", "(per read) longest anchor", "(per read) bridge attempts", "(per read) longest bridge attempt", "edgelane*"}
+
+enum : uint32_t { kTestEdgeRedo = 1u, kTestNoEdgeLane = 2u };
 
 struct Wv {
   DevParams P; TableView T; SearchLimits C;
@@ -1333,11 +1335,13 @@
   return rc >= 0;
 }
 
-TALC_D bool trail_seed_and_extend(int set_, int t_, int len_, int xdrop_) {
+TALC_D bool trail_seed_and_extend(int set_, int t_, int len_, int xdrop_, bool leafFell = false) {
   const int set = uni(set_), t = uni(t_), len = uni(len_), xdrop = uni(xdrop_);
   WSYNC();
   const uint32_t buf = (uint32_t)uni((int)tr_buf(set, t));
-  SeedExt e = seed_and_extension_leaf(X.ref, (int)X.refLen, X.seqPool + (uint64_t)buf * X.C.seqCap, len, xdrop, buf + 1u);
+  SeedExt e;
+  e.fallback = true;
+  if (!leafFell) e = seed_and_extension_leaf(X.ref, (int)X.refLen, X.seqPool + (uint64_t)buf * X.C.seqCap, len, xdrop, buf + 1u);
   if (uni((int)e.fallback) != 0) e = seed_and_extension(X.ref, (int)X.refLen, X.seqPool + (uint64_t)buf * X.C.seqCap, len, xdrop, true);
   const int lenHistExt = uni(e.lenHistExt), score = uni(e.score), posOnRef = uni(e.posOnRef);
   const bool stop = uni((int)e.stop) != 0;
@@ -1939,13 +1943,13 @@
 }
 
 TALC_DNC int score_edges_multi(int ib_, int n_, int len_, int& xdrop_);
-TALC_D int score_edges(int ib_, int n_, int len_, int& xdrop_) {
+TALC_D int score_edges(int ib_, int n_, int len_, int& xdrop_, bool leafFell = false) {
   const int n = uni(n_), len = uni(len_);
   if (n == 0) return 0;
   const int ib = uni(ib_);
   const int xdrop = uni(xdrop_) + 2;
   if (n == 1) {
-    const bool ok = uni((int)trail_seed_and_extend(ib, 0, len, xdrop)) != 0;
+    const bool ok = uni((int)trail_seed_and_extend(ib, 0, len, xdrop, leafFell)) != 0;
     xdrop_ = ok ? (int)((double)uni(tr_get(ib, 0).score) * (-1)) : 0;
     if (!ok) { record_edge(ib, 0, len); pool_free((uint32_t)uni((int)tr_buf(ib, 0))); return 0; }
     return 1;
@@ -2187,70 +2191,19 @@
   return (uint32_t)__builtin_amdgcn_update_dpp((int)old, (int)v, 0x110 + P, 0xF, 0xF, false);
 }
 
-template <bool dirRight, bool WIDEF>
-TALC_D int fast_forward_walk(int len_, uint32_t& stepCounter_, uint32_t PATH_MAXLENGTH_, bool edge_) {
-  PROF_DECL; PROF_DECL2;
-  PROF_BEGIN2();
-  const DevParams& P = X.P;
+struct WalkLanes { uint32_t laneOff, laneShift, laneSingle; int lj; };
+struct WalkTip { uint64_t kmer, key; uint32_t hh, cnt; uint32_t ePre; bool havePre; int done, flushed; };
+template <bool dirRight, bool WIDEF, class Also>
+TALC_D int walk_record(const WalkLanes& WL, WalkTip& W, int room, const uint32_t TALC_AS1* wtab, uint64_t cap, uint32_t K, gu8 seq, int len0,
+                       uint32_t* recN, int nAims, uint32_t wideMask, unsigned long long* wideBloom, int& nOK, int& aimIdx, Also also) {
+  PROF_DECL;
   const int l = lane_id();
-  const bool edge = uni((int)edge_) != 0;
-  if (uni((int)(X.traceSteps)) != 0) return 0;
-  const TrailRec r0 = tr_get(X.ia, 0);
-  if (uni64(r0.nmask) != 0ull) return 0;
-  const uint32_t K = (uint32_t)uni((int)P.K), CHECK = (uint32_t)uni((int)P.CHECK_INTERVAL);
-  const uint32_t seqCap = (uint32_t)uni((int)X.C.seqCap), PMAX = (uint32_t)uni((int)PATH_MAXLENGTH_);
-  const uint64_t cap = uni64(X.T.capacity);
-  const uint32_t TALC_AS1* wtab = (const uint32_t TALC_AS1*)uni_ptr(dirRight ? X.T.walkRight : X.T.walkLeft);
-  const uint32_t wideMask = WIDEF ? (uint32_t)uni((int)X.wideMask) : 0u;
-  unsigned long long* const wideBloom = WIDEF ? (unsigned long long*)uni_ptr(X.wideBloom) : nullptr;
   const uint64_t kmask = (1ULL << (2 * K)) - 1, m1 = (1ULL << (2 * (K - 1))) - 1;
-  uint64_t kmer = uni64(r0.kmer);
-  uint32_t cnt = (uint32_t)uni((int)r0.cnt);
-  const int len0 = uni(len_);
-  const uint32_t sc0 = (uint32_t)uni((int)stepCounter_);
-  int maxSteps = 0;
-  if (sc0 < PMAX && (uint32_t)len0 < seqCap) {
-    maxSteps = (int)min(PMAX - sc0, seqCap - (uint32_t)len0);
-    if (edge) maxSteps = min(maxSteps, (int)(CHECK - (sc0 % CHECK)));
-  }
-  gu8 seq = (gu8)uni_ptr(X.seqPool + (uint64_t)r0.buf * X.C.seqCap);
-  const int nAims = edge ? 0 : uni(dirRight ? X.nAncR : X.nAncL);
-  int lanc = uni((int)r0.lanc), ranc = uni((int)r0.ranc);
-  bool popped = false;
-  uint32_t* recN = (uint32_t*)g_dp;
-  uint32_t cFlush = cnt;
-  double dist = r0.dist;
-  int done = 0, flushed = 0;
-
-  auto flush = [&]() {
-    const int n = done - flushed;
-    if (n <= 0) return;
-    PROF_DECL; PROF_BEGIN();
-    const uint32_t cn = (l < n) ? recN[l] : 1u;
-    const uint32_t cprev = (l == 0) ? cFlush : ((l < n) ? recN[l - 1] : 1u);
-    const double term = fabs((double)cprev - (double)cn) / sqrt((double)cprev);
-    double* recT = (double*)(g_dp + 64);
-    recT[l] = term;
-    LSYNC();
-#pragma unroll 8
-    for (int j = 0; j < n; ++j) dist = dist + recT[j];
-    cFlush = (uint32_t)lane_get((int)cn, n - 1);
-    flushed = done;
-    LSYNC();
-    PROF_END(PF_FFFLUSH);
-  };
-
-  const uint32_t laneOff = (l < TALC_WALK_LEVELS) ? (uint32_t)(2 + (l >> 1)) : (l == TALC_WALK_LEVELS + 1 ? 1u : 0u);
-  const uint32_t laneShift = (l < TALC_WALK_LEVELS && (l & 1)) ? 16u : 0u;
-  const int lj = min(l, TALC_WALK_LEVELS - 1);
-  const uint32_t laneSingle = (l < TALC_WALK_LEVELS) ? kWalkSingle : 0u;
-  uint64_t key = dirRight ? (kmer & m1) : (kmer >> 2);
-  uint32_t hh = (uint32_t)(table_hash(key) >> 32);
-  PROF_END2(PF_FFENTRY);
-  uint32_t ePre = 0;
-  bool havePre = false;
-  while (done < maxSteps) {
-    if (done - flushed > 64 - TALC_WALK_LEVELS) flush();
+  const uint32_t laneOff = WL.laneOff, laneShift = WL.laneShift, laneSingle = WL.laneSingle;
+  const int lj = WL.lj;
+  uint64_t& kmer = W.kmer; uint64_t& key = W.key; uint32_t& hh = W.hh; uint32_t& cnt = W.cnt; uint32_t& ePre = W.ePre; bool& havePre = W.havePre;
+  int& done = W.done; const int flushed = W.flushed;
+  nOK = 0; aimIdx = -1;
     PROF_BEGIN();
     uint64_t slot = ((uint64_t)hh * (uint64_t)(uint32_t)cap) >> 32;
     uint32_t e = havePre ? ePre : wtab[slot * 8 + laneOff];
@@ -2267,22 +2220,22 @@
 #ifdef TALC_PROF
     if (l == 0) g_prof[PF_NRECS] += 1;
 #endif
-    if (!found) break;
+    if (!found) return 0;
     PROF_BEGIN();
     const uint32_t lev = (e >> laneShift) & 0xFFFFu, top = lev & kWalkTopNone;
 #ifdef TALC_PROF
     {
       const unsigned long long pm = ballot64((l < TALC_WALK_LEVELS) && (lev & kWalkSingle) != 0u);
       const int j0 = __builtin_ctzll(~pm);
-      if (j0 < TALC_WALK_LEVELS && j0 < maxSteps - done) {
+      if (j0 < TALC_WALK_LEVELS && j0 < room) {
         const uint32_t t0 = (uint32_t)lane_get((int)top, j0);
         if (l == 0) g_prof[(t0 >= X.P.MIN_COUNT) ? PF_FSFORK : PF_FSDEAD] += 1;
       }
     }
 #endif
     const unsigned long long passMask = ballot64((lev & laneSingle) != 0u);
-    int nOK = min(__builtin_ctzll(~passMask), maxSteps - done);
-    if (nOK == 0) break;
+    nOK = min(__builtin_ctzll(~passMask), room);
+    if (nOK == 0) return 0;
     const uint32_t which = (l < TALC_WALK_LEVELS) ? (lev >> kWalkBaseShift) : 0u;
     uint32_t pre = which << (dirRight ? 2 * (TALC_WALK_LEVELS - 1 - lj) : 2 * lj);
     pre |= dpp_row_shr<1>(pre, 0u);
@@ -2321,7 +2274,7 @@
     }
     const unsigned long long hitMask = ballot64(seen || dup) | (1ull << TALC_WALK_LEVELS);
     const int hitLevel = __builtin_ctzll(hitMask);
-    int aimIdx = -1;
+    aimIdx = -1;
     if (nAims > 0 && nAims <= AIMS_LDS && hitLevel < nOK) {
       const uint64_t kmH = ((uint64_t)(uint32_t)lane_get((int)(uint32_t)(km >> 32), hitLevel) << 32) | (uint32_t)lane_get((int)(uint32_t)km, hitLevel);
       const unsigned long long am = ballot64((l < nAims) && (g_aimK[l < AIMS_LDS ? l : 0] == kmH) && (g_aimN[l < AIMS_LDS ? l : 0] == 0ull));
@@ -2332,12 +2285,13 @@
 #endif
     nOK = min(nOK, hitLevel);
     const int nTake = nOK + (aimIdx >= 0 ? 1 : 0);
-    if (nTake == 0) break;
+    if (nTake == 0) return 0;
     if (l < nTake) {
       atomicOr(&g_bloom[bwi], bm);
       if (WIDEF) wide_or(wideW, bmW);
       recN[done - flushed + l] = top;
       seq[len0 + done + l] = (uint8_t)which;
+      also(len0 + done + l, which);
     }
     const int last = nTake - 1;
     kmer = ((uint64_t)(uint32_t)lane_get((int)(uint32_t)(km >> 32), last) << 32) | (uint32_t)lane_get((int)(uint32_t)km, last);
@@ -2348,6 +2302,84 @@
     done += nTake;
     LSYNC();
     PROF_END(PF_FFREC);
+  return nTake;
+}
+TALC_D void walk_flush(WalkTip& W, uint32_t* recN, uint32_t& cFlush, double& dist) {
+  const int l = lane_id();
+  int& done = W.done; int& flushed = W.flushed;
+  const int n = done - flushed;
+  if (n <= 0) return;
+  PROF_DECL; PROF_BEGIN();
+  const uint32_t cn = (l < n) ? recN[l] : 1u;
+  const uint32_t cprev = (l == 0) ? cFlush : ((l < n) ? recN[l - 1] : 1u);
+  const double term = fabs((double)cprev - (double)cn) / sqrt((double)cprev);
+  double* recT = (double*)(g_dp + 64);
+  recT[l] = term;
+  LSYNC();
+#pragma unroll 8
+  for (int j = 0; j < n; ++j) dist = dist + recT[j];
+  cFlush = (uint32_t)lane_get((int)cn, n - 1);
+  flushed = done;
+  LSYNC();
+  PROF_END(PF_FFFLUSH);
+}
+
+template <bool dirRight, bool WIDEF>
+TALC_D int fast_forward_walk(int len_, uint32_t& stepCounter_, uint32_t PATH_MAXLENGTH_, bool edge_) {
+  PROF_DECL2;
+  PROF_BEGIN2();
+  const DevParams& P = X.P;
+  const int l = lane_id();
+  const bool edge = uni((int)edge_) != 0;
+  if (uni((int)(X.traceSteps)) != 0) return 0;
+  const TrailRec r0 = tr_get(X.ia, 0);
+  if (uni64(r0.nmask) != 0ull) return 0;
+  const uint32_t K = (uint32_t)uni((int)P.K), CHECK = (uint32_t)uni((int)P.CHECK_INTERVAL);
+  const uint32_t seqCap = (uint32_t)uni((int)X.C.seqCap), PMAX = (uint32_t)uni((int)PATH_MAXLENGTH_);
+  const uint64_t cap = uni64(X.T.capacity);
+  const uint32_t TALC_AS1* wtab = (const uint32_t TALC_AS1*)uni_ptr(dirRight ? X.T.walkRight : X.T.walkLeft);
+  const uint32_t wideMask = WIDEF ? (uint32_t)uni((int)X.wideMask) : 0u;
+  unsigned long long* const wideBloom = WIDEF ? (unsigned long long*)uni_ptr(X.wideBloom) : nullptr;
+  const uint64_t m1 = (1ULL << (2 * (K - 1))) - 1;
+  WalkTip W;
+  uint64_t& kmer = W.kmer; uint32_t& cnt = W.cnt;
+  kmer = uni64(r0.kmer);
+  cnt = (uint32_t)uni((int)r0.cnt);
+  const int len0 = uni(len_);
+  const uint32_t sc0 = (uint32_t)uni((int)stepCounter_);
+  int maxSteps = 0;
+  if (sc0 < PMAX && (uint32_t)len0 < seqCap) {
+    maxSteps = (int)min(PMAX - sc0, seqCap - (uint32_t)len0);
+    if (edge) maxSteps = min(maxSteps, (int)(CHECK - (sc0 % CHECK)));
+  }
+  gu8 seq = (gu8)uni_ptr(X.seqPool + (uint64_t)r0.buf * X.C.seqCap);
+  const int nAims = edge ? 0 : uni(dirRight ? X.nAncR : X.nAncL);
+  int lanc = uni((int)r0.lanc), ranc = uni((int)r0.ranc);
+  bool popped = false;
+  uint32_t* recN = (uint32_t*)g_dp;
+  uint32_t cFlush = cnt;
+  double dist = r0.dist;
+  int& done = W.done; int& flushed = W.flushed;
+  done = 0; flushed = 0;
+
+  auto flush = [&]() { walk_flush(W, recN, cFlush, dist); };
+
+  WalkLanes WL;
+  WL.laneOff = (l < TALC_WALK_LEVELS) ? (uint32_t)(2 + (l >> 1)) : (l == TALC_WALK_LEVELS + 1 ? 1u : 0u);
+  WL.laneShift = (l < TALC_WALK_LEVELS && (l & 1)) ? 16u : 0u;
+  WL.lj = min(l, TALC_WALK_LEVELS - 1);
+  WL.laneSingle = (l < TALC_WALK_LEVELS) ? kWalkSingle : 0u;
+  W.key = dirRight ? (kmer & m1) : (kmer >> 2);
+  W.hh = (uint32_t)(table_hash(W.key) >> 32);
+  PROF_END2(PF_FFENTRY);
+  W.ePre = 0;
+  W.havePre = false;
+  while (done < maxSteps) {
+    if (done - flushed > 64 - TALC_WALK_LEVELS) flush();
+    int nOK, aimIdx;
+    const int nTake = walk_record<dirRight, WIDEF>(WL, W, maxSteps - done, wtab, cap, K, seq, len0, recN, nAims, wideMask, wideBloom, nOK, aimIdx,
+                                                   [](int, uint32_t) {});
+    if (nTake == 0) break;
     if (aimIdx >= 0) {
       flush();
       WSYNC();
@@ -2403,6 +2435,147 @@
                                 : fast_forward_walk<false, false>(len, stepCounter, PATH_MAXLENGTH, edge);
   }
   [[clang::musttail]] return fast_forward_steps(len, stepCounter, PATH_MAXLENGTH, edge);
+}
+
+struct EdgeLaneRet { int len; uint32_t stepCounter; int xdrop; int ff; int dead; int leafFell; };
+constexpr int kLaneStageOff = 768;
+
+template <bool dirRight>
+TALC_D EdgeLaneRet edge_lane_dir(int len_, uint32_t stepCounter_, uint32_t PATH_MAXLENGTH_, int xdrop_) {
+  PROF_DECL;
+  const DevParams& P = X.P;
+  const int l = lane_id();
+  EdgeLaneRet R;
+  R.len = uni(len_); R.stepCounter = (uint32_t)uni((int)stepCounter_); R.xdrop = uni(xdrop_); R.ff = 0; R.dead = 0; R.leafFell = 0;
+  if (uni((int)(X.traceSteps)) != 0) return R;
+  const TrailRec r0 = tr_get(X.ia, 0);
+  if (uni64(r0.nmask) != 0ull) return R;
+  const uint32_t K = (uint32_t)uni((int)P.K), CHECK = (uint32_t)uni((int)P.CHECK_INTERVAL);
+  const uint32_t seqCap = (uint32_t)uni((int)X.C.seqCap), PMAX = (uint32_t)uni((int)PATH_MAXLENGTH_);
+  const uint32_t MAXFAIL = (uint32_t)uni((int)P.MAX_BORDER_FAILURES);
+  const uint64_t cap = uni64(X.T.capacity);
+  const uint32_t TALC_AS1* wtab = (const uint32_t TALC_AS1*)uni_ptr(dirRight ? X.T.walkRight : X.T.walkLeft);
+  const uint64_t m1 = (1ULL << (2 * (K - 1))) - 1;
+  WalkTip W;
+  uint64_t& kmer = W.kmer; uint32_t& cnt = W.cnt;
+  kmer = uni64(r0.kmer);
+  cnt = (uint32_t)uni((int)r0.cnt);
+  const int len0 = R.len;
+  const uint32_t sc0 = R.stepCounter;
+  const uint32_t buf = (uint32_t)uni((int)r0.buf);
+  gu8 seq = (gu8)uni_ptr(X.seqPool + (uint64_t)buf * X.C.seqCap);
+  int lanc = uni((int)r0.lanc), ranc = uni((int)r0.ranc), score = uni((int)r0.score);
+  uint32_t fail = (uint32_t)uni((int)r0.fail);
+  int xdrop = R.xdrop;
+  uint32_t* recN = (uint32_t*)g_dp;
+  uint32_t cFlush = cnt;
+  double dist = r0.dist;
+  int& done = W.done; int& flushed = W.flushed;
+  done = 0; flushed = 0;
+  const int S = dirRight ? (int)K - 1 : (int)K;
+  const int refLen = uni((int)X.refLen);
+  const int dlen = refLen - S;
+  const int qpad = (dlen + 16) & ~7;
+  constexpr int STAGE = 3 * LDS_DP_CAP * 4;
+  const bool stageFits = dlen > 0 && kLaneStageOff + qpad + dlen + 16 <= STAGE;
+  uint8_t TALC_AS3* const stage = (uint8_t TALC_AS3*)g_dp + kLaneStageOff;
+  bool staged = false;
+  unsigned long long ncells = 0;
+#ifdef TALC_PROF
+  uint32_t rounds = 0;
+#endif
+
+  auto flush = [&]() { walk_flush(W, recN, cFlush, dist); };
+
+  WalkLanes WL;
+  WL.laneOff = (l < TALC_WALK_LEVELS) ? (uint32_t)(2 + (l >> 1)) : (l == TALC_WALK_LEVELS + 1 ? 1u : 0u);
+  WL.laneShift = (l < TALC_WALK_LEVELS && (l & 1)) ? 16u : 0u;
+  WL.lj = min(l, TALC_WALK_LEVELS - 1);
+  WL.laneSingle = (l < TALC_WALK_LEVELS) ? kWalkSingle : 0u;
+  W.key = dirRight ? (kmer & m1) : (kmer >> 2);
+  W.hh = (uint32_t)(table_hash(W.key) >> 32);
+  W.ePre = 0;
+  W.havePre = false;
+  uint32_t phase = sc0 % CHECK;
+
+  while (true) {
+    const uint32_t sc = sc0 + (uint32_t)done;
+    const int roundStart = done;
+    int lim = done;
+    if (sc < PMAX && (uint32_t)(len0 + done) < seqCap)
+      lim = done + (int)min(min(PMAX - sc, seqCap - (uint32_t)(len0 + done)), CHECK - phase);
+#ifdef TALC_PROF
+    ++rounds;
+#endif
+    while (done < lim) {
+      if (done - flushed > 64 - TALC_WALK_LEVELS) flush();
+      int nOK, aimIdx;
+      const int nTake = walk_record<dirRight, false>(WL, W, lim - done, wtab, cap, K, seq, len0, recN, 0, 0u, nullptr, nOK, aimIdx,
+                                                     [&](int pos, uint32_t base) { const int qi = pos - S; if (stageFits && qi < dlen) stage[qi] = (uint8_t)base; });
+      if (nTake == 0) break;
+      if (nOK < TALC_WALK_LEVELS) break;
+    }
+    R.ff = done - roundStart;
+    phase += (uint32_t)R.ff;
+    if (phase == CHECK) phase = 0;
+    if (R.ff == 0 || phase != 0) break;
+    const int len = len0 + done, x = xdrop + 2;
+    const int qlen = len - S;
+    if (!stageFits || len > refLen) break;
+    if (min(max(x, 0), qlen) + min(max(x, 0), dlen) + 1 > 63) break;
+    PROF_BEGIN();
+#ifdef TALC_PROF
+    if (l == 0) g_prof[PF_XCALLS] += 1;
+#endif
+    if (!staged) {
+      WSYNC();
+      stage_copy(stage, (gcu8)seq + S, qlen);
+      stage_copy(stage + qpad, (gcu8)uni_ptr(X.ref) + S, dlen);
+      if (l == 0) stage[qpad + dlen] = 0xF1;
+      staged = true;
+    }
+    if (l == 0) stage[qlen] = 0xF0;
+    int extCols = 0, extRows = 0, extScore = 0;
+    const int rc = wave_xdrop_wfa<1, true>(nullptr, qlen, nullptr, dlen, x, stage, STAGE - kLaneStageOff, extCols, extRows, extScore, ncells, nullptr, buf + 1u, qpad);
+    PROF_END(PF_XDROP);
+    const int lenRefExt = S + uni(extRows), lenHistExt = S + uni(extCols);
+    const int posOnRef = dirRight ? lenRefExt : (refLen - (int)K - uni(extRows));
+    bool stop = false;
+    int sNew;
+    if (max(lenRefExt, lenHistExt) >= (int)K) {
+      if (uni(rc) != 1) { R.leafFell = 1; break; }
+      sNew = uni(extScore);
+    } else { sNew = -x; stop = true; }
+    fail = (lenHistExt == len) ? 0u : fail + 1u;
+    score = sNew;
+    if (dirRight) ranc = posOnRef; else lanc = posOnRef;
+    if (!((fail <= MAXFAIL) & !stop)) { R.dead = 1; xdrop = 0; break; }
+    xdrop = (int)((double)score * (-1));
+    R.ff = 0;
+    if (!(sc0 + (uint32_t)done < PMAX)) break;
+  }
+
+  flush();
+  R.len = len0 + done; R.stepCounter = sc0 + (uint32_t)done; R.xdrop = xdrop;
+#ifdef TALC_PROF
+  if (l == 0) { g_prof[PF_NCALLS] += rounds; g_prof[PF_NSTEPS] += (uint32_t)done; }
+#endif
+  X.cells += ncells;
+  if (done) {
+    X.steps += (unsigned long long)done;
+    if (l == 0) {
+      TrailRec r;
+      r.kmer = kmer; r.nmask = 0ull; r.dist = dist; r.cnt = cnt; r.score = score; r.fail = fail; r.lanc = lanc; r.ranc = ranc; r.buf = buf;
+      tr_put(X.ia, 0, r);
+    }
+  }
+  if (R.dead | R.leafFell) WSYNC();
+  else LSYNC();
+  return R;
+}
+TALC_DN EdgeLaneRet edge_lane(int len, uint32_t stepCounter, uint32_t PATH_MAXLENGTH, int xdrop) {
+  return uni((int)X.dirRight) ? edge_lane_dir<true>(len, stepCounter, PATH_MAXLENGTH, xdrop)
+                              : edge_lane_dir<false>(len, stepCounter, PATH_MAXLENGTH, xdrop);
 }
 
 TALC_DN int fork_step(int len_, uint32_t sc_, uint32_t PMAX_) {
@@ -2804,13 +2977,30 @@
   int len = (int)K;
   while ((int)(nCur > 0) & (int)((uint32_t)nCur <= maxInner) & (int)((uint32_t)uni((int)stepCounter) < PATH_MAXLENGTH) & (int)(uni((int)X.overflow) == 0)) {
     if (nCur == 1) {
-      PROF_BEGIN2();
-      const int ff = uni(fast_forward(len, stepCounter, PATH_MAXLENGTH, true));
-      len += ff;
-      PROF_END2(PF_FFWD);
-      if (ff > 0 && ((uint32_t)uni((int)stepCounter) % CHECK == 0)) {
+      int ff;
+      bool leafFell = false;
+      if (uni((int)(X.T.walkRight != nullptr && X.P.MIN_COUNT < kWalkTopNone && X.wideMask == 0u && (X.taskTest & kTestNoEdgeLane) == 0u)) != 0) {
         PROF_BEGIN2();
-        nCur = uni(score_edges(X.ia, 1, len, xdrop));
+        const EdgeLaneRet R = edge_lane(len, stepCounter, PATH_MAXLENGTH, xdrop);
+        len = uni(R.len); stepCounter = (uint32_t)uni((int)R.stepCounter); xdrop = uni(R.xdrop); ff = uni(R.ff);
+        leafFell = uni(R.leafFell) != 0;
+        PROF_END2(PF_EDGELANE);
+        if (uni(R.dead) != 0) {
+          PROF_BEGIN2();
+          record_edge(X.ia, 0, len); pool_free((uint32_t)uni((int)tr_buf(X.ia, 0)));
+          nCur = 0;
+          PROF_END2(PF_STEPE);
+          continue;
+        }
+      } else {
+        PROF_BEGIN2();
+        ff = uni(fast_forward(len, stepCounter, PATH_MAXLENGTH, true));
+        len += ff;
+        PROF_END2(PF_FFWD);
+      }
+      if (leafFell || (ff > 0 && ((uint32_t)uni((int)stepCounter) % CHECK == 0))) {
+        PROF_BEGIN2();
+        nCur = uni(score_edges(X.ia, 1, len, xdrop, leafFell));
         PROF_END2(PF_STEPE);
         continue;
       }
@@ -3042,7 +3232,7 @@
     WSYNC();
     X.best2[0].have = false; X.best2[1].have = false;
     edge_anchor_search_task(mine, s);
-    if (X.taskTest) X.nanSeen = 1u;
+    if (X.taskTest & kTestEdgeRedo) X.nanSeen = 1u;
     edge_box_store(box, s, X.complexRegion ? 1u : 0u);
   }
   agent_fence();
diff --git a/talc_amd/csrc/talc_switches.h b/talc_amd/csrc/talc_switches.h
--- a/talc_amd/csrc/talc_switches.h
+++ b/talc_amd/csrc/talc_switches.h
@@ -19,6 +19,7 @@
   int edgeTasks = -1;
   uint32_t edgeTaskMin = 150, edgeTaskHeavy = 200, edgeTaskRounds = 0xFFFF, edgeLingerMod = 16;
   bool edgeRedo = false;
+  bool edgeLane = true;
   bool traceSteps = false;
   uint32_t fakeGpus = 0;
   std::string profReads;
@@ -45,6 +46,7 @@
   s.edgeTaskRounds = clamped("TALC_EDGE_TASK_ROUNDS", 0xFFFF, 0, 0xFFFF);
   s.edgeLingerMod = clamped("TALC_EDGE_LINGER_MOD", 16, 1, 1L << 20);
   s.edgeRedo = given("TALC_TEST_EDGE_REDO");
+  s.edgeLane = num("TALC_TEST_EDGE_LANE", 1) != 0;
   s.traceSteps = num("TALC_TRACE_STEPS", 0) != 0;
   s.fakeGpus = clamped("TALC_FAKE_GPUS", 0, 0, 1L << 20);
   if (const char* e = std::getenv("TALC_PROF_READS")) s.profReads = e;
diff --git a/talc_amd/csrc/talc_wave.h b/talc_amd/csrc/talc_wave.h
--- a/talc_amd/csrc/talc_wave.h
+++ b/talc_amd/csrc/talc_wave.h
@@ -586,11 +586,11 @@
 struct WfaKeep { uint32_t owner; int level; int qlenAt; int pad_; uint16_t F[64]; uint8_t E[64]; };
 __shared__ WfaKeep g_keep;
 
-template <int NR>
+template <int NR, bool PRESTAGED = false>
 TALC_D int wave_xdrop_wfa(const uint8_t* __restrict__ querySeg_, int qlen, const uint8_t* __restrict__ dbSeg_, int dlen, int x,
                           uint8_t TALC_AS3* stage, int stageCap, int& extCols, int& extRows, int& extScore,
-                          unsigned long long& cells, const WfaPhase* ph = nullptr, uint32_t keepKey_ = 0) {
-  gcu8 querySeg = (gcu8)uni_ptr(querySeg_); gcu8 dbSeg = (gcu8)uni_ptr(dbSeg_);
+                          unsigned long long& cells, const WfaPhase* ph = nullptr, uint32_t keepKey_ = 0, int qpadPre = 0) {
+  gcu8 querySeg = PRESTAGED ? nullptr : (gcu8)uni_ptr(querySeg_); gcu8 dbSeg = PRESTAGED ? nullptr : (gcu8)uni_ptr(dbSeg_);
   const int l = lane_id();
   qlen = uni(qlen); dlen = uni(dlen); x = uni(x);
   extCols = extRows = extScore = 0;
@@ -603,15 +603,15 @@
   const int nd = kmax - kmin + 1;
   if (nd > 64 * NR - 1) return -1;
   const int qS = min(qlen, dlen + X), dS = min(dlen, qlen + X);
-  const int qpad = (qS + 16) & ~7;
-  if (qpad + dS + 16 > stageCap) return -1;
+  const int qpad = PRESTAGED ? qpadPre : (qS + 16) & ~7;
+  if (!PRESTAGED && qpad + dS + 16 > stageCap) return -1;
   const unsigned long long _t0 = WPROF_T();
-  if (fromLevel < 0) {
+  if (!PRESTAGED && fromLevel < 0) {
     stage_copy(stage, querySeg, qS);
     stage_copy(stage + qpad, dbSeg, dS);
     if (l == 0) { stage[qS] = 0xF0; stage[qpad + dS] = 0xF1; }
   }
-  WSYNC();
+  if (PRESTAGED) LSYNC(); else WSYNC();
   WPROF_ADD(0, _t0);
   const unsigned long long _t1 = WPROF_T();
   const int bmax = x >= 2 ? x - 1 : (x == 1 ? 1 : 0);
diff --git a/talc_amd/csrc/talc_wfa.h b/talc_amd/csrc/talc_wfa.h
--- a/talc_amd/csrc/talc_wfa.h
+++ b/talc_amd/csrc/talc_wfa.h
@@ -7,15 +7,19 @@
 
 struct WfaResult { int moved; int extCols; int extRows; int score; };
 
-inline WfaResult wfa_xdrop_scalar(const uint8_t* q, int qlen, const uint8_t* d, int dlen, int x) {
+struct WfaKept { int level; int qlenAt; int F[64]; int E[64]; };
+constexpr int kWfaMaxKeepLevel = 31;
+
+inline WfaResult wfa_xdrop_scalar_run(const uint8_t* q, int qlen, const uint8_t* d, int dlen, int x, WfaKept* keep, bool* resumed) {
   WfaResult res = {0, 0, 0, 0};
+  if (resumed) *resumed = false;
   if (qlen == 0 || dlen == 0) return res;
   const int NEG = -(1 << 29);
   const int bmax = x >= 2 ? x - 1 : (x == 1 ? 1 : 0);
   const int X = x < 0 ? 0 : x;
   const int kmin = -(X < dlen ? X : dlen), kmax = (X < qlen ? X : qlen);
   const int nd = kmax - kmin + 1;
-  std::vector<int> F(nd + 2, NEG), G(nd + 2, NEG), E(nd + 2, 0), amin(nd + 2), amax(nd + 2);
+  std::vector<int> F(nd + 2, NEG), G(nd + 2, NEG), E(nd + 2, 0), EG(nd + 2, 0), amin(nd + 2), amax(nd + 2);
   auto idx = [&](int k) { return k - kmin + 1; };
   for (int k = kmin; k <= kmax; ++k) {
     const int ak = k < 0 ? -k : k;
@@ -29,10 +33,34 @@
     return c + r;
   };
   const int corner = qlen + dlen, kc = qlen - dlen;
-  F[idx(0)] = x >= 0 ? extend(0, 0) : 0;
-  bool cornerHit = (kc >= kmin && kc <= kmax && F[idx(kc)] == corner);
+  bool tracking = keep != nullptr;
+  auto keep_level = [&](int level) {
+    if (level < 1 || level > kWfaMaxKeepLevel) return;
+    keep->level = level; keep->qlenAt = qlen;
+    for (int k = -level; k <= level; ++k) {
+      const bool in = k >= kmin && k <= kmax;
+      keep->F[k + 32] = in ? F[idx(k)] : NEG;
+      keep->E[k + 32] = in ? E[idx(k)] : 0;
+    }
+  };
+  int eStart = 1;
+  bool cornerHit = false;
+  const int lv = keep ? keep->level : 0;
+  if (keep && lv >= 1 && lv < x && lv <= kWfaMaxKeepLevel && lv < keep->qlenAt && keep->qlenAt <= qlen && lv < dlen) {
+    for (int k = -lv; k <= lv; ++k) { F[idx(k)] = keep->F[k + 32] >= 0 ? keep->F[k + 32] : NEG; E[idx(k)] = keep->E[k + 32]; }
+    eStart = lv + 1;
+    if (resumed) *resumed = true;
+  } else {
+    F[idx(0)] = x >= 0 ? extend(0, 0) : 0;
+    cornerHit = (kc >= kmin && kc <= kmax && F[idx(kc)] == corner);
+    if (tracking && F[idx(0)] == 2 * qlen) tracking = false;
+  }
   int cornerE = 0;
-  for (int e = 1; e <= x && !cornerHit; ++e) {
+  int eLast = eStart - 1;
+  for (int e = eStart; e <= x && !cornerHit; ++e) {
+    if (tracking && (e == x || e == kWfaMaxKeepLevel + 1)) { keep_level(e - 1); tracking = false; }
+    bool meets = false;
+    EG = E;
     for (int k = kmin; k <= kmax; ++k) {
       const int i = idx(k);
       const int fm = F[i], fl = F[i - 1], fr = F[i + 1];
@@ -41,12 +69,16 @@
       for (int t = 0; t < 3; ++t)
         if (v[t] >= amin[i] && v[t] <= amax[i] && v[t] > best) best = v[t];
       int nv = fm;
-      if (best > fm) { nv = extend(best, k); E[i] = e; }
+      if (best > fm) { nv = extend(best, k); EG[i] = e; meets |= (nv == 2 * qlen - k); }
       G[i] = nv;
     }
+    if (tracking && meets) { keep_level(e - 1); tracking = false; }
     F.swap(G);
+    E.swap(EG);
     if (kc >= kmin && kc <= kmax && F[idx(kc)] == corner) { cornerHit = true; cornerE = e; }
+    eLast = e;
   }
+  if (tracking && !cornerHit && eLast < x) keep_level(eLast);
   if (cornerHit) { res.moved = 1; res.extCols = qlen; res.extRows = dlen; res.score = -cornerE; return res; }
   int A = 0;
   for (int k = kmin; k <= kmax; ++k) if (F[idx(k)] > A) A = F[idx(k)];
@@ -104,4 +136,8 @@
   return res;
 }
 
+inline WfaResult wfa_xdrop_scalar(const uint8_t* q, int qlen, const uint8_t* d, int dlen, int x) {
+  return wfa_xdrop_scalar_run(q, qlen, d, dlen, x, nullptr, nullptr);
 }
+
+}
```

New measurement: 4.759 billion (median of 6 runs). 1.02x the previous value.
